# Guillaume-SOULIER/SOS-Radiative-Transfer

Measured on AMD Instinct MI355X. Metric: SOS columns/sec to 1e-4 convergence (Ntau=200, Nmu=128), higher is better.
Workload: dtype f64

## Files before the change

### include/sosrt.h

```cpp
#ifndef SOSRT_H
#define SOSRT_H

#ifdef __cplusplus
extern "C" {
#endif

typedef struct sosrt_handle sosrt_t;

#define SOSRT_OK              0
#define SOSRT_E_INVALID      -1
#define SOSRT_E_HIP          -2
#define SOSRT_E_STATE        -3
#define SOSRT_E_NOMEM        -4

#define SOSRT_COL_OK           0
#define SOSRT_COL_INDEXERROR   1
#define SOSRT_COL_MAXORDERS    2
#define SOSRT_COL_INTERNAL     3

#define SOSRT_GEOM_THREE_ZONE  0
#define SOSRT_GEOM_SINGLE_SLAB 1

#define SOSRT_SURFACE_NONE       0
#define SOSRT_SURFACE_SPECULAR   1
// ... 78 lines not shown
#define SOSRT_PHASE_TABLE     3
int sosrt_phase_table(sosrt_t* h, const double* tab_mu, const double* tab_p, int ntab);
int sosrt_phase_table_dev(sosrt_t* h, const double* d_tab_mu, const double* d_tab_p, int ntab);

#define SOSRT_MIE_MAX_X 20000.0
#define SOSRT_MIE_MAX_MX 200000.0
#define SOSRT_MIE_MAX_WORKSPACE (2ull << 30)
int sosrt_mie_ensembles(sosrt_t* h, int S, const double* wl, const double* m_re, const double* m_im, const double* r_m,
                        const double* sig, int nb_radius, double r_min, double r_max, int ntab, double* p_out, double* bulk_out);
int sosrt_mie_ensembles_dev(sosrt_t* h, int S, const double* wl, const double* m_re, const double* m_im, const double* r_m,
                            const double* sig, int nb_radius, double r_min, double r_max, int ntab, double* d_p_out,
                            double* d_bulk_out);
int sosrt_mie_efficiencies(sosrt_t* h, int K, const double* m_re, const double* m_im, const double* x, double* out);
int sosrt_mie_timing(sosrt_t* h, double* ms );

int sosrt_phase_p0_dev(sosrt_t* h, int B, int kind, double g, const double* d_mu0, double* d_P0_out);
int sosrt_phase_p0(sosrt_t* h, int B, int kind, double g, const double* mu0, double* P0_out);
int sosrt_phase_matrix(sosrt_t* h, int kind, double g, double* P_out);
int sosrt_phase_matrix_dev(sosrt_t* h, int kind, double g, double* d_P_out);

#define SOSRT_MAX_MODES 64
int sosrt_phase_modes(sosrt_t* h, int kind, double g, int m_first, int m_count, int nphi, double* P_out);
int sosrt_phase_p0_modes_dev(sosrt_t* h, int B, int kind, double g, int m_first, int m_count, int nphi, const double* d_mu0,
                             double* d_P0_out);
int sosrt_phase_p0_modes(sosrt_t* h, int B, int kind, double g, int m_first, int m_count, int nphi, const double* mu0,
                         double* P0_out);
int sosrt_set_order_targets(sosrt_t* h, const int* d_targets);
int sosrt_azimuth_accumulate_dev(sosrt_t* h, int B, int m, const double* d_Im, int nlev, const int* d_levels, int nphi_out,
                                 const double* d_phi, double* d_out);

int sosrt_comm_unique_id(void* id_out);
int sosrt_comm_init(sosrt_t* h, int rank, int world, const void* unique_id);
int sosrt_gather(sosrt_t* h, int root, const long long* counts, const double* d_send, double* d_recv);
int sosrt_comm_destroy(sosrt_t* h);

int sosrt_limit_mu_down(sosrt_t* h, int R, int idx, const double* rows, double* out);
int sosrt_asymptotic_down(sosrt_t* h, int R, int stride, const int* len, const double* J, const double* tau,
                          const double* tau_t, const double* mu, double* out);

int sosrt_plan_weights(sosrt_t* h, double* w_out );
int sosrt_plan_fold(sosrt_t* h, int which , double* W_out );
int sosrt_plan_fix_table(sosrt_t* h, int idx, int* s0, int* ns, double* C_out);
int sosrt_plan_fix_count(double tau_ref, int N);
#define SOSRT_PLAN_GEMM_DENSE        0
#define SOSRT_PLAN_GEMM_LIVE64       1
#define SOSRT_PLAN_GEMM_LIVE32       2
#define SOSRT_PLAN_GEMM_LIVE32_DEEP  3
#define SOSRT_PLAN_GEMM_LIVE16_REGS  4
#define SOSRT_PLAN_TRANSPORT_GENERAL 0
#define SOSRT_PLAN_TRANSPORT_FAST    1
#define SOSRT_PLAN_TRANSPORT_RING    3
#define SOSRT_PLAN_TRANSPORT_SCAN    4
int sosrt_plan_launch(sosrt_t* h, int batch, int live, int surface, int zones, int cus, int* out );

#define SOSRT_K_GEMM      0
#define SOSRT_K_TRANSPORT 1
#define SOSRT_K_FIRST     2
#define SOSRT_K_SMALLMU   3
#define SOSRT_K_ORDER_LOOP 4
#define SOSRT_K_COUNT     5
int sosrt_profile_enable(sosrt_t* h, int on);
int sosrt_profile_reset(sosrt_t* h);
int sosrt_profile_get(sosrt_t* h, int kernel, double* total_ms, long long* launches, double* work );

int sosrt_debug_stamps(sosrt_t* h, unsigned long long* d_stamps);

int sosrt_microbench(sosrt_t* h, int which, double* result);

#ifdef __cplusplus
}
#endif
#endif
```

### sos-radiative-transfer_amd/csrc/api.hip

```cpp
#include <hip/hip_runtime.h>

#include <algorithm>
#include <cmath>
#include <cstdarg>
#include <cstdio>
#include <cstdlib>
#include <chrono>
#include <cstring>
#include <mutex>
#include <new>
#include <string>
#include <vector>

#include "../../include/sosrt.h"
#include "comm.hpp"
#include "kernels.hpp"
#include "plan.hpp"

using namespace sosrt;

namespace {
thread_local std::string g_err;

int fail(int code, const char* fmt, ...) {
// ... 62 lines not shown
    int ntab = 0;
    char* d_mie = nullptr;
    char* h_mie = nullptr;
    size_t mie_cap = 0, mie_hcap = 0;
    hipEvent_t mie_ev = nullptr, mie_t[4] = {nullptr, nullptr, nullptr, nullptr};
    bool mie_timed = false;
    bool resident = false;
    int resident_B = 0;
    FixTab* d_fix = nullptr;
    int* d_small = nullptr;
    int *d_idx_up = nullptr, *d_idx_down = nullptr;
    int *d_nz = nullptr, *d_zr0 = nullptr, *d_zmix = nullptr;
    double *d_zwr = nullptr, *d_zdtr = nullptr;
    int max_nz = 1;
    bool simple_zones = true;
    double* d_scal = nullptr;
    ColDesc* d_desc = nullptr;
    double *d_rca = nullptr, *d_rcr = nullptr;
    int* d_slabrows = nullptr;
    int* d_mainrows = nullptr;
    int nslab = 0, nmain = 0;
    int max_main = 0, max_slab = 0;
    static constexpr int kMaxMixGroups = 32;
    static constexpr int kMaxMixGroupsSets = 128;
    static constexpr size_t kMixCacheBytes = 256ull << 20;
    int mix_groups_max = 1 << 30;
    bool wr_on_device = false;
    int nsets = 1;
    std::vector<std::vector<double>> Wrx_h;
    double* d_Wrsets = nullptr;
    size_t wrsets_capacity = 0;
    double* d_Wrsets_s = nullptr;
    size_t wrsets_s_capacity = 0;
    int* d_mixset = nullptr;
    int max_set_used = 0;
    int p0_zones = 0;
    double* d_P0rz = nullptr;
    size_t p0rz_capacity = 0;
    std::vector<int> c_nz, c_zr0, c_zmix, c_zset;
    std::vector<double> c_zwr, c_zdtr, c_alb_atm, c_dtau_atm;
    int mix_groups = 0;
    bool mix_dirty = true;
    double *d_Wmix = nullptr, *d_mixca = nullptr, *d_mixcr = nullptr;
    int* d_mixgroup = nullptr;
    int* d_slabtilegroup = nullptr;
    int contraction = SOSRT_CONTRACT_F64;
    double asymmetry = 0;
    bool sym_ok = false;
    bool sym_dirty = true, symmix_dirty = true, symsets_dirty = true;
    double *d_Wa_s = nullptr, *d_Wr_s = nullptr, *d_Wmix_s = nullptr;
    int lr_rank = -1;
    double lr_residual = 0;
    double *d_lrU = nullptr, *d_lrV = nullptr;
    size_t mixs_capacity = 0;
    float *d_Wa32 = nullptr, *d_Wmix32 = nullptr;
    size_t mix32_capacity = 0;
    bool w32_dirty = true;
    int* d_livelist = nullptr;
    size_t mix_capacity = 0;
    double *d_tau = nullptr, *d_P0a = nullptr, *d_P0r = nullptr;
    double *d_Jn = nullptr, *d_InA = nullptr, *d_InB = nullptr, *d_I = nullptr, *d_E = nullptr;
    int use_etab = 1;
    int *d_active = nullptr, *d_norders = nullptr, *d_status = nullptr, *d_redo = nullptr, *d_erep = nullptr;
    int *d_nactive_sets = nullptr, *d_nactive = nullptr;
    int nactive_set = 0;
    unsigned long long* d_tauhash = nullptr;
    int transport_mode = 3;
    int scan_cols = 200;
    bool ring_ok = false, scan_ok = false, scan_split_ok = false;
    int scan_split = 1;
    int cu_count = 0;
    double* d_scan_scratch = nullptr;
    int* d_scan_sync = nullptr;
    int gemm_tail_cols = 1 << 30;
    double gemm_tail_frac = 0.6;
    int gemm_small_cols = 200;
    int dense_live_list = 1;
    int gemm_regs_cols = -1;
    bool fast_ok = false;
    double* d_ratio = nullptr;
    int* h_pub = nullptr;
    bool need_small = true;
    int pub_seq = 0;
    int last_max_orders = 0;
    long long last_sum_orders = 0;
    Prof prof[kMaxGroups];
    int order_loop = 0;
    double ol_frac = 0.5;
    int* d_olsync = nullptr;
    int* h_oldone = nullptr;
    unsigned long long* d_ollog = nullptr;
    int ol_launches = 0, ol_refused = 0;
    bool ol_group_used[kMaxGroups] = {false, false};
    Rccl::comm_t comm = nullptr;
    int comm_rank = -1, comm_world = 0;
};

namespace {

size_t field_elems(const sosrt_handle* h) { return (size_t)h->max_batch * h->L * h->D; }

template <class T>
int dalloc(T** p, size_t n) {
    hipError_t e = hipMalloc((void**)p, n * sizeof(T));
    if (e != hipSuccess) return fail(SOSRT_E_NOMEM, "hipMalloc of %zu bytes failed: %s", n * sizeof(T), hipGetErrorString(e));
    return 0;
// ... 178 lines not shown
}

int ensure_matrices(sosrt_handle* h, hipStream_t s) {
    const Grid& g = h->g;
    const size_t per = (size_t)g.Dp * g.Wld;
    const bool mixed = h->mix_groups > 0 && h->mix_dirty;
    if (mixed) {
        prof_break(h);
        const bool sets = h->max_set_used > 0;
        launch_wmix(s, per, h->mix_groups, h->d_Wa, sets ? h->d_Wrsets : h->d_Wr, h->d_mixca, h->d_mixcr, h->d_Wmix,
                    sets ? h->d_mixset : nullptr);
        h->mix_dirty = false;
        h->symmix_dirty = true;
    }
    if (!use_sym(h)) return 0;
    if (h->sym_dirty) {
        prof_break(h);
        if (!h->d_Wa_s) { if (int e = dalloc(&h->d_Wa_s, per)) return e; }
        if (!h->d_Wr_s) { if (int e = dalloc(&h->d_Wr_s, per)) return e; }
        launch_symfold(s, 1, g.N, g.D, g.Dp, g.Wld, h->d_Wa, h->d_Wa_s);
        launch_symfold(s, 1, g.N, g.D, g.Dp, g.Wld, h->d_Wr, h->d_Wr_s);
        h->sym_dirty = false;
        h->symsets_dirty = true;
    }
    if (h->symsets_dirty && h->nsets > 1 && h->mix_groups == 0 && h->max_set_used > 0) {
        prof_break(h);
        {
            if (per * h->nsets > h->wrsets_s_capacity) {
                if (h->d_Wrsets_s) hipFree(h->d_Wrsets_s);
                h->d_Wrsets_s = nullptr; h->wrsets_s_capacity = 0;
                if (int e = dalloc(&h->d_Wrsets_s, per * h->nsets)) return e;
                h->wrsets_s_capacity = per * h->nsets;
            }
            launch_symfold(s, h->nsets, g.N, g.D, g.Dp, g.Wld, h->d_Wrsets, h->d_Wrsets_s);
        }
        h->symsets_dirty = false;
    }
    if (h->mix_groups > 0 && h->symmix_dirty) {
        prof_break(h);
        const size_t need = per * h->mix_groups;
        if (need > h->mixs_capacity) {
            if (h->d_Wmix_s) hipFree(h->d_Wmix_s);
            h->d_Wmix_s = nullptr; h->mixs_capacity = 0;
            if (int e = dalloc(&h->d_Wmix_s, need)) return e;
            h->mixs_capacity = need;
        }
        launch_symfold(s, h->mix_groups, g.N, g.D, g.Dp, g.Wld, h->d_Wmix, h->d_Wmix_s);
        h->symmix_dirty = false;
    }
    return 0;
}

void run_source(sosrt_handle* h, const double* In_1, double* Jn, const int* active, int tail_cols = 0, int pub_tag = 0,
                int grp = -1, bool all_live = false, bool regs_tile = false, int dense_live_cap = 0) {
    const int g0 = grp < 0 ? 0 : grp, g1 = grp < 0 ? h->ngroups : grp + 1;
    const int pg = grp < 0 ? 0 : grp;
    hipStream_t s = group_stream(h, pg);
    GemmArgs ga;
    ga.A = In_1; ga.Wa = h->d_Wa; ga.Wr = h->d_Wr; ga.ca = h->d_rca; ga.cr = h->d_rcr;
    if (h->nslab > 0) {
        ga.rows_main = h->d_mainrows + h->main_off[g0];
        ga.n_main = h->main_off[g1] - h->main_off[g0];
    } else {
        ga.rows_main = nullptr;
        ga.n_main = (h->gb[g1] - h->gb[g0]) * h->L;
        ga.A = In_1 + (size_t)h->gb[g0] * h->L * h->D;
        Jn += (size_t)h->gb[g0] * h->L * h->D;
        ga.ca = h->d_rca + (size_t)h->gb[g0] * h->L;
        ga.cr = h->d_rcr + (size_t)h->gb[g0] * h->L;
        if (active) active += h->gb[g0];
    }
    ga.rows_slab = h->d_slabrows + h->slab_off[g0]; ga.n_slab = h->slab_off[g1] - h->slab_off[g0];
    ga.D = h->g.D; ga.Dp = h->g.Dp; ga.Wld = h->g.Wld; ga.L = h->L; ga.C = Jn; ga.active = active;
    if (grp >= 0 && h->ngroups > 1) ga.pad_lds = h->coresident_pad;
    if (pub_tag) {
        ga.nactive = h->d_nactive + pg; ga.need_small = h->d_nactive + sosrt_handle::kMaxGroups;
        ga.host_pub = h->h_pub + 8 * pg; ga.tag = pub_tag;
    }
    ga.check_tiles = all_live ? 0 : 1;
    if (ensure_matrices(h, s)) return;
    if (h->mix_groups > 0) {
        ga.Wmix = h->d_Wmix; ga.mix_group = h->d_mixgroup; ga.slab_tile_group = h->d_slabtilegroup + h->slab_off[g0] / 32;
    }
    const bool two_pass_sets = h->mix_groups == 0 && h->max_set_used > 0 && h->nslab > 0;
    if (two_pass_sets) {
        ga.Wr = h->d_Wrsets; ga.mix_group = h->d_mixgroup; ga.slab_tile_group = h->d_slabtilegroup + h->slab_off[g0] / 32;
    }
    if (use_lowrank(h)) { ga.lr_rank = h->lr_rank; ga.lrU = h->d_lrU; ga.lrV = h->d_lrV; }
    if (use_sym(h)) {
        ga.sym = 1; ga.Ks = (h->g.N + GEMM_KC - 1) / GEMM_KC * GEMM_KC;
#ifdef SOSRT_DIAG
        if (h->diag_ks_mult > 1 && ga.Ks * h->diag_ks_mult <= h->g.Dp) ga.Ks *= h->diag_ks_mult;
#endif
        ga.Wa = h->d_Wa_s; ga.Wr = two_pass_sets ? h->d_Wrsets_s : h->d_Wr_s;
        if (ga.Wmix) ga.Wmix = h->d_Wmix_s;
    }
    if (h->contraction == SOSRT_CONTRACT_F32) {
        if (h->w32_dirty) {
            prof_break(h);
            const size_t per = (size_t)h->g.Dp * h->g.Wld;
            launch_to_float(s, per, h->d_Wa, h->d_Wa32);
            if (h->mix_groups > 0) launch_to_float(s, per * h->mix_groups, h->d_Wmix, h->d_Wmix32);
            h->w32_dirty = false;
        }
        prof_begin(h, SOSRT_K_GEMM, pg);
        launch_gemm_f32(s, ga, h->d_Wa32, h->d_Wmix32);
        prof_end(h, SOSRT_K_GEMM, pg);
        return;
    }
    prof_begin(h, SOSRT_K_GEMM, pg);
    if (tail_cols > 0 && active && h->nslab >= 0) {
        ga.col0 = h->nslab > 0 ? h->gb[g0] : 0; ga.B = h->gb[g1] - h->gb[g0];
        ga.max_main = h->max_main; ga.max_slab = h->max_slab;
        ga.idx_up = h->nslab > 0 ? h->d_idx_up : nullptr; ga.idx_down = h->nslab > 0 ? h->d_idx_down : nullptr;
        ga.live_list = h->d_livelist + h->gb[g0]; ga.live_cap = tail_cols;
        launch_gemm_tail(s, ga, tail_cols, tail_cols <= h->gemm_small_cols, regs_tile);
    } else {
        if (dense_live_cap > 0 && active && h->nslab >= 0) {
            ga.col0 = h->nslab > 0 ? h->gb[g0] : 0; ga.B = h->gb[g1] - h->gb[g0];
            ga.live_list = h->d_livelist + h->gb[g0]; ga.live_cap = dense_live_cap;
        }
        launch_gemm(s, ga);
    }
    prof_end(h, SOSRT_K_GEMM, pg);
}

struct SolveShape {
    bool ring_like = false;
    bool fast = false;
    int nzcap = kRingZones;
    int ring_mode = 1;
};
SolveShape solve_shape(const sosrt_handle* h, int max_nz) {
    SolveShape sh;
    sh.ring_like = h->transport_mode >= 2 && h->ring_ok && (max_nz <= kRingZones || transport_ring_fits(h->g, max_nz));
    sh.fast = h->transport_mode >= 1 && h->fast_ok && (max_nz <= kRingZones || sh.ring_like);
    sh.nzcap = max_nz > kRingZones ? max_nz : kRingZones;
    sh.ring_mode = (h->transport_mode >= 2 && h->ring_ok) ? 3 : 1;
    return sh;
}
struct OrderInputs {
    int nb = 0;
    int known = 0;
    int surface = SOSRT_SURFACE_NONE;
    bool simple_zones = true;
    bool slabs_mixed = true;
    bool need_small = false;
    bool saving = false;
    int orders_left = 1 << 30;
    int cu_share = 0;
};
struct LaunchPlan {
    int tail_cols = 0;
    int live_cap = 0;
    int gemm = SOSRT_PLAN_GEMM_DENSE;
    int transport = SOSRT_PLAN_TRANSPORT_GENERAL;
    int parts = 1;
    int repair = 0;
    int order_loop = 0;
    int ol_parts = 0;
    int ol_grid = 0;
};
LaunchPlan plan_order(const sosrt_handle* h, const SolveShape& sh, const OrderInputs& in) {
    LaunchPlan pl;
    const Grid& g = h->g;
    const bool live_tiling = h->contraction != SOSRT_CONTRACT_F32 && in.simple_zones && in.known <= h->gemm_tail_cols &&
                             (in.known <= h->gemm_tail_frac * in.nb || in.nb <= h->gemm_small_cols) &&
                             (in.known < in.nb || in.nb <= h->gemm_small_cols);
    pl.tail_cols = live_tiling ? in.known : 0;
    pl.gemm = !live_tiling ? SOSRT_PLAN_GEMM_DENSE
                           : (pl.tail_cols <= h->gemm_small_cols ? ((use_sym(h) && pl.tail_cols <= 32) ? SOSRT_PLAN_GEMM_LIVE32_DEEP : SOSRT_PLAN_GEMM_LIVE32)
                                                                 : SOSRT_PLAN_GEMM_LIVE64);
    {
        const int nct = (g.D + GEMM_BN - 1) / GEMM_BN;
        const int auto_cap = (3 * h->cu_count / 2) / (((g.L + 15) / 16 + 1) * nct);
        const int cap = h->gemm_regs_cols >= 0 ? h->gemm_regs_cols : auto_cap;
        if (live_tiling && use_sym(h) && pl.tail_cols <= cap && 16 * (g.D + 2) * 8 <= 150 * 1024 &&
            ((g.N + GEMM_KC - 1) / GEMM_KC * GEMM_KC) % 64 == 0) pl.gemm = SOSRT_PLAN_GEMM_LIVE16_REGS;
    }
    pl.live_cap = live_tiling ? pl.tail_cols : ((h->contraction != SOSRT_CONTRACT_F32 && h->dense_live_list && in.known < in.nb) ? in.known : 0);
    {
        const int cols_now = pl.live_cap > 0 ? pl.live_cap : in.nb;
        const int split_cap = sh.ring_mode == 3 ? h->cu_count : 4 * h->cu_count;
        const bool can_split = h->scan_split && h->scan_split_ok && transport_scan_parts(g) * cols_now <= split_cap &&
                               (in.surface == SOSRT_SURFACE_SPECULAR || in.surface == SOSRT_SURFACE_NONE);
        const bool want_scan = h->transport_mode == 4 || (h->transport_mode == 3 && cols_now <= h->scan_cols);
        const bool split = can_split && transport_scan_fits(g, sh.nzcap, true) && (sh.fast || (h->use_etab && h->transport_mode >= 3));
        const bool scan = want_scan && ((sh.fast && sh.ring_mode == 3 && h->scan_ok && transport_scan_fits(g, sh.nzcap, false)) || split);
        pl.transport = scan ? SOSRT_PLAN_TRANSPORT_SCAN
                            : (!sh.fast ? SOSRT_PLAN_TRANSPORT_GENERAL : (sh.ring_mode == 3 ? SOSRT_PLAN_TRANSPORT_RING : SOSRT_PLAN_TRANSPORT_FAST));
        if (scan && split) pl.parts = transport_scan_parts(g);
        pl.repair = (h->N - 3 > 61 && pl.transport == SOSRT_PLAN_TRANSPORT_FAST) ? 1 : 0;
    }
    if (h->order_loop && in.cu_share > 0 && h->transport_mode == 3 && sh.fast && sh.ring_mode == 3 && sh.nzcap <= kRingZones &&
        use_sym(h) && in.simple_zones && in.slabs_mixed && !in.saving && !in.need_small && in.orders_left >= 1 &&
        in.known <= kOrderLoopMaxCols) {
        Grid gt = g;
        gt.nsmall = 0;
        const bool split_ok = h->scan_split && (in.surface == SOSRT_SURFACE_SPECULAR || in.surface == SOSRT_SURFACE_NONE) && order_loop_ok(gt, true);
        const int sp = order_loop_parts(gt, true);
        if (split_ok && sp * in.known <= h->ol_frac * in.cu_share) {
            pl.order_loop = 1; pl.ol_parts = sp;
        } else if (order_loop_ok(gt, false) && in.known <= h->ol_frac * in.cu_share) {
            pl.order_loop = 1; pl.ol_parts = 1;
        }
        if (pl.order_loop) pl.ol_grid = in.cu_share;
    }
    return pl;
}

std::mutex g_ol_mutex;
int g_ol_held[64];
int ol_acquire(int device, int total, int want, int least) {
    if (device < 0 || device >= 64) return 0;
    std::lock_guard<std::mutex> lk(g_ol_mutex);
    int got = total - g_ol_held[device];
    if (got > want) got = want;
    if (got < least || got <= 0) return 0;
    g_ol_held[device] += got;
    return got;
}
void ol_release(int device, int n) {
    if (device < 0 || device >= 64 || n <= 0) return;
    std::lock_guard<std::mutex> lk(g_ol_mutex);
    g_ol_held[device] -= n;
}

}

extern "C" {

const char* sosrt_last_error(void) { return g_err.c_str(); }
int sosrt_version(void) { return SOSRT_VERSION; }

int sosrt_plan_fix_count(double tau_ref, int N) { return fix_count(tau_ref, N); }

int sosrt_create(int device, int L, int N, int max_batch, int max_orders, sosrt_t** out) {
    if (!out) return fail(SOSRT_E_INVALID, "out is null");
    *out = nullptr;
    if (L < 2) return fail(SOSRT_E_INVALID, "nb_layers must be >= 2 (got %d)", L);
    if (N < 4) return fail(SOSRT_E_INVALID, "nb_angles must be >= 4 (got %d)", N);
    if (N > 1024) return fail(SOSRT_E_INVALID, "nb_angles must be <= 1024 (got %d)", N);
    if (max_batch < 1 || max_orders < 1) return fail(SOSRT_E_INVALID, "max_batch and max_orders must be >= 1");
    {
        const int nt = (N + 63) / 64 * 64;
        const size_t need = (size_t)(3 * (size_t)L + nt + nt / 64 + 4) * sizeof(double);
        if (need > 64 * 1024)
            return fail(SOSRT_E_INVALID, "nb_layers = %d does not fit: at most %d layers at nb_angles = %d", L,
                        (int)((64 * 1024 / sizeof(double) - nt - nt / 64 - 4) / 3), N);
    }
    sosrt_handle* h = new (std::nothrow) sosrt_handle();
    if (!h) return fail(SOSRT_E_NOMEM, "out of host memory");
    h->device = device; h->L = L; h->N = N; h->D = 2 * N; h->max_batch = max_batch; h->max_orders = max_orders;
    h->order_budget = max_orders;
    h->saved_slots = max_orders;
    h->gpu = device >= 0;
    h->cu_count = 256;
    if (const char* ev = getenv("SOSRT_ETAB")) h->use_etab = atoi(ev);
    if (const char* ev = getenv("SOSRT_CONTRACT"))
        if (strcmp(ev, "full") == 0) h->contraction = SOSRT_CONTRACT_F64_FULL;
    if (const char* ev = getenv("SOSRT_TRANSPORT"))
        h->transport_mode = strcmp(ev, "general") == 0 ? 0 : (strcmp(ev, "ring") == 0 ? 2 : (strcmp(ev, "scan") == 0 ? 4 : (strcmp(ev, "auto") == 0 ? 3 : 1)));
    if (const char* ev = getenv("SOSRT_SCAN_COLS")) h->scan_cols = atoi(ev);
    if (const char* ev = getenv("SOSRT_SCAN_SPLIT")) h->scan_split = atoi(ev);
    if (const char* ev = getenv("SOSRT_GEMM_TAIL")) h->gemm_tail_cols = atoi(ev);
    if (const char* ev = getenv("SOSRT_GEMM_TAIL_FRAC")) h->gemm_tail_frac = atof(ev);
    if (const char* ev = getenv("SOSRT_GEMM_SMALL")) h->gemm_small_cols = atoi(ev);
    if (const char* ev = getenv("SOSRT_DENSE_LIVE_LIST")) h->dense_live_list = atoi(ev) != 0;
    if (const char* ev = getenv("SOSRT_GEMM_REGS")) h->gemm_regs_cols = atoi(ev);
    if (const char* ev = getenv("SOSRT_GROUPS")) h->want_groups = atoi(ev) >= 2 ? 2 : (atoi(ev) == 1 ? 1 : 0);
    if (const char* ev = getenv("SOSRT_SPLIT_MIN")) h->split_min = atoi(ev);
    if (const char* ev = getenv("SOSRT_MIX_GROUPS")) h->mix_groups_max = atoi(ev);
#ifdef SOSRT_DIAG
    if (const char* ev = getenv("SOSRT_STAGGER")) h->stagger = atof(ev);
    if (const char* ev = getenv("SOSRT_GROUP_SPLIT")) h->split_at = atoi(ev);
    if (const char* ev = getenv("SOSRT_GROUP_PRIO")) h->prio2 = atoi(ev);
    if (const char* ev = getenv("SOSRT_GEMM_PAD_LDS")) h->coresident_pad = atoi(ev);
    if (const char* ev = getenv("SOSRT_GEMM_KS_MULT")) h->diag_ks_mult = atoi(ev);
#endif
    if (const char* ev = getenv("SOSRT_GROUP_RING_SLOTS")) h->coresident_slots = atoi(ev);
    if (const char* ev = getenv("SOSRT_ORDER_LOOP")) h->order_loop = atoi(ev) != 0;
    if (const char* ev = getenv("SOSRT_RING_SLOTS")) g_ring_slots = atoi(ev);
#ifdef SOSRT_RING_DEBUG
    if (const char* ev = getenv("SOSRT_RING_DEBUG")) g_ring_debug = atoi(ev);
#endif
    Grid& g = h->g;
    g.L = L; g.N = N; g.D = 2 * N;
    g.Dp = (g.D + GEMM_KC - 1) / GEMM_KC * GEMM_KC;
    g.Wld = (g.D + GEMM_BN - 1) / GEMM_BN * GEMM_BN;
    if (h->gpu) {
        int e = 0;
        auto body = [&]() -> int {
            HIPCHK(hipSetDevice(device));
            HIPCHK(hipStreamCreateWithFlags(&h->own_stream, hipStreamDefault));
            h->stream = h->own_stream;
            HIPCHK(hipEventCreateWithFlags(&h->ev_fork, hipEventDisableTiming));
            HIPCHK(hipEventCreateWithFlags(&h->ev_join, hipEventDisableTiming));
            const size_t mb = max_batch, fe = field_elems(h);
            if ((e = dalloc(&h->d_mu, g.D))) return e;
            if ((e = dalloc(&h->d_Wa, (size_t)g.Dp * g.Wld))) return e;
            if ((e = dalloc(&h->d_Wr, (size_t)g.Dp * g.Wld))) return e;
            if ((e = dalloc(&h->d_lrU, (size_t)kLowRankMax * g.D))) return e;
            if ((e = dalloc(&h->d_lrV, (size_t)kLowRankMax * g.D))) return e;
            if ((e = dalloc(&h->d_wfdn, N))) return e;
            if ((e = dalloc(&h->d_wfup, N))) return e;
            if ((e = dalloc(&h->d_w, g.D))) return e;
            if ((e = dalloc(&h->d_phi, 2 * kNPhi))) return e;
            if ((e = dalloc(&h->d_z, L))) return e;
            if ((e = dalloc(&h->d_fix, 4))) return e;
            if ((e = dalloc(&h->d_small, N))) return e;
            if ((e = dalloc(&h->d_idx_up, mb))) return e;
            if ((e = dalloc(&h->d_idx_down, mb))) return e;
            if ((e = dalloc(&h->d_nz, mb))) return e;
            if ((e = dalloc(&h->d_zr0, mb * kMaxZones))) return e;
            if ((e = dalloc(&h->d_zmix, mb * kMaxZones))) return e;
            if ((e = dalloc(&h->d_zwr, mb * kMaxZones))) return e;
            if ((e = dalloc(&h->d_zdtr, mb * kMaxZones))) return e;
            if ((e = dalloc(&h->d_scal, 7 * mb))) return e;
            if ((e = dalloc(&h->d_desc, mb))) return e;
            if ((e = dalloc(&h->d_rca, mb * L))) return e;
            if ((e = dalloc(&h->d_rcr, mb * L))) return e;
            if ((e = dalloc(&h->d_slabrows, mb * L + 64 * (size_t)sosrt_handle::kMaxMixGroupsSets * sosrt_handle::kMaxGroups))) return e;
            if ((e = dalloc(&h->d_slabtilegroup, mb * L / 32 + 2 * sosrt_handle::kMaxMixGroupsSets * sosrt_handle::kMaxGroups + 2))) return e;
            if ((e = dalloc(&h->d_mainrows, mb * L))) return e;
            if ((e = dalloc(&h->d_tau, mb * L))) return e;
            if ((e = dalloc(&h->d_P0a, mb * g.D))) return e;
            if ((e = dalloc(&h->d_P0r, mb * g.D))) return e;
            if ((e = dalloc(&h->d_Jn, fe))) return e;
            if ((e = dalloc(&h->d_InA, fe))) return e;
            if ((e = dalloc(&h->d_InB, fe))) return e;
            if ((e = dalloc(&h->d_I, fe))) return e;
            if ((e = dalloc(&h->d_E, fe))) return e;
            if ((e = dalloc(&h->d_active, mb))) return e;
            if ((e = dalloc(&h->d_norders, mb))) return e;
            if ((e = dalloc(&h->d_status, mb))) return e;
            if ((e = dalloc(&h->d_nactive_sets, 2 * (sosrt_handle::kMaxGroups + 1)))) return e;
            HIPCHK(hipMemset(h->d_nactive_sets, 0, 2 * (sosrt_handle::kMaxGroups + 1) * sizeof(int)));
            h->d_nactive = h->d_nactive_sets;
            if ((e = dalloc(&h->d_redo, mb))) return e;
            if ((e = dalloc(&h->d_erep, mb))) return e;
            if ((e = dalloc(&h->d_mixgroup, mb))) return e;
            if ((e = dalloc(&h->d_livelist, mb))) return e;
            if ((e = dalloc(&h->d_mixca, sosrt_handle::kMaxMixGroupsSets))) return e;
            if ((e = dalloc(&h->d_mixcr, sosrt_handle::kMaxMixGroupsSets))) return e;
            if ((e = dalloc(&h->d_mixset, sosrt_handle::kMaxMixGroupsSets))) return e;
            if ((e = dalloc(&h->d_tauhash, mb))) return e;
            if ((e = dalloc(&h->d_ratio, mb))) return e;
            if ((e = dalloc(&h->d_scan_scratch, mb * transport_scan_scratch_doubles()))) return e;
            if ((e = dalloc(&h->d_scan_sync, 2 * mb))) return e;
            if ((e = dalloc(&h->d_olsync, sosrt_handle::kMaxGroups * order_loop_sync_ints(kOrderLoopMaxCols)))) return e;
            HIPCHK(hipHostMalloc((void**)&h->h_oldone, 2 * sosrt_handle::kMaxGroups * sizeof(int), hipHostMallocCoherent));
            memset(h->h_oldone, 0, 2 * sosrt_handle::kMaxGroups * sizeof(int));
            HIPCHK(hipMemset(h->d_scan_sync, 0, 2 * mb * sizeof(int)));
            HIPCHK(hipDeviceGetAttribute(&h->cu_count, hipDeviceAttributeMultiprocessorCount, device));
            HIPCHK(hipHostMalloc((void**)&h->h_pub, (8 * sosrt_handle::kMaxGroups + 2) * sizeof(int), hipHostMallocCoherent));
            memset(h->h_pub, 0, (8 * sosrt_handle::kMaxGroups + 2) * sizeof(int));

            HIPCHK(hipMemset(h->d_Wa, 0, (size_t)g.Dp * g.Wld * sizeof(double)));
            HIPCHK(hipMemset(h->d_Wr, 0, (size_t)g.Dp * g.Wld * sizeof(double)));
            HIPCHK(hipMemset(h->d_status, 0, mb * sizeof(int)));
            HIPCHK(hipMemset(h->d_redo, 0, mb * sizeof(int)));
            HIPCHK(hipMemset(h->d_tau, 0, mb * L * sizeof(double)));
            return 0;
        };
        if ((e = body())) { sosrt_destroy(h); return e; }
        g.mu = h->d_mu; g.Wa = h->d_Wa; g.Wr = h->d_Wr; g.fix = h->d_fix; g.small_lanes = h->d_small;
        g.wflux_dn = h->d_wfdn; g.wflux_up = h->d_wfup; g.nsmall = 0;
    }
    *out = h;
    return 0;
}

int sosrt_destroy(sosrt_t* h) {
    if (!h) return 0;
    if (h->gpu) {
        hipSetDevice(h->device);
        if (h->comm) { rccl().CommDestroy(h->comm); h->comm = nullptr; }
        if (h->own_stream) hipStreamSynchronize(h->own_stream);
        void* ptrs[] = {h->d_mu, h->d_Wa, h->d_Wr, h->d_wfdn, h->d_wfup, h->d_fix, h->d_small, h->d_idx_up,
                        h->d_idx_down, h->d_scal, h->d_desc, h->d_rca, h->d_rcr, h->d_slabrows, h->d_mainrows, h->d_tau, h->d_P0a,
                        h->d_P0r, h->d_Jn, h->d_InA, h->d_InB, h->d_I, h->d_E, h->d_active, h->d_norders, h->d_status,
                        h->d_nactive_sets, h->d_ratio, h->d_redo, h->d_erep, h->d_tauhash, h->d_Wmix, h->d_mixca, h->d_mixcr,
                        h->d_mixgroup, h->d_Wa_s, h->d_Wr_s, h->d_Wmix_s, h->d_scan_scratch, h->d_scan_sync, h->d_w, h->d_phi, h->d_z, h->d_tab, h->d_slabtilegroup, h->d_livelist, h->d_Wa32, h->d_Wmix32, h->d_nz, h->d_zr0, h->d_zmix, h->d_zwr, h->d_zdtr, h->d_olsync, h->d_ollog, h->d_modetab, h->d_lrU, h->d_lrV, h->d_Wrsets, h->d_Wrsets_s, h->d_mixset, h->d_P0rz};
        for (void* p : ptrs)
            if (p) hipFree(p);
        if (h->h_pub) hipHostFree(h->h_pub);
        if (h->h_oldone) hipHostFree(h->h_oldone);
        if (h->d_mie) hipFree(h->d_mie);
        if (h->h_mie) hipHostFree(h->h_mie);
        if (h->mie_ev) hipEventDestroy(h->mie_ev);
        for (auto& e : h->mie_t)
            if (e) hipEventDestroy(e);

        for (auto& p : h->prof)
            for (auto& e : p.ev) hipEventDestroy(e);
        if (h->stream2) { hipStreamSynchronize(h->stream2); hipStreamDestroy(h->stream2); }
        if (h->ev_fork) hipEventDestroy(h->ev_fork);
        if (h->ev_join) hipEventDestroy(h->ev_join);
        if (h->own_stream) hipStreamDestroy(h->own_stream);
    }
    delete h;
    return 0;
}

int sosrt_set_stream(sosrt_t* h, void* s) {
    if (int e = need_gpu(h)) return e;
    h->stream = (hipStream_t)s;
    return 0;
}

int sosrt_use_own_stream(sosrt_t* h) {
    if (int e = need_gpu(h)) return e;
    h->stream = h->own_stream;
    return 0;
}

int sosrt_set_saved_orders(sosrt_t* h, int slots) {
    if (!h) return fail(SOSRT_E_INVALID, "null handle");
    if (slots < 1 || slots > h->max_orders) return fail(SOSRT_E_INVALID, "slots must be in 1..max_orders=%d (got %d)", h->max_orders, slots);
    h->saved_slots = slots;
    return 0;
}

int sosrt_set_order_budget(sosrt_t* h, int max_orders) {
    if (!h) return fail(SOSRT_E_INVALID, "null handle");
    if (max_orders < 1 || max_orders > h->max_orders)
        return fail(SOSRT_E_INVALID, "the order budget must be in 1..max_orders=%d of sosrt_create (got %d)", h->max_orders, max_orders);
    h->order_budget = max_orders;
    return 0;
}

int sosrt_set_first_order(sosrt_t* h, int mode) {
    if (int e = need_gpu(h)) return e;
    if (mode != SOSRT_FIRST_ORDER_CODED && mode != SOSRT_FIRST_ORDER_README) return fail(SOSRT_E_INVALID, "unknown first-order mode %d", mode);
    if (mode == SOSRT_FIRST_ORDER_README && (h->nsets > 1 || h->p0_zones > 0))
        return fail(SOSRT_E_INVALID, "SOSRT_FIRST_ORDER_README reads one aerosol matrix: it cannot be combined with several phase sets");
    if (mode == SOSRT_FIRST_ORDER_README && h->geom != SOSRT_GEOM_THREE_ZONE)
        return fail(SOSRT_E_INVALID, "the README's Lambertian first order needs the three-zone geometry (it has a surface)");
    h->first_order_mode = mode;
    return 0;
}

int sosrt_set_contraction(sosrt_t* h, int mode) {
    if (int e = need_gpu(h)) return e;
    if (mode != SOSRT_CONTRACT_F64 && mode != SOSRT_CONTRACT_F32 && mode != SOSRT_CONTRACT_F64_FULL && mode != SOSRT_CONTRACT_F64_DENSE) return fail(SOSRT_E_INVALID, "unknown contraction mode %d", mode);
    if (mode == SOSRT_CONTRACT_F32) {
        HIPCHK(hipSetDevice(h->device));
        const size_t per = (size_t)h->g.Dp * h->g.Wld;
        if (!h->d_Wa32) { if (int e = dalloc(&h->d_Wa32, per)) return e; }
        h->w32_dirty = true;
    }
    h->contraction = mode;
    return 0;
}

int sosrt_set_order_loop(sosrt_t* h, int mode) {
    if (!h) return fail(SOSRT_E_INVALID, "null handle");
    if (mode < 0 || mode > 2) return fail(SOSRT_E_INVALID, "order-loop mode must be 0, 1 or 2 (got %d)", mode);
    h->order_loop = mode;
    return 0;
}

int sosrt_order_loop_stats(sosrt_t* h, int* launches, int* refused, long long* column_orders) {
    if (!h) return fail(SOSRT_E_INVALID, "null handle");
    if (launches) *launches = h->ol_launches;
    if (refused) *refused = h->ol_refused;
    if (column_orders) {
        *column_orders = 0;
        if (h->gpu && h->ol_launches > 0) {
            HIPCHK(hipSetDevice(h->device));
            HIPCHK(hipStreamSynchronize(h->stream));
            if (h->stream2) HIPCHK(hipStreamSynchronize(h->stream2));
            for (int k = 0; k < sosrt_handle::kMaxGroups; ++k) {
                if (!h->ol_group_used[k]) continue;
                int v = 0;
                HIPCHK(hipMemcpy(&v, h->d_olsync + (size_t)k * order_loop_sync_ints(kOrderLoopMaxCols) + kOlOrders, sizeof v, hipMemcpyDeviceToHost));
                *column_orders += v;
            }
        }
    }
    return 0;
}

int sosrt_plan_launch(sosrt_t* h, int batch, int live, int surface, int zones, int cus, int* out) {
    if (!h || !out) return fail(SOSRT_E_INVALID, "null argument");
    if (!h->have_grid) return fail(SOSRT_E_STATE, "sosrt_set_grid has not been called");
    if (batch < 1 || live < 0 || live > batch) return fail(SOSRT_E_INVALID, "need 0 <= live <= batch, batch >= 1");
    if (zones < 1 || zones > kMaxZones) return fail(SOSRT_E_INVALID, "zones must be in 1..%d", kMaxZones);
    int want = h->want_groups;
    if (want == 0) want = batch > h->split_min ? 2 : 1;
    const int ng = (want >= 2 && batch >= h->split_min && batch >= 2) ? 2 : 1;
    const int nb = ng == 2 ? batch / 2 : batch;
    const int saved_cus = h->cu_count;
    if (cus > 0) h->cu_count = cus;
    const SolveShape sh = solve_shape(h, zones);
    OrderInputs oi;
    oi.nb = nb; oi.known = live < nb ? live : nb; oi.surface = surface;
    oi.simple_zones = zones == 3 || zones == 1;
    oi.cu_share = h->cu_count / ng;
    const bool saved_sym = h->sym_ok;
    if (!h->have_phase) h->sym_ok = true;
    const LaunchPlan pl = plan_order(h, sh, oi);
    h->sym_ok = saved_sym;
    h->cu_count = saved_cus;
    out[0] = ng; out[1] = pl.gemm; out[2] = pl.tail_cols; out[3] = pl.transport; out[4] = pl.parts; out[5] = pl.repair;
    out[6] = pl.order_loop; out[7] = pl.ol_parts; out[8] = pl.ol_grid;
    return 0;
}

int sosrt_phase_asymmetry(sosrt_t* h, double* asymmetry, int* uses_symmetry) {
    if (!h) return fail(SOSRT_E_INVALID, "null handle");
    if (!h->have_phase) return fail(SOSRT_E_STATE, "sosrt_set_phase has not been called");
    if (asymmetry) *asymmetry = h->asymmetry;
    if (uses_symmetry) *uses_symmetry = use_sym(h) ? 1 : 0;
    return 0;
}

int sosrt_phase_rank(sosrt_t* h, int* rank, double* residual, int* uses) {
    if (!h) return fail(SOSRT_E_INVALID, "null handle");
    if (!h->have_phase) return fail(SOSRT_E_STATE, "sosrt_set_phase has not been called");
    if (rank) *rank = h->lr_rank;
    if (residual) *residual = h->lr_residual;
    if (uses) *uses = use_lowrank(h) ? 1 : 0;
    return 0;
}

int sosrt_synchronize(sosrt_t* h) {
    if (int e = need_gpu(h)) return e;
    HIPCHK(hipStreamSynchronize(h->stream));
    return 0;
}

int sosrt_set_grid(sosrt_t* h, const double* mu) {
    if (!h || !mu) return fail(SOSRT_E_INVALID, "null argument");
    for (int k = 0; k < h->D; ++k)
        if (!std::isfinite(mu[k])) return fail(SOSRT_E_INVALID, "mu[%d] is not finite", k);
    for (int k = 0; k < h->N; ++k) {
        if (!(mu[k] <= 0)) return fail(SOSRT_E_INVALID, "mu[%d]=%g: the first nb_angles directions must be <= 0", k, mu[k]);
        if (!(mu[h->N + k] >= 0)) return fail(SOSRT_E_INVALID, "mu[%d]=%g: the last nb_angles directions must be >= 0", h->N + k, mu[h->N + k]);
    }
    h->plan.set_grid(h->N, mu);
    for (int b = 0; b < 4; ++b)
        if (h->plan.fix[b].idx > kFixMaxIdx) return fail(SOSRT_E_INVALID, "nb_angles too large for the extrapolation tables");
    h->have_grid = true;
    h->have_phase = false;
    h->fast_ok = transport_fast_ok(h->plan);
    if (h->gpu) {
        HIPCHK(hipSetDevice(h->device));
        HIPCHK(hipMemcpy(h->d_mu, mu, h->D * sizeof(double), hipMemcpyHostToDevice));
        HIPCHK(hipMemcpy(h->d_wfdn, h->plan.wflux_dn.data(), h->N * sizeof(double), hipMemcpyHostToDevice));
        HIPCHK(hipMemcpy(h->d_wfup, h->plan.wflux_up.data(), h->N * sizeof(double), hipMemcpyHostToDevice));
        HIPCHK(hipMemcpy(h->d_w, h->plan.w.data(), h->D * sizeof(double), hipMemcpyHostToDevice));
        {
            double phi[kNPhi], tab[2 * kNPhi];
            const double step = 3.141592653589793 / (kNPhi - 1);
            for (int q = 0; q < kNPhi; ++q) phi[q] = q * step;
            phi[kNPhi - 1] = 3.141592653589793;
            for (int q = 0; q < kNPhi; ++q) {
                tab[q] = std::cos(0 - phi[q]);
// ... 772 lines not shown
                if (got == 0) { oi.cu_share = 0; pl = plan_order(h, shape, oi); }
                else { pl.ol_grid = got; ol_held[k] = got; }
            }
            if (pl.order_loop && h->order_loop == 2) pl.ol_grid = 2 * h->cu_count;
            if (pl.order_loop) {
                OrderLoopArgs oa;
                Grid gt = g;
                gt.nsmall = 0;
                oa.t = TransportArgs{gt, tau_g, h->d_Jn + fo, nullptr, d_I_out + fo, nullptr, 0, h->d_desc + q.b0, q.cv, 0, 1, h->d_E, erep_g, nullptr};
                oa.t.nzcap = kRingZones;
                oa.t.scan_split = pl.ol_parts > 1 ? 1 : 0;
                oa.t.scan_scratch = h->d_scan_scratch + (size_t)q.b0 * transport_scan_scratch_doubles();
                oa.t.scan_sync = h->d_scan_sync + 2 * q.b0;
                GemmArgs& ga = oa.gm;
                ga.A = nullptr; ga.Wa = h->d_Wa_s; ga.Wr = h->d_Wr_s; ga.ca = h->d_rca; ga.cr = h->d_rcr;
                ga.D = g.D; ga.Dp = g.Dp; ga.Wld = g.Wld; ga.L = h->L; ga.C = h->d_Jn;
                ga.sym = 1; ga.Ks = (g.N + GEMM_KC - 1) / GEMM_KC * GEMM_KC;
                if (use_lowrank(h)) { ga.lr_rank = h->lr_rank; ga.lrU = h->d_lrU; ga.lrV = h->d_lrV; }
                ga.max_main = h->max_main; ga.max_slab = h->max_slab;
                ga.idx_up = h->nslab > 0 ? h->d_idx_up : nullptr; ga.idx_down = h->nslab > 0 ? h->d_idx_down : nullptr;
                if (h->mix_groups > 0) { ga.Wmix = h->d_Wmix_s; ga.mix_group = h->d_mixgroup; }
                oa.in0 = q.In_1;
                oa.gbufP = q.In;
                oa.gbufQ = (q.In_1 == d_I_out) ? h->d_InA : q.In_1;
                oa.bufP = oa.gbufP + fo; oa.bufQ = oa.gbufQ + fo;
                oa.order0 = q.n + 1; oa.kmax = h->order_budget - q.n;
                oa.B = q.nb; oa.col0 = q.b0;
                oa.fixcap = (int)(0.06 * g.N) + 1;
                oa.sync = h->d_olsync + (size_t)k * order_loop_sync_ints(kOrderLoopMaxCols);
                oa.host_done = h->h_oldone + 2 * k;
                oa.tag = q.ol_tag = ((++h->pub_seq) & 0x3fffffff) | 0x40000000;
#ifdef SOSRT_OL_STAMPS
                if (getenv("SOSRT_OL_LOG")) {
                    if (!h->d_ollog) { if (int e = dalloc(&h->d_ollog, 65001)) return bail(e); }
                    HIPCHK(hipMemsetAsync(h->d_ollog, 0, 8, sg));
                    oa.log = h->d_ollog;
                }
#endif
                prof_break(h);
                HIPCHK(hipMemsetAsync(oa.sync, 0, order_loop_sync_ints(q.known) * sizeof(int), sg));
                prof_begin(h, SOSRT_K_ORDER_LOOP, k);
                const hipError_t le = launch_order_loop(sg, pl.ol_grid, pl.ol_parts > 1, oa);
                prof_end(h, SOSRT_K_ORDER_LOOP, k);
                if (le != hipSuccess) return bail(fail(SOSRT_E_HIP, "order-loop launch failed: %s", hipGetErrorString(le)));
                q.ol_pending = true;
                used_order_loop = true;
                ++h->ol_launches;
                continue;
            }
            const int n = ++q.n;
            n_max = n > n_max ? n : n_max;
            const int tail_cols = pl.tail_cols;
            run_source(h, q.In_1, h->d_Jn, h->d_active, tail_cols, tagbase + n - 1, k, q.known == q.nb, pl.gemm == SOSRT_PLAN_GEMM_LIVE16_REGS,
                       tail_cols > 0 ? 0 : pl.live_cap);
            if (g.nsmall > 0 && h->need_small) {
                prof_begin(h, SOSRT_K_SMALLMU, k);
                launch_smallmu(sg, g, q.nb, tau_g, h->d_Jn + fo, q.In + fo, h->d_desc + q.b0, q.cv.active);
                prof_end(h, SOSRT_K_SMALLMU, k);
            }
            prof_begin(h, SOSRT_K_TRANSPORT, k);
            double* sv_n = (d_I_saved_out && n <= h->saved_slots) ? d_I_saved_out + (size_t)q.b0 * saved_stride + (size_t)(n - 1) * LD : nullptr;
            if (pl.transport != SOSRT_PLAN_TRANSPORT_GENERAL) {
                Grid gt = g;
                if (pl.transport >= SOSRT_PLAN_TRANSPORT_RING && !h->need_small) gt.nsmall = 0;
                launch_transport(sg, gt, q.nb, tau_g, h->d_Jn + fo, q.In + fo, d_I_out + fo, sv_n, saved_stride, h->d_desc + q.b0, q.cv, n, 1,
                                 h->d_E, pl.transport, erep_g, pl.live_cap, h->d_livelist + q.b0, NG > 1 ? h->coresident_slots : 0,
                                 pl.parts > 1 ? 1 : 0, h->d_scan_scratch + (size_t)q.b0 * transport_scan_scratch_doubles(),
                                 h->d_scan_sync + 2 * q.b0, nzcap);
                if (pl.repair)
                    launch_transport(sg, g, q.nb, tau_g, h->d_Jn + fo, q.In + fo, d_I_out + fo, sv_n, saved_stride, h->d_desc + q.b0, q.cv, n, 1,
                                     h->d_E, 2, erep_g);
            } else {
                launch_transport(sg, g, q.nb, tau_g, h->d_Jn + fo, q.In + fo, d_I_out + fo, sv_n, saved_stride, h->d_desc + q.b0, q.cv, n, 1,
                                 h->use_etab ? h->d_E : nullptr, 0, erep_g);
            }
            prof_end(h, SOSRT_K_TRANSPORT, k);
            if (q.In_1 == d_I_out) { q.In_1 = q.In; q.In = h->d_InA; }
            else { double* tmp = q.In_1; q.In_1 = q.In; q.In = tmp; }
        }
        if (!progressed) __builtin_ia32_pause();
    }
    if (NG > 1) {
        HIPCHK(hipEventRecord(h->ev_join, h->stream2));
        HIPCHK(hipStreamWaitEvent(s, h->ev_join, 0));
    }
    prof_break(h);
    launch_finalize(s, B, make_conv(h, tol), h->order_budget, d_n_orders_out, d_status_out);
    HIPCHK(hipGetLastError());
    h->last_max_orders = used_order_loop ? -1 : n_max;
    h->last_sum_orders = -1;
    return 0;
}

int sosrt_solve(sosrt_t* h, int B, const double* tau, const double* P0_atm, const double* P0_aer, double tol,
                const double* I1_in, double* I_out, double* I_saved_out, int* n_orders_out, int* status_out) {
    if (int e = check_ready(h, B, true)) return e;
    if (!tau) return fail(SOSRT_E_INVALID, "null argument");
    HIPCHK(hipSetDevice(h->device));
    hipStream_t s = h->stream;
    h->resident = false;
    const size_t LD = (size_t)h->L * h->D, n = (size_t)B * LD;
    HIPCHK(hipMemcpyAsync(h->d_tau, tau, (size_t)B * h->L * sizeof(double), hipMemcpyHostToDevice, s));
    if (P0_atm) HIPCHK(hipMemcpyAsync(h->d_P0a, P0_atm, (size_t)B * h->D * sizeof(double), hipMemcpyHostToDevice, s));
    const double* d_p0r = nullptr;
    if (int e = stage_p0_aer(h, B, P0_aer, s, &d_p0r)) return e;
    double* d_I1 = nullptr;
    double* d_saved = nullptr;
    int rc = 0;
    auto body = [&]() -> int {
        if (I1_in) {
            if (int e = dalloc(&d_I1, n)) return e;
            HIPCHK(hipMemcpyAsync(d_I1, I1_in, n * sizeof(double), hipMemcpyHostToDevice, s));
        }
        if (I_saved_out) {
            if (int e = dalloc(&d_saved, (size_t)B * h->saved_slots * LD)) return e;
            HIPCHK(hipMemsetAsync(d_saved, 0, (size_t)B * h->saved_slots * LD * sizeof(double), s));
        }
        if (int e = sosrt_solve_dev(h, B, h->d_tau, P0_atm ? h->d_P0a : nullptr, d_p0r, tol, d_I1,
                                    h->d_I, d_saved, nullptr, nullptr))
            return e;
        if (I_out) HIPCHK(hipMemcpyAsync(I_out, h->d_I, n * sizeof(double), hipMemcpyDeviceToHost, s));
// ... 759 lines not shown
```

### sos-radiative-transfer_amd/csrc/jn_gemm_tile.hpp

```cpp
#pragma once
#include "kernels.hpp"
#include "transport_util.hpp"

namespace sosrt {

namespace {

typedef double f64x4 __attribute__((ext_vector_type(4)));

constexpr int A_LD = GEMM_KC + 2;
constexpr int B_LD = GEMM_BN + 16;

struct ListRows {
    const int* rows;
    int n;
    __device__ int operator()(int lr) const { return lr < n ? (rows ? rows[lr] : lr) : -1; }
};
struct ColumnRows {
    int base, iu, ns, n;
    bool slab;
    __device__ int operator()(int lr) const {
        if (lr >= n) return -1;
        return base + (slab ? iu + lr : (lr < iu ? lr : lr + ns));
    }
// ... 290 lines not shown
        const int b_ = (blk_);                                                                                    \
        if (b_ < nblk) {                                                                                          \
            const int pass_ = b_ >= nkb ? 1 : 0;                                                                  \
            lone_load(F, pass_ ? rW1 : rW0, b_ - pass_ * nkb, fk, Wld, Nh, mcol);                                 \
        }                                                                                                         \
    }
    const __amdgpu_buffer_rsrc_t rW0 = make_rsrc(wmix ? wmix : g.Wa, g.Dp * Wld * 8);
    const __amdgpu_buffer_rsrc_t rW1 = make_rsrc(SLAB ? g.Wr : g.Wa, g.Dp * Wld * 8);
    if (!PRELOADED) {
        SOSRT_LONE_LOAD(f0, 0);
        SOSRT_LONE_LOAD(f1, 1);
    }
    asm volatile("s_waitcnt vmcnt(0)" ::: "memory");
    __syncthreads();
    f64x4 accx = (f64x4){0, 0, 0, 0}, accy = (f64x4){0, 0, 0, 0};
    const double* __restrict__ arow = sRaw + (size_t)fr * RS;
#define SOSRT_LONE_COMPUTE(F, blk_)                                                                               \
    {                                                                                                             \
        const int b_ = (blk_);                                                                                    \
        const int pass_ = b_ >= nkb ? 1 : 0;                                                                      \
        const double cf_ = pass_ ? cf_r : cf_a;                                                                   \
        const int k0_ = 4 * (b_ - pass_ * nkb) * LONE_KB + fk;                                                    \
        _Pragma("unroll") for (int q = 0; q < LONE_KB; ++q) {                                                     \
            const int k_ = k0_ + 4 * q;                                                                           \
            const bool ok_ = grow >= 0 && k_ < Nn;                                                                \
            const double a_ = arow[k_], m_ = arow[D - 1 - k_];                  \
            const double u_ = ok_ ? cf_ * (a_ + m_) : 0.0, v_ = ok_ ? cf_ * (a_ - m_) : 0.0;                      \
            accx = __builtin_amdgcn_mfma_f64_16x16x4f64(u_, F.s[q], accx, 0, 0, 0);                               \
            accy = __builtin_amdgcn_mfma_f64_16x16x4f64(v_, F.a[q], accy, 0, 0, 0);                               \
        }                                                                                                         \
    }
    for (int blk = 0; blk < nblk; blk += 2) {
        SOSRT_LONE_COMPUTE(f0, blk);
        SOSRT_LONE_LOAD(f0, blk + 2);
        if (blk + 1 < nblk) {
            SOSRT_LONE_COMPUTE(f1, blk + 1);
            SOSRT_LONE_LOAD(f1, blk + 3);
        }
    }
#undef SOSRT_LONE_LOAD
#undef SOSRT_LONE_COMPUTE
#pragma unroll
    for (int r = 0; r < 4; ++r) {
        const int gr = row_of(tile * 16 + 4 * r + fk);
        if (gr >= 0 && mcol < Nn) {
            const double x = accx[r], y = accy[r];
            g.C[(size_t)gr * D + mcol] = x + y;
            g.C[(size_t)gr * D + D - 1 - mcol] = x - y;
        }
    }
}

constexpr int LR_ROWS = 4;
template <bool COH>
__device__ __forceinline__ void lowrank_rows(const GemmArgs& g, const int (&rows)[LR_ROWS], int lane) {
    const int D = g.D, R = g.lr_rank;
    __amdgpu_buffer_rsrc_t rA[LR_ROWS], rC[LR_ROWS];
    double cf[LR_ROWS];
#pragma unroll
    for (int i = 0; i < LR_ROWS; ++i) {
        const int r = rows[i] >= 0 ? rows[i] : rows[0];
        const int bytes = rows[i] >= 0 ? D * 8 : 0;
        rA[i] = make_rsrc(g.A + (size_t)r * D, bytes);
        rC[i] = make_rsrc(g.C + (size_t)r * D, bytes);
        cf[i] = rows[i] >= 0 ? g.ca[rows[i]] : 0.0;
    }
    const double* __restrict__ U = g.lrU;
    const double* __restrict__ V = g.lrV;
    double m[LR_ROWS][kLowRankMax];
#pragma unroll
    for (int i = 0; i < LR_ROWS; ++i)
#pragma unroll
        for (int q = 0; q < kLowRankMax; ++q) m[i][q] = 0.0;
#pragma unroll 2
    for (int k = 2 * lane; k < D; k += 128) {
        double2 x[LR_ROWS];
#pragma unroll
        for (int i = 0; i < LR_ROWS; ++i) x[i] = bload2_aux<COH ? 16 : 0>(rA[i], k * 8, 0);
#pragma unroll
        for (int q = 0; q < kLowRankMax; ++q) {
            if (q < R) {
                const double2 u = *reinterpret_cast<const double2*>(U + (size_t)q * D + k);
#pragma unroll
                for (int i = 0; i < LR_ROWS; ++i) m[i][q] = __builtin_fma(x[i].y, u.y, __builtin_fma(x[i].x, u.x, m[i][q]));
            }
        }
    }
#pragma unroll
    for (int s = 32; s >= 1; s >>= 1)
#pragma unroll
        for (int q = 0; q < kLowRankMax; ++q)
            if (q < R) {
#pragma unroll
                for (int i = 0; i < LR_ROWS; ++i) m[i][q] += __shfl_xor(m[i][q], s);
            }
#pragma unroll 2
    for (int k = 2 * lane; k < D; k += 128) {
        double2 o[LR_ROWS];
#pragma unroll
        for (int i = 0; i < LR_ROWS; ++i) o[i] = make_double2(0.0, 0.0);
#pragma unroll
        for (int q = 0; q < kLowRankMax; ++q) {
            if (q < R) {
                const double2 v = *reinterpret_cast<const double2*>(V + (size_t)q * D + k);
#pragma unroll
                for (int i = 0; i < LR_ROWS; ++i) {
                    o[i].x = __builtin_fma(m[i][q], v.x, o[i].x);
                    o[i].y = __builtin_fma(m[i][q], v.y, o[i].y);
                }
            }
        }
#pragma unroll
        for (int i = 0; i < LR_ROWS; ++i) bstore2_aux<COH ? 17 : 0>(rC[i], k * 8, 0, make_double2(cf[i] * o[i].x, cf[i] * o[i].y));
    }
}
template <bool COH, class RowOf>
__device__ __forceinline__ void lowrank_tile(const GemmArgs& g, RowOf row_of, int tile, int BM, int bn0, bool check_active) {
    const int nct = (g.D + GEMM_BN - 1) / GEMM_BN, ct = bn0 / GEMM_BN;
    const int lane = threadIdx.x & 63, wave = __builtin_amdgcn_readfirstlane(threadIdx.x) >> 6;
    const int per = (BM - ct + nct - 1) / nct;
    const bool chk = check_active && g.active && g.check_tiles;
    for (int j = LR_ROWS * wave; j < per; j += 4 * LR_ROWS) {
        int rows[LR_ROWS];
        int n = 0;
#pragma unroll
        for (int i = 0; i < LR_ROWS; ++i) {
            int r = j + i < per ? __builtin_amdgcn_readfirstlane(row_of(tile * BM + ct + nct * (j + i))) : -1;
            if (chk && r >= 0 && !g.active[r / g.L]) r = -1;
            rows[i] = r;
            n += r >= 0 ? 1 : 0;
        }
        if (n == 0) continue;
        if (rows[0] < 0)
#pragma unroll
            for (int i = 1; i < LR_ROWS; ++i)
                if (rows[i] >= 0) { rows[0] = rows[i]; rows[i] = -1; break; }
        lowrank_rows<COH>(g, rows, lane);
    }
}

constexpr int TAIL_RT_SLAB = 1;
constexpr int TAIL_RT = 2;

}
}
```

### sos-radiative-transfer_amd/csrc/kernels.hip

```cpp
#include <cstdlib>

#include "kernels.hpp"

#include "../../include/sosrt.h"

namespace sosrt {


typedef double f64x4 __attribute__((ext_vector_type(4)));

#define SOSRT_PI 3.14159265358979323846

__device__ __forceinline__ double wave_fmax(double v) {
#pragma unroll
    for (int o = 32; o > 0; o >>= 1) v = fmax(v, __shfl_xor(v, o, 64));
    return v;
}
__device__ __forceinline__ double wave_sum(double v) {
#pragma unroll
    for (int o = 32; o > 0; o >>= 1) v += __shfl_xor(v, o, 64);
    return v;
}

__device__ double block_pymax(double x, bool valid, double* s_red, int first_tid = 0) {
// ... 957 lines not shown
            bool same = true;
            for (int i = lane; i < L; i += 64) same = same && (tb[i] == tc[i]);
            if (__ballot(!same) == 0) rep = cc;
        }
    }
    if (lane == 0) erep[b] = rep;
}
void launch_tau_groups(hipStream_t s, const Grid& g, int B, const double* tau, unsigned long long* hash, int* erep,
                       const int* need_small, int* host_flag, int tag) {
    hipLaunchKernelGGL(k_tau_rep, dim3(B), dim3(64), 0, s, g.L, tau, hash, erep, need_small, host_flag, tag);
}

template <int MAXT>
static void launch_transport_t(hipStream_t s, dim3 grid, dim3 block, size_t shm, const TransportArgs& a, int mode) {
    if (mode == 1) {
        launch_transport_fast(s, grid, block, a);
    } else if (mode == 3) {
        launch_transport_ring(s, grid, a, g_ring_slots);
    } else if (mode == 4) {
        launch_transport_scan(s, grid, a);
    } else if (mode == 2) {
        if (a.accumulate) {
            if (a.saved) hipLaunchKernelGGL((k_transport<MAXT, true, true, true, true>), grid, block, shm, s, a);
            else hipLaunchKernelGGL((k_transport<MAXT, true, false, true, true>), grid, block, shm, s, a);
        } else {
            hipLaunchKernelGGL((k_transport<MAXT, false, false, true, true>), grid, block, shm, s, a);
        }
    } else if (a.accumulate) {
        if (a.Etab) {
            if (a.saved) hipLaunchKernelGGL((k_transport<MAXT, true, true, true>), grid, block, shm, s, a);
            else hipLaunchKernelGGL((k_transport<MAXT, true, false, true>), grid, block, shm, s, a);
        } else {
            if (a.saved) hipLaunchKernelGGL((k_transport<MAXT, true, true, false>), grid, block, shm, s, a);
            else hipLaunchKernelGGL((k_transport<MAXT, true, false, false>), grid, block, shm, s, a);
        }
    } else {
        if (a.Etab) hipLaunchKernelGGL((k_transport<MAXT, false, false, true>), grid, block, shm, s, a);
        else hipLaunchKernelGGL((k_transport<MAXT, false, false, false>), grid, block, shm, s, a);
    }
}

unsigned long long* g_transport_stamps = nullptr;
int g_ring_slots = 3, g_ring_debug = 0;

bool transport_fast_ok(const Plan& plan) {
    for (int bkt = 0; bkt < 4; ++bkt)
        if (plan.fix[bkt].idx > 0 && (plan.fix[bkt].s0 >> 6) != ((plan.N - 1) >> 6)) return false;
    return true;
}

void launch_transport(hipStream_t s, const Grid& g, int B, const double* tau, const double* Jn, double* In, double* I,
                      double* saved, size_t saved_col_stride, const ColDesc* desc, Conv cv, int order,
                      int accumulate, const double* Etab, int mode, const int* erep, int live, const int* live_list,
                      int ring_slots, int scan_split, double* scan_scratch, int* scan_sync, int nzcap) {
    const int nt = round64(g.N);
    const size_t shm = (size_t)(g.L + 2 * TC * (nt + 2) + 2 * nt + nt / 64 + 2) * sizeof(double);
    TransportArgs a{g, tau, Jn, In, I, accumulate ? saved : nullptr, saved_col_stride, desc, cv, order, accumulate, Etab, Etab ? erep : nullptr, g_transport_stamps};
    a.slots = ring_slots;
    a.nzcap = nzcap > kRingZones ? nzcap : kRingZones;
    if (mode == 4 && scan_split && scan_scratch && scan_sync) { a.scan_split = 1; a.scan_scratch = scan_scratch; a.scan_sync = scan_sync; }
    if ((mode == 3 || mode == 4) && accumulate && live > 0 && live < B && live_list) {
        a.live = live;
        a.live_list = live_list;
        B = live;
    }
    if (nt <= 128) launch_transport_t<128>(s, dim3(B), dim3(nt), shm, a, mode);
    else if (nt <= 256) launch_transport_t<256>(s, dim3(B), dim3(nt), shm, a, mode);
    else if (nt <= 512) launch_transport_t<512>(s, dim3(B), dim3(nt), shm, a, mode);
    else launch_transport_t<1024>(s, dim3(B), dim3(nt), shm, a, mode);
}

__global__ void k_finalize(int B, Conv cv, int max_orders, int* __restrict__ n_out, int* __restrict__ status_out) {
    const int b = blockIdx.x * blockDim.x + threadIdx.x;
    if (b >= B) return;
    int st = cv.status[b];
    if (cv.active[b]) { st = SOSRT_COL_MAXORDERS; cv.status[b] = st; }
    if (n_out) n_out[b] = cv.norders[b];
    if (status_out) status_out[b] = st;
}
void launch_finalize(hipStream_t s, int B, Conv cv, int max_orders, int* n_out, int* status_out) {
    hipLaunchKernelGGL(k_finalize, dim3((B + 127) / 128), dim3(128), 0, s, B, cv, max_orders, n_out, status_out);
}

__global__ void k_fluxes(Grid g, int B, const double* __restrict__ tau_all, const double* __restrict__ I_all,
                         const ColDesc* __restrict__ desc, int beam_norm, double* __restrict__ fdn,
                         double* __restrict__ fup) {
    const int row = blockIdx.x * (blockDim.x >> 6) + (threadIdx.x >> 6);
    if (row >= B * g.L) return;
    const int lane = threadIdx.x & 63, b = row / g.L, t = row % g.L;
    const double* I = I_all + (size_t)row * g.D;
    double sd = 0, su = 0;
    for (int k = lane; k < g.N; k += 64) {
        sd += g.wflux_dn[k] * I[k];
        su += g.wflux_up[k] * I[g.N + k];
    }
    sd = wave_sum(sd);
    su = wave_sum(su);
    if (lane == 0) {
        const ColDesc& d = desc[b];
        const double* tau = tau_all + (size_t)b * g.L;
        const double F0 = SOSRT_PI / d.mu0;
        const double fb = beam_norm ? F0 : F0 / (4 * SOSRT_PI);
        fdn[row] = sd - fb * exp(-tau[t] / d.mu0);
        fup[row] = su + fb * d.rho * exp(-(2 * tau[g.L - 1] - tau[t]) / d.mu0);
    }
}
void launch_fluxes(hipStream_t s, const Grid& g, int B, const double* tau, const double* I, const ColDesc* desc,
                   int beam_norm, double* fdn, double* fup) {
    const int rows = B * g.L;
    hipLaunchKernelGGL(k_fluxes, dim3((rows + 3) / 4), dim3(256), 0, s, g, B, tau, I, desc, beam_norm, fdn, fup);
}

// ... 103 lines not shown
```

### sos-radiative-transfer_amd/csrc/kernels.hpp

```cpp
#pragma once
#include <hip/hip_runtime.h>

#include "plan.hpp"

namespace sosrt {

constexpr int kMaxZones = 8;
constexpr int kRingZones = 3;

struct alignas(16) ColDesc {
    int nz;
    int r0[kMaxZones];
    int r1[kMaxZones];
    int mix[kMaxZones];
    int nfix[kMaxZones];
    int fixtab[kMaxZones];
    int surface;
    int geom;
    double mu0, rho, T, tau_bottom;
    double wa;
    double wr[kMaxZones];
    double fa[kMaxZones];
    double fr[kMaxZones];
    double ca[kMaxZones];
// ... 35 lines not shown
    const double* wflux_dn;
    const double* wflux_up;
};

struct Conv {
    int* active;
    int* norders;
    int* status;
    int* nactive;
    double* ratio;
    int* redo;
    const int* target;
    double tol;
};

__device__ __forceinline__ bool conv_go(const Conv& cv, int b, int order, double r) {
    return cv.target ? order < cv.target[b] : r >= cv.tol;
}

constexpr int GEMM_BM = 64, GEMM_BN = 128, GEMM_KC = 16;
#ifndef SOSRT_GEMM_RT
#define SOSRT_GEMM_RT 4
#endif
#ifndef SOSRT_GEMM_WPS
#define SOSRT_GEMM_WPS 3
#endif
constexpr int GEMM_RT = SOSRT_GEMM_RT;
constexpr int GEMM_WPS = SOSRT_GEMM_WPS;

constexpr int TC = 8;

struct TransportArgs {
    Grid g;
    const double* tau;
    const double* Jn;
    double* In;
    double* I;
    double* saved;
    size_t saved_col_stride;
    const ColDesc* desc;
    Conv cv;
    int order;
    int accumulate;
    const double* Etab;
    const int* erep;
    unsigned long long* stamps;
    int live = 0;
    const int* live_list = nullptr;
    int slots = 0;
    int nzcap = kRingZones;
    int scan_split = 0;
    double* scan_scratch = nullptr;
    int* scan_sync = nullptr;
};
void launch_transport_fast(hipStream_t s, dim3 grid, dim3 block, const TransportArgs& a);
bool transport_ring_ok(const Grid& g);
bool transport_ring_fits(const Grid& g, int nzcap);
void launch_transport_ring(hipStream_t s, dim3 grid, const TransportArgs& a, int slots);
bool transport_scan_ok(const Grid& g);
bool transport_scan_split_ok(const Grid& g);
bool transport_scan_fits(const Grid& g, int nzcap, bool split);
int transport_scan_parts(const Grid& g);
size_t transport_scan_scratch_doubles();
void launch_transport_scan(hipStream_t s, dim3 grid, const TransportArgs& a);
constexpr int kOrderLoopMaxCols = 256;
constexpr int kOlArrive = 0, kOlState = 32, kOlLeft = 64, kOlAbort = 96, kOlOrders = 100, kOlCols = 128;
constexpr int kOlColStride = 64, kOlOrdDone = 0, kOlColStop = 1, kOlJnDone = 32;
constexpr int kOlReady = 1, kOlNotResident = 2, kOlAborted = 3;
inline size_t order_loop_sync_ints(int cols) { return (size_t)kOlCols + (size_t)cols * kOlColStride; }
extern int g_ring_slots, g_ring_debug;
extern unsigned long long* g_transport_stamps;

struct SolveSetup {
    int* zero_next = nullptr;
    int n_zero = 0;
    int* redo = nullptr;
    unsigned long long* hash = nullptr;
    int* scan_sync = nullptr;
};
void launch_prepare(hipStream_t s, const Grid& g, int B, int geom, int surface, ColScalars sc, const double* tau,
                    ColDesc* desc, double* rowcoef_a, double* rowcoef_r, int* need_small = nullptr, SolveSetup su = SolveSetup());
void launch_first_order_readme(hipStream_t s, const Grid& g, const double* w, int B, const double* tau, const double* P0a,
                               const double* P0r, const ColDesc* desc, double* I1_out, double* I_out, double* saved,
                               size_t saved_col_stride, Conv cv, int do_conv);
void launch_first_order(hipStream_t s, const Grid& g, int B, const double* tau, const double* P0a, const double* P0r,
                        const ColDesc* desc, double* I1_out, double* I_out, double* saved, size_t saved_col_stride,
                        Conv cv, int do_conv, int p0r_zones = 0 );
struct GemmArgs {
    const double* A;
    const double* Wa;
    const double* Wr;
    const double* ca;
    const double* cr;
    const int* rows_main;
    int n_main;
    const int* rows_slab;
    int n_slab;
    int D, Dp, Wld, L;
    double* C;
    const int* active;
    int B = 0;
    int col0 = 0;
    const int* idx_up = nullptr;
    const int* idx_down = nullptr;
    int max_main = 0, max_slab = 0;
    const double* Wmix = nullptr;
    const int* mix_group = nullptr;
    int pad_lds = 0;
    int* live_list = nullptr;
    int live_cap = 0;
    const int* slab_tile_group = nullptr;
    const int* nactive = nullptr;
    const int* need_small = nullptr;
    int* host_pub = nullptr;
    int tag = 0;
    int sym = 0;
    int Ks = 0;
    int check_tiles = 1;
    int lr_rank = -1;
    const double* lrU = nullptr;
    const double* lrV = nullptr;
};
constexpr int kLowRankMax = 4;

__device__ inline void publish_live_now(const GemmArgs& g) {
    const int live = __hip_atomic_load(g.nactive, __ATOMIC_RELAXED, __HIP_MEMORY_SCOPE_AGENT);
    int* slot = g.host_pub + 4 * (g.tag & 1);
    __hip_atomic_store(slot, live, __ATOMIC_RELAXED, __HIP_MEMORY_SCOPE_SYSTEM);
    __hip_atomic_store(slot + 2, g.need_small ? g.need_small[0] : 1, __ATOMIC_RELAXED, __HIP_MEMORY_SCOPE_SYSTEM);
    __hip_atomic_store(slot + 1, g.tag, __ATOMIC_RELEASE, __HIP_MEMORY_SCOPE_SYSTEM);
}
__device__ inline void publish_live(const GemmArgs& g) {
    if (g.host_pub && blockIdx.x == 0 && blockIdx.y == 0 && threadIdx.x == 0) publish_live_now(g);
}
struct PerDeviceOnce {
    bool seen[64] = {};
    bool first() {
        int d = 0;
        if (hipGetDevice(&d) != hipSuccess || d < 0 || d >= 64) return true;
        if (seen[d]) return false;
        seen[d] = true;
        return true;
    }
};
void launch_gemm(hipStream_t s, const GemmArgs& a);
struct OrderLoopArgs {
    TransportArgs t;
    GemmArgs gm;
    const double* in0;
    double* gbufP;
    double* gbufQ;
    double* bufP;
    double* bufQ;
    int order0;
    int kmax;
    int B, col0;
    int fixcap;
    int* sync;
    int* host_done;
    int tag;
    unsigned long long* log = nullptr;
    int astage = 0;
};
bool order_loop_ok(const Grid& g, bool split);
int order_loop_parts(const Grid& g, bool split);
hipError_t launch_order_loop(hipStream_t s, int grid, bool split, const OrderLoopArgs& p);
void launch_gemm_f32(hipStream_t s, const GemmArgs& a, const float* Wa32, const float* Wmix32);
void launch_to_float(hipStream_t s, size_t n, const double* src, float* dst);
void launch_wmix(hipStream_t s, size_t n, int ngroups, const double* Wa, const double* Wr, const double* ca, const double* cr,
                 double* Wmix, const int* gset = nullptr );
void launch_fold_sets(hipStream_t s, int S, int D, int Wld, size_t per, const double* w, const double* P, double* W);
void launch_fold_asymmetry(hipStream_t s, int S, int nblk, int D, int Wld, size_t per, const double* W, double* out);
void launch_symfold(hipStream_t s, int nmat, int N, int D, int Dp, int Wld, const double* W, double* SA);
void launch_gemm_tail(hipStream_t s, const GemmArgs& a, int cols, bool small_tiles, bool regs = false);
void launch_smallmu(hipStream_t s, const Grid& g, int B, const double* tau, const double* Jn, double* In,
                    const ColDesc* desc, const int* active);
void launch_transport(hipStream_t s, const Grid& g, int B, const double* tau, const double* Jn, double* In, double* I,
                      double* saved, size_t saved_col_stride, const ColDesc* desc, Conv cv, int order, int accumulate,
                      const double* Etab, int mode, const int* erep = nullptr, int live = 0, const int* live_list = nullptr,
                      int ring_slots = 0, int scan_split = 0, double* scan_scratch = nullptr, int* scan_sync = nullptr,
                      int nzcap = kRingZones);
bool transport_fast_ok(const Plan& plan);
void launch_attenuation(hipStream_t s, const Grid& g, int B, const double* tau, double* Etab, const int* erep);
void launch_tau_groups(hipStream_t s, const Grid& g, int B, const double* tau, unsigned long long* hash, int* erep,
                       const int* need_small = nullptr, int* host_flag = nullptr, int tag = 0);
void launch_fluxes(hipStream_t s, const Grid& g, int B, const double* tau, const double* I, const ColDesc* desc,
                   int beam_norm, double* fdn, double* fup);
struct EpilogueOut {
    double* flux_down;
    double* flux_up;
    double* diffusivity;
    double* heating_rate;
    double* net_toa;
};
void launch_epilogue(hipStream_t s, const Grid& g, const double* w, int B, const double* tau, const double* I,
                     const ColDesc* desc, int beam_norm, const double* z_profile, const EpilogueOut& out);
void launch_phase_p0(hipStream_t s, const Grid& g, const double* w, int B, int kind, double gpar, const double* tab_mu,
                     const double* tab_p, int ntab, const double* cosphi, const double* wphi, int nphi,
                     const double* mu0, double* P0);
void launch_phase_matrix(hipStream_t s, const Grid& g, const double* w, int kind, double gpar, const double* tab_mu,
                         const double* tab_p, int ntab, const double* cosphi, const double* wphi, int nphi, double* P);
constexpr int kMaxModes = 64;
void launch_phase_modes(hipStream_t s, const Grid& g, const double* w, int kind, double gpar, const double* tab_mu,
                        const double* tab_p, int ntab, const double* cosphi, const double* tab, int nphi, int m_first,
                        int m_count, double* P_out);
void launch_phase_p0_modes(hipStream_t s, const Grid& g, const double* w, int B, int kind, double gpar, const double* tab_mu,
                           const double* tab_p, int ntab, const double* cosphi, const double* tab, int nphi, int m_first,
                           int m_count, const double* mu0, double* P0_out);
void launch_azimuth_accumulate(hipStream_t s, const Grid& g, int B, int m, const double* Im, int nlev, const int* levels,
                               int nphi_out, const double* phi, double* out);
constexpr int kMieQ = 6;
constexpr int kMieChunk = 4;
inline int mie_chunks(int R) { return (R + kMieChunk - 1) / kMieChunk; }
void launch_mie_coefficients(hipStream_t s, int nlanes, int R, int n_cap, const double* x, const int* nmax, const int* nstart,
                             const double* m_re, const double* m_im, const double* radii, const double* r_m, const double* sig,
                             double* ab, double* qw);
void launch_mie_angles(hipStream_t s, int S, int R, int ntab, int n_cap, const double* mu, const double* ab, const int* nmax,
                       const double* tn, const double* qw, double* part);
void launch_mie_integrate(hipStream_t s, int S, int R, int ntab, const double* part, const double* radii, const double* qw,
                          double* p, double* bulk);
void launch_limit_rows(hipStream_t s, const Grid& g, int R, int table, const double* rows, double* out);
void launch_asymptotic(hipStream_t s, int R, int stride, const int* len, const double* J, const double* tau,
                       const double* tau_t, const double* mu, double* out);
void launch_finalize(hipStream_t s, int B, Conv cv, int max_orders, int* n_out = nullptr, int* status_out = nullptr);
void launch_bench(hipStream_t s, int which, double* a, double* b, size_t n, int iters);

}
```

### sos-radiative-transfer_amd/csrc/transport_ring.hip

```cpp
#include <type_traits>

#include "../../include/sosrt.h"
#include "kernels.hpp"
#include "transport_util.hpp"

namespace sosrt {

namespace {

#ifndef SOSRT_RING_STORE_AUX
#define SOSRT_RING_STORE_AUX 0
#endif
__device__ __forceinline__ void rstore(__amdgpu_buffer_rsrc_t r, int voff, int soff, double x) { bstore_aux<SOSRT_RING_STORE_AUX>(r, voff, soff, x); }

typedef __attribute__((address_space(3))) void* lds_ptr_t;

constexpr size_t kRingLdsBytes = 152 * 1024;

template <int CNT>
__device__ __forceinline__ void wait_vm() {
    asm volatile("s_waitcnt vmcnt(%0)" ::"n"(CNT) : "memory");
}
__device__ __forceinline__ void wg_barrier() {
    asm volatile("s_waitcnt lgkmcnt(0)\n\ts_barrier" ::: "memory");
}

template <bool ACC, bool SAVED, int PIECES, bool MZ>
__global__ __launch_bounds__(512) void k_transport_ring(TransportArgs a, int NS, int dbg_arg, int fixcap) {
    constexpr int NWL = 2;
#ifdef SOSRT_RING_DEBUG
    const int dbg = dbg_arg;
#else
    constexpr int dbg = 0;
    (void)dbg_arg;
#endif
    int b = blockIdx.x;
    if (ACC && a.live > 0) {
        b = a.live_list[blockIdx.x];
        if (b < 0) return;
    } else if (ACC && !a.cv.active[b]) {
        return;
    }
    const Grid& g = a.g;
    const int tid = threadIdx.x, lane = tid & 63;
    const int wid = __builtin_amdgcn_readfirstlane(tid) >> 6;
    const int L = g.L, N = g.N, D = g.D;
    const int nwc = (N + 63) >> 6;
    const bool loader = wid >= nwc;
    const int lid = wid - nwc;
    const bool w0 = wid == 0 && !(dbg & 8);
    const bool wl = wid == ((N - 1) >> 6) && !(dbg & 4);
    auto stamp = [&](int i) {
        if (a.stamps && (tid == 0 || tid == 64)) a.stamps[((size_t)b * 2 + (tid >> 6)) * 8 + i] = clock64();
    };
    stamp(0);
    constexpr int NARR = ACC ? 3 : 2;
    constexpr int RS = 128 * PIECES;
    constexpr int SLOT = NARR * TC * RS;
    constexpr int IPC = NARR * TC * PIECES;
    extern __shared__ double sm[];
    double* ring = sm;
    double* s_sfc = ring + (size_t)NS * SLOT;
    double* s_fixc = s_sfc;
    double* s_red = s_sfc + max(RS, (MZ ? a.nzcap : kRingZones) * fixcap * kFixMaxSrc);
    double* s_hd = s_red + (blockDim.x >> 6) + 2;
    double* s_S = s_hd + L + 1;
    double* s_x = s_S + (size_t)g.nsmall * L;
    double* s_prmu = s_x + TC * 16;
    int* s_nf = reinterpret_cast<int*>(s_prmu + 16);
    const int xb_dn = max(((N - 1) & 63) - 15, 0);
    __shared__ int s_flag[3];
    const ColDesc* __restrict__ dg = a.desc + b;
    const int nz = dg->nz;
    const ZoneRows<MZ> zr(dg);
    const int nfix0 = dg->nfix[0], nfix1 = dg->nfix[1], nfix2 = dg->nfix[2];
    const int surface = dg->surface;
    const double rho = dg->rho;
    const int fbytes = L * D * 8, RB = D * 8;
    const int lbytes = (dbg & 1) ? 0 : fbytes, sbytes = (dbg & 2) ? 0 : fbytes;
    const __amdgpu_buffer_rsrc_t rJ = make_rsrc(a.Jn + (size_t)b * L * D, lbytes);
    const __amdgpu_buffer_rsrc_t rE = make_rsrc(a.Etab + (size_t)(a.erep ? a.erep[b] : b) * L * D, lbytes);
    const __amdgpu_buffer_rsrc_t rIn = make_rsrc(a.In + (size_t)b * L * D, sbytes);
    const __amdgpu_buffer_rsrc_t rIl = make_rsrc(ACC ? a.I + (size_t)b * L * D : a.In, ACC ? lbytes : 0);
    const __amdgpu_buffer_rsrc_t rI = make_rsrc(ACC ? a.I + (size_t)b * L * D : a.In, ACC ? sbytes : 0);
    const __amdgpu_buffer_rsrc_t rS = make_rsrc(SAVED ? a.saved + (size_t)b * a.saved_col_stride : a.In, SAVED ? sbytes : 0);
    const int NCH = (L + TC - 1) / TC, NQ = 2 * NCH, R = NS - 1;
    const bool valid = tid < N;
    const int tidc = valid ? tid : N - 1;
    unsigned long long sp_dn = NCH > 64 ? ~0ull : 1ull << (NCH - 1), sp_up = sp_dn;
    if (NCH <= 64) {
        sp_dn |= zr.boundary_chunks(L, TC, false);
        sp_up |= zr.boundary_chunks(L, TC, true);
    }
    auto plain_run = [&](unsigned long long mask, int j) {
        const unsigned long long rest = NCH > 64 ? 1ull : mask >> j;
        return rest ? __builtin_ctzll(rest) : 0;
    };
    double rdn_v = 0, rdn_i = 1, rup_v = 0, rup_i = 1;
    double sfc_own = 0;
    int slot_rd = 0;

    int slot_ld = 0;
    auto issue = [&](int q) {
        const bool up = q >= NCH;
        const int j = up ? q - NCH : q;
        double* dst = ring + (size_t)slot_ld * SLOT;
        slot_ld = slot_ld + 1 == NS ? 0 : slot_ld + 1;
        const int half = up ? N * 8 : 0;
        const int vo = lane * 16;
#pragma unroll
        for (int i = 0; i < TC / NWL; ++i) {
            const int u = i * NWL + lid;
            const int row = up ? max(L - 1 - j * TC - u, 0) : min(j * TC + u, L - 1);
#pragma unroll
            for (int p = 0; p < PIECES; ++p) {
                const int so = row * RB + half + p * 1024;
                __builtin_amdgcn_raw_ptr_buffer_load_lds(rJ, (lds_ptr_t)(dst + (0 * TC + u) * RS + p * 128), 16, vo, so, 0, 0);
                __builtin_amdgcn_raw_ptr_buffer_load_lds(rE, (lds_ptr_t)(dst + (1 * TC + u) * RS + p * 128), 16, vo, so, 0, 0);
                if (ACC) __builtin_amdgcn_raw_ptr_buffer_load_lds(rIl, (lds_ptr_t)(dst + (2 * TC + u) * RS + p * 128), 16, vo, so, 0, 0);
            }
        }
    };
    auto loader_phase = [&](auto keep_t, int qa, int qb) {
        constexpr int KEEP = decltype(keep_t)::value;
        for (int q = qa; q < qb; ++q) {
            if (q + R < NQ) {
                issue(q + R);
                wait_vm<KEEP>();
            } else {
                wait_vm<0>();
            }
            wg_barrier();
        }
    };
    const int ncomp = nwc * 64;
    if (loader) {
        for (int q = 0; q < min(R, NQ); ++q) issue(q);
    } else {
        for (int zz = 0; zz < (MZ ? nz : kRingZones); ++zz) {
            const FixTab& src = g.fix[dg->fixtab[zz]];
            for (int i = tid; i < fixcap * kFixMaxSrc; i += ncomp) s_fixc[zz * fixcap * kFixMaxSrc + i] = src.C[i];
        }
        if (tid < 3) s_flag[tid] = 0;
        for (int i = tid; i < (L + 31) / 32; i += ncomp) s_nf[i] = 0;
        const double* __restrict__ tau = a.tau + (size_t)b * L;
        for (int t = tid; t <= L; t += ncomp) s_hd[t] = (t == 0 || t == L) ? 0.0 : (tau[t] - tau[t - 1]) * 0.5;
        if (tid < 16) s_prmu[tid] = (tid > 0 && tid < N) ? 1.0 / g.mu[N + tid] : 0.0;
        const double* __restrict__ In0 = a.In + (size_t)b * L * D;
        for (int i = tid; i < g.nsmall * L; i += ncomp) {
            const int k = i / L, t = i - k * L;
            s_S[i] = In0[(size_t)t * D + g.small_lanes[k]];
        }
    }
    __syncthreads();

    const int seam_barriers = surface == SOSRT_SURFACE_NONE ? 0 : (surface == SOSRT_SURFACE_SPECULAR ? 1 : 3);
    double Bv = 0;
    if (loader) {
        constexpr int PER = IPC / NWL;
        auto run = [&](auto keep_t) {
            loader_phase(keep_t, 0, NCH);
            for (int i = 0; i < seam_barriers; ++i) wg_barrier();
            loader_phase(keep_t, NCH, NQ);
            wait_vm<0>();
        };
        if (R <= 1) run(std::integral_constant<int, 0>{});
        else if (R == 2) run(std::integral_constant<int, (PER < 60 ? PER : 60)>{});
        else if (R == 3) run(std::integral_constant<int, (2 * PER < 60 ? 2 * PER : 60)>{});
        else run(std::integral_constant<int, (3 * PER < 60 ? 3 * PER : 60)>{});
    } else {
    stamp(1);
    const double mu_up = (valid && tid > 0) ? g.mu[N + tidc] : 1.0;
    const int uT = lane >> 3, pT = lane & 7;
    const double muT = (pT + 1 < N) ? g.mu[N + pT + 1] : 1.0;
    const double* xrow = s_x + uT * 16;
    {
        const int m = tidc;
        const int vo = m * 8;
        const double mu = g.mu[m];
        const bool tr = valid && m <= N - 2;
        const bool small = tr && fabs(mu) < kMuThreshold;
        const bool stdl = tr && !small;
        const double nrmu = stdl ? -1.0 / mu : 0.0;
        const bool has_small = wl && g.nsmall > 0;
        double Dv = 0, Jprev = 0;
        double c[kFixMaxSrc] = {0, 0, 0, 0, 0};
        double cT[kFixMaxSrc] = {0, 0, 0, 0, 0};
        int sl[kFixMaxSrc] = {0, 0, 0, 0, 0};
        int nfx = 0;
        bool fixlane = false;
        auto load_fix = [&](int zz) {
            const double* ftC = s_fixc + zz * fixcap * kFixMaxSrc;
            nfx = zz == 0 ? nfix0 : (zz == 1 ? nfix1 : ((!MZ || zz == 2) ? nfix2 : zr.nfix(zz)));
            const int ns = nfx < 2 ? 2 : (nfx < kFixMaxSrc ? nfx : kFixMaxSrc);
            fixlane = valid && nfx > 0 && m >= N - nfx;
            const int i = fixlane ? N - 1 - m : 0;
            const int s0 = nfx < 2 ? N - nfx - 2 : N - nfx - ns;
#pragma unroll
            for (int q = 0; q < kFixMaxSrc; ++q) {
                c[q] = (fixlane && q < ns) ? ftC[i * ns + min(q, ns - 1)] : 0.0;
                cT[q] = (pT < nfx && q < ns) ? ftC[pT * ns + min(q, ns - 1)] : 0.0;
                sl[q] = (s0 + min(q, ns - 1)) & 63;
            }
        };
        if (wl) load_fix(0);
        const int sbase = small ? (m - g.small_lanes[0]) * L : 0;
        int t0 = 0, q = 0;
        auto process = [&](auto special_t, auto mode_t, const double* slot, double (&Jc)[TC], double (&Ic)[TC], double (&Ec)[TC]) __attribute__((always_inline)) {
            constexpr bool SP = decltype(special_t)::value;
            constexpr int MODE = decltype(mode_t)::value;
            double cc[TC], v[TC], Sc[TC];
#pragma unroll
            for (int u = 0; u < TC; ++u) Sc[u] = 0;
            if ((SP || MODE == 2) && has_small) {
#pragma unroll
                for (int u = 0; u < TC; ++u) {
                    const double sv = s_S[sbase + min(t0 + u, L - 1)];
                    Sc[u] = small ? sv : 0.0;
                }
            }
#pragma unroll
            for (int u = 0; u < TC; ++u) {
                const int t = SP ? min(t0 + u, L - 1) : t0 + u;
                const double hk = s_hd[t];
                const double Jp = u == 0 ? Jprev : Jc[u - 1];
// ... 32 lines not shown
                        if (ACC) rstore(rI, voT, 0, IcT + acc);
                        if (SAVED) rstore(rS, voT, 0, acc);
                    }
                } else if (MODE == 2 && wl && nfx > 0) {
#pragma unroll
                    for (int u = 0; u < TC; ++u) {
                        double acc = 0;
#pragma unroll
                        for (int k = 0; k < kFixMaxSrc; ++k) acc = fix_acc(c[k], readlane_f64(v[u], sl[k]), acc);
                        v[u] = fixlane ? acc : v[u];
                    }
                }
                if (valid && !(tfix && fixlane)) {
#pragma unroll
                    for (int u = 0; u < TC; ++u) {
                        const int so = (t0 + u) * RB;
                        rstore(rIn, vo, so, v[u]);
                        if (ACC) rstore(rI, vo, so, Ic[u] + v[u]);
                        if (SAVED) rstore(rS, vo, so, v[u]);
                    }
                }
            } else {
#pragma unroll
                for (int u = 0; u < TC; ++u) {
                    const int t = t0 + u;
                    if (wl) { const int zs = zr.starts(t); if (zs) load_fix(zs); }
                    const double Dn = rec_step(Dv, Ec[u], cc[u]);
                    double x = has_small ? rec_add(Dn, Sc[u]) : Dn;
                    if (wl && nfx > 0) {
                        double acc = 0;
#pragma unroll
                        for (int k = 0; k < kFixMaxSrc; ++k) acc = fix_acc(c[k], readlane_f64(x, sl[k]), acc);
                        x = fixlane ? acc : x;
                    }
                    v[u] = x;
                    const bool zone_end = zr.ends(t);
                    Dv = t < L ? (zone_end ? (stdl ? x : 0.0) : Dn) : Dv;
                    if (valid && t < L) {
                        const int so = t * RB;
                        rstore(rIn, vo, so, x);
                        if (ACC) rstore(rI, vo, so, Ic[u] + x);
                        if (SAVED) rstore(rS, vo, so, x);
                    }
                }
            }
            if (SP && t0 + TC >= L) {
#pragma unroll
                for (int u = 0; u < TC; ++u)
                    if (t0 + u == L - 1) { sfc_own = v[u]; rdn_v = v[u]; rdn_i = Ic[u] + v[u]; }
            }
            Jprev = Jc[TC - 1];
            t0 += TC;
        };
        auto chunk = [&](auto special_t, auto mode_t) __attribute__((always_inline)) {
            const double* sp = ring + (size_t)slot_rd * SLOT + tid;
            slot_rd = slot_rd + 1 == NS ? 0 : slot_rd + 1;
            double Jc[TC], Ic[TC], Ec[TC];
#pragma unroll
            for (int u = 0; u < TC; ++u) {
                Jc[u] = sp[(0 * TC + u) * RS];
                Ec[u] = sp[(1 * TC + u) * RS];
                Ic[u] = ACC ? sp[(2 * TC + u) * RS] : 0.0;
            }
            process(special_t, mode_t, sp - tid, Jc, Ic, Ec);
            wg_barrier();
        };
        using M0 = std::integral_constant<int, 0>;
        using M1 = std::integral_constant<int, 1>;
        using M2 = std::integral_constant<int, 2>;
        while (q < NCH) {
            const int qe = q + plain_run(sp_dn, q);
            const int mode = (!wl || (nfx == 0 && !has_small)) ? 0 : ((!has_small && nfx <= 8 && sl[0] >= xb_dn) ? 1 : 2);
            if (mode == 0) for (; q < qe; ++q) chunk(std::false_type{}, M0{});
            else if (mode == 1) for (; q < qe; ++q) chunk(std::false_type{}, M1{});
            else for (; q < qe; ++q) chunk(std::false_type{}, M2{});
            if (q < NCH) { chunk(std::true_type{}, M2{}); ++q; }
        }
    }

    stamp(2);
    if (surface != SOSRT_SURFACE_NONE) {
        if (valid) s_sfc[tid] = sfc_own;
        wg_barrier();
    }
    if (surface == SOSRT_SURFACE_SPECULAR) {
        Bv = valid ? rho * s_sfc[N - 1 - tid] : 0.0;
    } else if (surface == SOSRT_SURFACE_LAMBERTIAN || surface == SOSRT_SURFACE_LAMBERTIAN_README) {
        double term = 0;
        if (tid <= N - 3) {
            const int k0 = N - 2 - tid, k1 = k0 - 1;
            const double x0 = g.mu[k0], x1 = g.mu[k1];
            term = (x1 - x0) * (s_sfc[k1] * x1 + s_sfc[k0] * x0) / 2;
        }
        double ws = wave_sum_(term);
        wg_barrier();
        if (lane == 0) s_red[tid >> 6] = ws;
        wg_barrier();
        double S = 0;
        for (int i = 0; i < nwc; ++i) S += s_red[i];
        Bv = (surface == SOSRT_SURFACE_LAMBERTIAN_README ? 2 : -2) * rho * S;
    }

    stamp(3);
    {
        const int mj = N + tidc;
        const int vo = mj * 8;
        const bool tr = valid && tid > 0;
        const double mu = mu_up;
        const double prmu = tr ? 1.0 / mu : 0.0;
        const int last_cand = min(N - 3, 61);
        bool notfound = false;
        double U = Bv, Jnext = 0;
        auto blend = [&](double x, int t) {
            const double x1 = lane_up1(x), x2 = lane_up1(x1);
            const bool stop = lane >= 1 && lane <= last_cand && !(fabs((x - x1) - (x1 - x2)) > 0.0001);
            const unsigned long long mk = __ballot(stop);
            const int kf = mk ? __ffsll((long long)mk) : 1;
            if (mk == 0) {
                notfound = true;
                if (N - 3 > 61 && lane == 0) {
                    if (zr.starts(t)) s_flag[0] = 1;
                    else { flag_row(s_nf, t); s_flag[2] = 1; }
                }
            }
            const double r0 = readlane_f64(x, 0), rk = readlane_f64(x, kf);
            const double w = blend_weight(mu, readlane_f64(prmu, kf));
            const double bl = blend_val(w, r0, rk);
            return (tr && tid < kf) ? bl : x;
        };
// ... 47 lines not shown
                            const int voT = (t0 - uT) * RB + (N + k) * 8;
                            rstore(rIn, voT, 0, val);
                            if (ACC) rstore(rI, voT, 0, IcT + val);
                            if (SAVED) rstore(rS, voT, 0, val);
                        }
                    } else {
#pragma unroll
                        for (int u = 0; u < TC; ++u) {
                            const double xb_ = blend(v[u], t0 - u);
                            if (valid) {
                                const int so = (t0 - u) * RB;
                                rstore(rIn, vo, so, xb_);
                                if (ACC) rstore(rI, vo, so, Ic[u] + xb_);
                                if (SAVED) rstore(rS, vo, so, xb_);
                            }
                        }
                    }
                }
                if (valid && (MODE == 0 || (tblend && !(tid >= 1 && tid <= 8)))) {
#pragma unroll
                    for (int u = 0; u < TC; ++u) {
                        const int so = (t0 - u) * RB;
                        rstore(rIn, vo, so, v[u]);
                        if (ACC) rstore(rI, vo, so, Ic[u] + v[u]);
                        if (SAVED) rstore(rS, vo, so, v[u]);
                    }
                }
            } else {
#pragma unroll
                for (int u = 0; u < TC; ++u) {
                    const int t = t0 - u;
                    const double Un = rec_step(U, Ec[u], cc[u]);
                    double x = Un;
                    if (w0 && t >= 0) x = blend(tid == 0 ? Jc[u] : Un, t);
                    v[u] = x;
                    const bool zone_start = zr.starts(t) != 0;
                    U = t >= 0 ? ((zone_start && tr) ? x : Un) : U;
                    if (valid && t >= 0) {
                        const int so = t * RB;
                        rstore(rIn, vo, so, x);
                        if (ACC) rstore(rI, vo, so, Ic[u] + x);
                        if (SAVED) rstore(rS, vo, so, x);
                    }
                }
            }
            if (SP && t0 - TC < 0) {
#pragma unroll
                for (int u = 0; u < TC; ++u)
                    if (t0 - u == 0) { rup_v = v[u]; rup_i = Ic[u] + v[u]; }
            }
            Jnext = Jc[TC - 1];
            t0 -= TC;
        };
        auto chunk = [&](auto special_t, auto mode_t) __attribute__((always_inline)) {
            const double* sp = ring + (size_t)slot_rd * SLOT + tid;
            slot_rd = slot_rd + 1 == NS ? 0 : slot_rd + 1;
            double Jc[TC], Ic[TC], Ec[TC];
#pragma unroll
            for (int u = 0; u < TC; ++u) {
                Jc[u] = sp[(0 * TC + u) * RS];
                Ec[u] = sp[(1 * TC + u) * RS];
                Ic[u] = ACC ? sp[(2 * TC + u) * RS] : 0.0;
            }
            process(special_t, mode_t, sp - tid, Jc, Ic, Ec);
            wg_barrier();
        };
        using M0 = std::integral_constant<int, 0>;
        using M1 = std::integral_constant<int, 1>;
        while (q < NQ) {
            const int qe = q + plain_run(sp_up, q - NCH);
            if (!w0) for (; q < qe; ++q) chunk(std::false_type{}, M0{});
            else for (; q < qe; ++q) chunk(std::false_type{}, M1{});
            if (q < NQ) { chunk(std::true_type{}, M1{}); ++q; }
        }
        if (w0 && notfound && lane == 0 && N - 3 <= 61) s_flag[1] = 1;
    }
    }
    stamp(4);
    __syncthreads();
    stamp(5);
    if (s_flag[1]) {
        if (tid == 0) {
            a.cv.status[b] = SOSRT_COL_INDEXERROR;
            if (ACC) { a.cv.active[b] = 0; a.cv.norders[b] = a.order; atomicSub(a.cv.nactive, 1); }
        }
        return;
    }
    if (!s_flag[0] && s_flag[2]) {
        if (finish_flagged_rows<ACC, SAVED>(s_nf, L, N, RB, g.mu, rIn, rI, rS, ring, rup_v, rup_i)) {
            if (tid == 0) {
                a.cv.status[b] = SOSRT_COL_INDEXERROR;
                if (ACC) { a.cv.active[b] = 0; a.cv.norders[b] = a.order; atomicSub(a.cv.nactive, 1); }
            }
            return;
        }
    }
    if (s_flag[0]) {
        const bool missing = redo_upward_sweep<ACC, SAVED, MZ>(L, N, RB, zr, s_hd, g.mu, rJ, rE, rIn, rI, rS, Bv, ring,
                                                            rup_v, rup_i);
        if (missing) {
            if (tid == 0) {
                a.cv.status[b] = SOSRT_COL_INDEXERROR;
                if (ACC) { a.cv.active[b] = 0; a.cv.norders[b] = a.order; atomicSub(a.cv.nactive, 1); }
            }
            return;
        }
    }
    if (ACC) {
        const double ra = block_pymax_(rup_v / rup_i, valid, s_red, 0);
        const double rb = block_pymax_(rdn_v / rdn_i, valid, s_red, 0);
        const double r = (rb > ra) ? rb : ra;
        if (tid == 0) {
            a.cv.ratio[b] = r;
            a.cv.norders[b] = a.order;
            if (!conv_go(a.cv, b, a.order, r)) {
                a.cv.active[b] = 0;
                atomicSub(a.cv.nactive, 1);
            }
        }
    } else if (tid == 0 && a.cv.status) {
        a.cv.status[b] = SOSRT_COL_OK;
    }
}

inline int ring_fixcap(const Grid& g) { return (int)(0.06 * g.N) + 1; }
inline size_t ring_extra_doubles(const Grid& g, int nt, int nzcap = kRingZones) {
    const int rs = g.N <= 128 ? 128 : 256, fc = nzcap * ring_fixcap(g) * kFixMaxSrc;
    return (size_t)(rs > fc ? rs : fc) + nt / 64 + 2 + g.L + 1 + (size_t)g.nsmall * g.L + TC * 16 + 16 + (g.L + 63) / 64;
}

template <int PIECES>
void launch_p(hipStream_t s, dim3 grid, dim3 block, const TransportArgs& a, int NS) {
    const int nt = (int)block.x;
    const int narr = a.accumulate ? 3 : 2;
    const size_t shm = ((size_t)NS * narr * TC * 128 * PIECES + ring_extra_doubles(a.g, nt, a.nzcap)) * sizeof(double);
#define SOSRT_RING_LAUNCH_Z(ACC_, SAVED_, MZ_)                                                                 \
    do {                                                                                                       \
        auto kern = k_transport_ring<ACC_, SAVED_, PIECES, MZ_>;                                               \
        static PerDeviceOnce big_lds;                                                                                 \
        if (big_lds.first()) {                                                                                        \
            hipFuncSetAttribute(reinterpret_cast<const void*>(kern), hipFuncAttributeMaxDynamicSharedMemorySize, \
                                (int)kRingLdsBytes);                                                                   \
        }                                                                                                      \
        hipLaunchKernelGGL(kern, grid, block, shm, s, a, NS, g_ring_debug, ring_fixcap(a.g));                           \
    } while (0)
#define SOSRT_RING_LAUNCH(ACC_, SAVED_)                                                                        \
    do {                                                                                                       \
        if (a.nzcap > kRingZones) SOSRT_RING_LAUNCH_Z(ACC_, SAVED_, true);                                     \
        else SOSRT_RING_LAUNCH_Z(ACC_, SAVED_, false);                                                         \
    } while (0)
    if (a.accumulate) {
        if (a.saved) SOSRT_RING_LAUNCH(true, true);
        else SOSRT_RING_LAUNCH(true, false);
    } else {
        SOSRT_RING_LAUNCH(false, false);
    }
#undef SOSRT_RING_LAUNCH
#undef SOSRT_RING_LAUNCH_Z
}

}

bool transport_ring_ok(const Grid& g) {
    if (g.N % 2 || g.N < 4 || g.N > 256) return false;
    const int nwc = (g.N + 63) / 64, pieces = g.N <= 128 ? 1 : 2;
    const size_t slot_bytes = (size_t)3 * TC * 128 * pieces * sizeof(double);
    if (flagged_rows_work_doubles(g.L, g.N) * sizeof(double) > 2 * slot_bytes * 2 / 3) return false;
    return 2 * slot_bytes + ring_extra_doubles(g, (nwc + 4) * 64) * sizeof(double) <= kRingLdsBytes;
}

bool transport_ring_fits(const Grid& g, int nzcap) {
    if (!transport_ring_ok(g)) return false;
    const int nwc = (g.N + 63) / 64, pieces = g.N <= 128 ? 1 : 2;
    const size_t slot_bytes = (size_t)3 * TC * 128 * pieces * sizeof(double);
    return 2 * slot_bytes + ring_extra_doubles(g, (nwc + 4) * 64, nzcap < kRingZones ? kRingZones : nzcap) * sizeof(double) <= kRingLdsBytes;
}

void launch_transport_ring(hipStream_t s, dim3 grid, const TransportArgs& a, int slots) {
    if (a.slots > 0) slots = a.slots;
    const int N = a.g.N;
    const int nwc = (N + 63) / 64;
    const int pieces = N <= 128 ? 1 : 2;
    const int narr = a.accumulate ? 3 : 2;
    const dim3 block((nwc + 2) * 64);
    const size_t slot_bytes = (size_t)narr * TC * 128 * pieces * sizeof(double);
    const size_t extra = ring_extra_doubles(a.g, (int)block.x, a.nzcap) * sizeof(double);
    int NS = slots < 2 ? 2 : slots;
    while (NS > 2 && NS * slot_bytes + extra > kRingLdsBytes) --NS;
    if (pieces == 1) launch_p<1>(s, grid, block, a, NS);
    else launch_p<2>(s, grid, block, a, NS);
}

}
```

### sos-radiative-transfer_amd/csrc/transport_scan.hip

```cpp
#include "transport_scan_body.hpp"

namespace sosrt {

namespace {

template <bool ACC, bool SAVED, bool SPLIT, int NC = 0, bool MZ = false, bool WIDE = false>
__global__ __launch_bounds__(768) void k_transport_scan(TransportArgs a, int fixcap) {
    const int nparts = SPLIT ? ((NC ? NC : a.g.N) + 63) >> 6 : 1;
    const int part = SPLIT ? (int)(blockIdx.x % nparts) : 0;
    int b = SPLIT ? (int)(blockIdx.x / nparts) : (int)blockIdx.x;
    if (ACC && a.live > 0) {
        b = a.live_list[b];
        if (b < 0) return;
    } else if (ACC && !a.cv.active[b]) {
        return;
    }
    (void)transport_scan_order<ACC, SAVED, SPLIT, NC, MZ, false, WIDE>(a, fixcap, b, part, ScanFused());
}

inline bool scan_wide(const Grid& g) { return (g.N & 1) || g.N > 256 || (g.L + TC - 1) / TC > 64; }

void launch_scan_wide(hipStream_t s, dim3 grid, const TransportArgs& a) {
    using C = ScanCfg<true, true>;
    const dim3 block((C::SW + NLOAD) * 64);
    const size_t shm = scan_lds_bytes<true, true>(a.g, a.nzcap);
#define SOSRT_SCAN_LAUNCH_W(SAVED_, MZ_)                                                                       \
    do {                                                                                                       \
        auto kern = k_transport_scan<true, SAVED_, true, 0, MZ_, true>;                                        \
        static PerDeviceOnce big_lds;                                                                                 \
        if (big_lds.first()) {                                                                                        \
            hipFuncSetAttribute(reinterpret_cast<const void*>(kern), hipFuncAttributeMaxDynamicSharedMemorySize, \
                                (int)kScanLdsBytes);                                                           \
        }                                                                                                      \
        hipLaunchKernelGGL(kern, grid, block, shm, s, a, scan_fixcap(a.g));                                    \
    } while (0)
    const bool mz = a.nzcap > kRingZones;
    if (a.saved && mz) SOSRT_SCAN_LAUNCH_W(true, true);
    else if (a.saved) SOSRT_SCAN_LAUNCH_W(true, false);
    else if (mz) SOSRT_SCAN_LAUNCH_W(false, true);
    else SOSRT_SCAN_LAUNCH_W(false, false);
#undef SOSRT_SCAN_LAUNCH_W
}

template <bool SPLIT>
void launch_scan_t(hipStream_t s, dim3 grid, const TransportArgs& a) {
    using C = ScanCfg<SPLIT>;
    const int nwc = SPLIT ? 1 : (a.g.N + 63) / 64;
    const dim3 block((nwc * C::SW + NLOAD) * 64);
    const size_t shm = scan_lds_bytes<SPLIT>(a.g, a.nzcap);
#define SOSRT_SCAN_LAUNCH_Z(ACC_, SAVED_, NC_, MZ_)                                                            \
    do {                                                                                                       \
        auto kern = k_transport_scan<ACC_, SAVED_, SPLIT, NC_, MZ_>;                                           \
        static PerDeviceOnce big_lds;                                                                                 \
        if (big_lds.first()) {                                                                                        \
            hipFuncSetAttribute(reinterpret_cast<const void*>(kern), hipFuncAttributeMaxDynamicSharedMemorySize, \
                                (int)kScanLdsBytes);                                                           \
        }                                                                                                      \
        hipLaunchKernelGGL(kern, grid, block, shm, s, a, scan_fixcap(a.g));                                    \
    } while (0)
#define SOSRT_SCAN_LAUNCH_N(ACC_, SAVED_, NC_) SOSRT_SCAN_LAUNCH_Z(ACC_, SAVED_, NC_, false)
#define SOSRT_SCAN_LAUNCH(ACC_, SAVED_)                                                                        \
    do {                                                                                                       \
        if (a.nzcap > kRingZones) SOSRT_SCAN_LAUNCH_Z(ACC_, SAVED_, 0, true);                                  \
        else SOSRT_SCAN_LAUNCH_Z(ACC_, SAVED_, 0, false);                                                      \
    } while (0)
    static const bool kFixN = !(getenv("SOSRT_SCAN_NC") && atoi(getenv("SOSRT_SCAN_NC")) == 0);
    if (a.accumulate) {
        if (a.saved) SOSRT_SCAN_LAUNCH(true, true);
        else if (SPLIT && kFixN && a.nzcap <= kRingZones && a.g.N == 128) SOSRT_SCAN_LAUNCH_N(true, false, SPLIT ? 128 : 0);
        else if (SPLIT && kFixN && a.nzcap <= kRingZones && a.g.N == 256) SOSRT_SCAN_LAUNCH_N(true, false, SPLIT ? 256 : 0);
        else SOSRT_SCAN_LAUNCH(true, false);
    } else {
        SOSRT_SCAN_LAUNCH(false, false);
    }
#undef SOSRT_SCAN_LAUNCH
#undef SOSRT_SCAN_LAUNCH_N
#undef SOSRT_SCAN_LAUNCH_Z
}

}

bool transport_scan_ok(const Grid& g) {
    if (g.N % 2 || g.N < 4 || g.N > 128) return false;
    if ((g.L + TC - 1) / TC > 64) return false;
    return scan_lds_bytes<false>(g) <= kScanLdsBytes;
}
bool transport_scan_split_ok(const Grid& g) {
    if (g.N <= 64 || g.N > kScanDirs) return false;
    if (scan_wide(g)) return (g.L + TC - 1) / TC <= kScanChunks && scan_lds_bytes<true, true>(g) <= kScanLdsBytes;
    return scan_lds_bytes<true>(g) <= kScanLdsBytes;
}
int transport_scan_parts(const Grid& g) { return (g.N + 63) / 64; }
bool transport_scan_fits(const Grid& g, int nzcap, bool split) {
    if (split && scan_wide(g)) return scan_lds_bytes<true, true>(g, nzcap) <= kScanLdsBytes;
    return (split ? scan_lds_bytes<true>(g, nzcap) : scan_lds_bytes<false>(g, nzcap)) <= kScanLdsBytes;
}
size_t transport_scan_scratch_doubles() { return kScanScratch; }

void launch_transport_scan(hipStream_t s, dim3 grid, const TransportArgs& a) {
    if (a.scan_split && a.accumulate && scan_wide(a.g)) launch_scan_wide(s, dim3(transport_scan_parts(a.g) * grid.x), a);
    else if (a.scan_split && a.accumulate) launch_scan_t<true>(s, dim3(transport_scan_parts(a.g) * grid.x), a);
    else launch_scan_t<false>(s, grid, a);
}

}
```

### sos-radiative-transfer_amd/csrc/transport_scan_body.hpp

```cpp
#pragma once
#include <cstdlib>
#include <type_traits>

#include "../../include/sosrt.h"
#include "kernels.hpp"
#include "transport_util.hpp"

namespace sosrt {

namespace {


template <bool SPLIT, bool WIDE = false> struct ScanCfg {
    static constexpr int SW = SPLIT ? 8 : 4;
    static constexpr int NST = SPLIT ? (WIDE ? 10 : 12) : 6;
    static constexpr int SROW = SPLIT ? 64 : 128;
    static constexpr int STAGE = (2 * TC + 1) * SROW;
};
constexpr int NLOAD = 4;
constexpr int CR = 16;
constexpr int kScanDirs = 512;
constexpr int kScanChunks = 128;
constexpr int kScanScratch = 5 * kScanDirs + 16;
static_assert(kScanChunks * TC / 32 <= 32, "the flagged-row mask of the split form's exchange holds 32 ints: 128 chunks of TC rows");
constexpr size_t kScanLdsBytes = 152 * 1024;
typedef __attribute__((address_space(3))) void* lds_ptr_t;
constexpr unsigned kSpinLimit = 1u << 20;
constexpr unsigned kFusedSpinLimit = 1u << 21;
struct ScanFused {
    int k = 1;
    int first = 1;
    int last = 0;
    const int* jn_done = nullptr;
    int jn_need = 0;
    int* ord_done = nullptr;
    int* col_stop = nullptr;
    int* abort = nullptr;
    int* orders = nullptr;
    unsigned long long* log = nullptr;
    int wg = 0;
};
#ifdef SOSRT_OL_STAMPS
__device__ __forceinline__ void ol_stamp(unsigned long long* log, int wg, int k, int ev) {
    if (!log) return;
    const unsigned long long i = __hip_atomic_fetch_add(log, 1ull, __ATOMIC_RELAXED, __HIP_MEMORY_SCOPE_AGENT);
    if (i < 65000) log[1 + i] = ((unsigned long long)(wg & 0xffff) << 48) | ((unsigned long long)(k & 0xff) << 40) | ((unsigned long long)(ev & 0xff) << 32) |
                                (unsigned long long)(wall_clock64() & 0xffffffffull);
}
#define SOSRT_OL_STAMP(log_, wg_, k_, ev_) ol_stamp(log_, wg_, k_, ev_)
#else
#define SOSRT_OL_STAMP(log_, wg_, k_, ev_)
#endif
__device__ __forceinline__ bool fused_wait_ge(const int* p, int want, int* abort) {
    for (unsigned it = 0;; ++it) {
        if (__hip_atomic_load(p, __ATOMIC_RELAXED, __HIP_MEMORY_SCOPE_AGENT) >= want) return true;
        if ((it & 63) == 63 && __hip_atomic_load(abort, __ATOMIC_RELAXED, __HIP_MEMORY_SCOPE_AGENT)) return false;
        if (it > kFusedSpinLimit) { __hip_atomic_store(abort, 1, __ATOMIC_RELAXED, __HIP_MEMORY_SCOPE_AGENT); return false; }
        __builtin_amdgcn_s_sleep(8);
    }
}

template <bool ACC, bool SAVED, bool SPLIT, int NC = 0, bool MZ = false, bool FUSED = false, bool WIDE = false>
__device__ __forceinline__ int transport_scan_order(const TransportArgs& a, int fixcap, const int b, const int part, const ScanFused& fu) {
    static_assert(!WIDE || (SPLIT && !FUSED && NC == 0), "WIDE is an instantiation of the plain split form");
    using Cfg = ScanCfg<SPLIT, WIDE>;
    constexpr int SW = Cfg::SW, NST = Cfg::NST, SROW = Cfg::SROW, STAGE = Cfg::STAGE;
    const int nparts = SPLIT ? ((NC ? NC : a.g.N) + 63) >> 6 : 1;
    constexpr int LDX = FUSED ? 16 : 0, STX = FUSED ? 17 : 0;
    const Grid& g = a.g;
    int tid_ = threadIdx.x;
    if (FUSED) asm volatile("" : "+v"(tid_));
    const int tid = tid_, lane = tid & 63;
    const int wid = __builtin_amdgcn_readfirstlane(tid) >> 6;
    const int L = g.L, N = NC ? NC : g.N, D = 2 * N;
    if (NC) fixcap = (int)(0.06 * NC) + 1;
    const int nwc = SPLIT ? 1 : (N + 63) >> 6;
    const int ND = ((N + 63) >> 6) * 64;
    const int ncw = nwc * SW;
    const bool loader = wid >= ncw;
    const int lg = wid % nwc, grp = loader ? wid - ncw : wid / nwc;
    const int dir = SPLIT ? part * 64 + lane : lg * 64 + lane;
    const int dn0 = SPLIT ? max(N - 64 * (part + 1), 0) : 0;
    const int dir_dn = SPLIT ? dn0 + lane : dir;
    const bool valid = dir < N;
    const bool valid_dn = SPLIT ? dir_dn < N - 64 * part : valid;
    const int dirc = valid ? dir : N - 1;
    const int dirc_dn = valid_dn ? dir_dn : 0;
    const bool w0 = !loader && (SPLIT ? part == 0 : lg == 0);
    const bool wl = !loader && (SPLIT ? part == 0 : lg == ((N - 1) >> 6));
    const int lane_last = SPLIT ? 63 : ((N - 1) & 63);
    const int dn_base = SPLIT ? N - 64 : (((N - 1) >> 6) << 6);
    const int nwaves = blockDim.x >> 6;
    const int NCH = (L + TC - 1) / TC;

#ifdef SOSRT_SCAN_STAMPS
    unsigned long long t_wait = 0, t_stage = 0, t_pre = 0, t_post = 0, t_c = 0;
    auto stamp = [&](int i) __attribute__((always_inline)) {
        if (a.stamps && lane == 0 && part == 0 && (wid == 0 || wid == ncw - 1))
            a.stamps[((size_t)b * 2 + (wid == 0 ? 0 : 1)) * 16 + i] = i == 6 ? t_wait : (i == 7 ? t_stage : (i == 8 ? t_pre : (i == 9 ? t_post : clock64())));
    };
#define SCAN_T0() t_c = clock64()
#define SCAN_T1() t_pre += clock64() - t_c
#define SCAN_T2() t_c = clock64()
#define SCAN_T3() t_post += clock64() - t_c
#define SCAN_CB(gq_)
#elif defined(SOSRT_SCAN_CHAIN)
    auto stamp = [](int) {};
    int cgq = 0;
#define SCAN_C(k_) do { if (a.stamps && lane == 0) a.stamps[(size_t)b * 4096 + (part * 128 + cgq) * 5 + (k_)] = clock64(); } while (0)
#define SCAN_CB(gq_) do { cgq = (gq_); SCAN_C(0); } while (0)
#define SCAN_T0() SCAN_C(1)
#define SCAN_T1() SCAN_C(2)
#define SCAN_T2() SCAN_C(3)
#define SCAN_T3() SCAN_C(4)
#else
    auto stamp = [](int) {};
#define SCAN_T0()
#define SCAN_T1()
#define SCAN_T2()
#define SCAN_T3()
#define SCAN_CB(gq_)
#endif
    stamp(0);
    extern __shared__ double sm[];
    double* s_stage = sm;
    double* s_carry = s_stage + (size_t)NST * STAGE;
    double* s_sfc = s_carry + (size_t)nwc * CR * 64;
    double* s_fixc = s_sfc + ND;
    double* s_red = s_fixc + (MZ ? a.nzcap : kRingZones) * fixcap * kFixMaxSrc;
    double* s_hd = s_red + nwaves + 2;
    double* s_S = s_hd + L + 1;
    double* s_prmu = s_S + (WIDE ? 0 : (size_t)g.nsmall * L);
    double* s_conv = s_prmu + 16;
    double* s_xw = s_conv + 4 * ND;
    int* s_flagq = reinterpret_cast<int*>(s_xw + (size_t)ncw * 2 * TC * 16);
    int* s_landed = s_flagq + nwc * CR;
    int* s_taken = s_landed + NST;
    int* s_nf = s_taken + NST * nwc;
    int* s_nfz = s_nf + (L + 31) / 32;
    __shared__ int s_flag[4];
    double* s_x = s_xw + (size_t)(loader ? 0 : wid) * 2 * TC * 16;
    double* s_xI = s_x + TC * 16;
    const int xb_dn = max(lane_last - 15, 0);

    const ColDesc* __restrict__ dg = a.desc + b;
    const int nz = dg->nz;
    const ZoneRows<MZ> zr(dg);
    const int nfix0 = dg->nfix[0], nfix1 = dg->nfix[1], nfix2 = dg->nfix[2];
    const int surface = dg->surface;
    const double rho = dg->rho;
    const int fbytes = L * D * 8, RB = D * 8;
    const __amdgpu_buffer_rsrc_t rJ = make_rsrc(a.Jn + (size_t)b * L * D, fbytes);
    const __amdgpu_buffer_rsrc_t rE = make_rsrc(a.Etab + (size_t)(a.erep ? a.erep[b] : b) * L * D, fbytes);
    const __amdgpu_buffer_rsrc_t rIn = make_rsrc(a.In + (size_t)b * L * D, fbytes);
    const __amdgpu_buffer_rsrc_t rI = make_rsrc(ACC ? a.I + (size_t)b * L * D : a.In, ACC ? fbytes : 0);
    (void)rJ; (void)rE;
    const __amdgpu_buffer_rsrc_t rS = make_rsrc(SAVED ? a.saved + (size_t)b * a.saved_col_stride : a.In, SAVED ? fbytes : 0);

    unsigned long long sp_dn = 0, sp_up = 0, sp_dn1 = 0, sp_up1 = 0;
    if (!WIDE) {
        sp_dn = sp_up = 1ull << (NCH - 1);
        sp_dn |= zr.boundary_chunks(L, TC, false);
        sp_up |= zr.boundary_chunks(L, TC, true);
    } else {
        sp_dn = zr.boundary_chunks(L, TC, false, 0); sp_dn1 = zr.boundary_chunks(L, TC, false, 1);
        sp_up = zr.boundary_chunks(L, TC, true, 0); sp_up1 = zr.boundary_chunks(L, TC, true, 1);
        if (NCH - 1 < 64) { sp_dn |= 1ull << (NCH - 1); sp_up |= 1ull << (NCH - 1); }
        else { sp_dn1 |= 1ull << (NCH - 1 - 64); sp_up1 |= 1ull << (NCH - 1 - 64); }
    }
    auto special_dn = [&](int q) __attribute__((always_inline)) { return WIDE ? (((q < 64 ? sp_dn : sp_dn1) >> (q & 63)) & 1) != 0 : ((sp_dn >> q) & 1) != 0; };
    auto special_up = [&](int j) __attribute__((always_inline)) { return WIDE ? (((j < 64 ? sp_up : sp_up1) >> (j & 63)) & 1) != 0 : ((sp_up >> j) & 1) != 0; };


    typedef __attribute__((address_space(3))) volatile int lds_vint;
    typedef __attribute__((address_space(3))) volatile double lds_vdouble;
    lds_vint* const l_flagq = (lds_vint*)(s_flagq + lg * CR);
    lds_vdouble* const l_carry = (lds_vdouble*)(s_carry + (size_t)lg * CR * 64 + lane);
    lds_vint* const l_landed = (lds_vint*)s_landed;
    lds_vint* const l_taken = (lds_vint*)s_taken;
    auto spin = [&](lds_vint* f, int want) __attribute__((always_inline)) {
#ifdef SOSRT_SCAN_STAMPS
        const unsigned long long w0_ = clock64();
#endif
        unsigned it = 0;
        while (*f != want) {
            __builtin_amdgcn_s_sleep(1);
            if (++it > kSpinLimit) { s_flag[2] = 1; break; }
        }
#ifdef SOSRT_SCAN_STAMPS
        t_wait += clock64() - w0_;
#endif
    };
    auto wait_carry = [&](int cs) __attribute__((always_inline)) -> double {
        spin(l_flagq + (cs & (CR - 1)), cs);
        return l_carry[(cs & (CR - 1)) * 64];
    };
    auto publish = [&](int cs, double val) __attribute__((always_inline)) {
        l_carry[(cs & (CR - 1)) * 64] = val;
        if (lane == 0) l_flagq[cs & (CR - 1)] = cs;
    };
    auto take = [&](auto clamp_t, int gq, int vo_, int so0, int dso, double (&J)[TC], double (&E)[TC], double (&I)[TC], double& Jx) __attribute__((always_inline)) {
        constexpr bool CLAMP = decltype(clamp_t)::value;
        const int stg = gq % NST;
#ifdef SOSRT_SCAN_STAMPS
        const unsigned long long tw_ = t_wait;
#endif
        spin(l_landed + stg, gq + 1);
#ifdef SOSRT_SCAN_STAMPS
        t_stage += t_wait - tw_; t_wait = tw_;
#endif
        typedef __attribute__((address_space(3))) double lds_double;
        const lds_double* st = (const lds_double*)(s_stage + (size_t)stg * STAGE + (SPLIT ? lane : (gq < NCH ? dirc_dn : dirc)));
        asm volatile("" ::: "memory");
#pragma unroll
        for (int u = 0; u < TC; ++u) {
            J[u] = st[(0 * TC + u) * SROW];
            E[u] = st[(1 * TC + u) * SROW];
        }
        Jx = st[(2 * TC) * SROW];
        asm volatile("" ::: "memory");
        if (lane == 0) l_taken[stg * nwc + lg] = gq + 1;
#pragma unroll
        for (int u = 0; u < TC; ++u) I[u] = ACC ? bload_aux<LDX>(rI, vo_, CLAMP ? min(max(so0 + u * dso, 0), (L - 1) * RB) : so0 + u * dso) : 0.0;
    };

    auto issue = [&](int gq) __attribute__((always_inline)) {
        const bool up = gq >= NCH;
        const int q = up ? gq - NCH : gq;
        double* dst = s_stage + (size_t)(gq % NST) * STAGE;
        const int t0 = up ? L - 1 - q * TC : q * TC;
        const int half = SPLIT ? (up ? N * 8 + part * 512 : dn0 * 8) : (up ? N * 8 : 0);
        if (WIDE && (N & 1)) {
            const int v4 = lane * 4;
#pragma unroll
            for (int u = 0; u < TC; ++u) {
                const int row = up ? max(t0 - u, 0) : min(t0 + u, L - 1);
                const int so = row * RB + half;
                __builtin_amdgcn_raw_ptr_buffer_load_lds(rJ, (lds_ptr_t)(dst + (0 * TC + u) * SROW), 4, v4, so, 0, LDX);
                __builtin_amdgcn_raw_ptr_buffer_load_lds(rJ, (lds_ptr_t)(dst + (0 * TC + u) * SROW + 32), 4, v4, so + 256, 0, LDX);
                __builtin_amdgcn_raw_ptr_buffer_load_lds(rE, (lds_ptr_t)(dst + (1 * TC + u) * SROW), 4, v4, so, 0, 0);
                __builtin_amdgcn_raw_ptr_buffer_load_lds(rE, (lds_ptr_t)(dst + (1 * TC + u) * SROW + 32), 4, v4, so + 256, 0, 0);
            }
            const int rx = up ? min(t0 + 1, L - 1) : max(t0 - 1, 0);
            __builtin_amdgcn_raw_ptr_buffer_load_lds(rJ, (lds_ptr_t)(dst + (2 * TC) * SROW), 4, v4, rx * RB + half, 0, LDX);
            __builtin_amdgcn_raw_ptr_buffer_load_lds(rJ, (lds_ptr_t)(dst + (2 * TC) * SROW + 32), 4, v4, rx * RB + half + 256, 0, LDX);
        } else if (SPLIT) {
            const int hl = lane >> 5, vl = (lane & 31) * 16;
#pragma unroll
            for (int u = 0; u < TC; u += 2) {
                const int uu = u + hl;
                const int row = up ? max(t0 - uu, 0) : min(t0 + uu, L - 1);
                const int vo = vl + row * RB;
                __builtin_amdgcn_raw_ptr_buffer_load_lds(rJ, (lds_ptr_t)(dst + (0 * TC + u) * SROW), 16, vo, half, 0, LDX);
                __builtin_amdgcn_raw_ptr_buffer_load_lds(rE, (lds_ptr_t)(dst + (1 * TC + u) * SROW), 16, vo, half, 0, 0);
            }
            const int rx = up ? min(t0 + 1, L - 1) : max(t0 - 1, 0);
            if (lane < 32) __builtin_amdgcn_raw_ptr_buffer_load_lds(rJ, (lds_ptr_t)(dst + (2 * TC) * SROW), 16, vl, rx * RB + half, 0, LDX);
        } else {
            const int vo = lane * 16;
#pragma unroll
            for (int u = 0; u < TC; ++u) {
                const int row = up ? max(t0 - u, 0) : min(t0 + u, L - 1);
                const int so = row * RB + half;
                __builtin_amdgcn_raw_ptr_buffer_load_lds(rJ, (lds_ptr_t)(dst + (0 * TC + u) * SROW), 16, vo, so, 0, LDX);
                __builtin_amdgcn_raw_ptr_buffer_load_lds(rE, (lds_ptr_t)(dst + (1 * TC + u) * SROW), 16, vo, so, 0, 0);
            }
            const int rx = up ? min(t0 + 1, L - 1) : max(t0 - 1, 0);
            __builtin_amdgcn_raw_ptr_buffer_load_lds(rJ, (lds_ptr_t)(dst + (2 * TC) * SROW), 16, vo, rx * RB + half, 0, LDX);
        }
    };
    auto load_chunks = [&](int g0, int g1, bool first_issued) __attribute__((always_inline)) {
        for (int gq = g0; gq < g1; gq += NLOAD) {
            if (gq >= NST)
                for (int i = 0; i < nwc; ++i) spin(l_taken + (gq % NST) * nwc + i, gq - NST + 1);
            if (!(first_issued && gq == g0)) issue(gq);
            asm volatile("s_waitcnt vmcnt(0)" ::: "memory");
            if (lane == 0) l_landed[gq % NST] = gq + 1;
        }
    };
    const int g_seam = min(NCH + NST, 2 * NCH);
    int g_next = grp;

    const double mu_up = (valid && dir > 0) ? g.mu[N + dirc] : 1.0;
    const int uT = lane >> 3, pT = lane & 7;
    const double muT = (pT + 1 < N) ? g.mu[N + pT + 1] : 1.0;
    const double* xrow = s_x + uT * 16;
    double Bv = 0;

    if (!FUSED && loader && g_next < g_seam) issue(g_next);
    {
        const int nt = blockDim.x;
        if (!FUSED || fu.first) {
            for (int zz = 0; zz < (MZ ? nz : kRingZones); ++zz) {
                const FixTab& src = g.fix[dg->fixtab[zz]];
                for (int i = tid; i < fixcap * kFixMaxSrc; i += nt) s_fixc[zz * fixcap * kFixMaxSrc + i] = src.C[i];
            }
            if (tid < kMaxZones) s_nfz[tid] = tid < nz ? dg->nfix[tid] : 0;
            const double* __restrict__ tau = a.tau + (size_t)b * L;
            for (int t = tid; t <= L; t += nt) s_hd[t] = (t == 0 || t == L) ? 0.0 : (tau[t] - tau[t - 1]) * 0.5;
            if (tid < 16) s_prmu[tid] = (tid > 0 && tid < N) ? 1.0 / g.mu[N + tid] : 0.0;
        }
        if (tid < 4) s_flag[tid] = 0;
        for (int i = tid; i < nwc * CR + NST + NST * nwc + (L + 31) / 32; i += nt) s_flagq[i] = 0;
        if (!FUSED && !WIDE) {
            const double* __restrict__ In0 = a.In + (size_t)b * L * D;
            for (int i = tid; i < g.nsmall * L; i += nt) {
                const int k = i / L, t = i - k * L;
                s_S[i] = In0[(size_t)t * D + g.small_lanes[k]];
            }
        }
    }
    __syncthreads();
    stamp(1);
    if (FUSED && loader) {
        if (!fused_wait_ge(fu.jn_done, fu.jn_need, fu.abort) && lane == 0) s_flag[2] = 1;
        if (FUSED && wid == ncw && lane == 0) SOSRT_OL_STAMP(fu.log, fu.wg, fu.k, 2);
    }

    if (loader) {
        load_chunks(g_next, g_seam, !FUSED);
        while (g_next < g_seam) g_next += NLOAD;
    } else {
        const int m = dirc_dn;
        const int vo = m * 8;
        const bool valid = valid_dn;
        const double mu = g.mu[m];
        const bool tr = valid && m <= N - 2;
        const bool small = tr && fabs(mu) < kMuThreshold;
        const bool stdl = tr && !small;
        const double nrmu = stdl ? -1.0 / mu : 0.0;
        const bool has_small = wl && g.nsmall > 0;
        const int sbase = small ? (m - g.small_lanes[0]) * L : 0;
        const int lmT = lane_last - pT;
        auto zone_of = [&](int t) __attribute__((always_inline)) { return zr.of(t); };
        const int nfix_packed = nfix0 | (nfix1 << 10) | (nfix2 << 20);
        auto nfix_of = [&](int zz) __attribute__((always_inline)) { if constexpr (MZ) { if (zz > 2) return s_nfz[min(zz, kMaxZones - 1)]; }
            return (nfix_packed >> (10 * zz)) & 1023; };
        auto chunk = [&](auto special_t, auto mode_t, int q) __attribute__((always_inline)) {
            constexpr bool SP = decltype(special_t)::value;
            constexpr int MODE = decltype(mode_t)::value;
            const int t0 = q * TC;
            double Jc[TC], Ec[TC], Ic[TC], Jx_;
            SCAN_CB(q);
            take(special_t, q, vo, t0 * RB, RB, Jc, Ec, Ic, Jx_);
            SCAN_T0();
            const double Jprev = q > 0 ? Jx_ : 0.0;
            double c[kFixMaxSrc] = {0, 0, 0, 0, 0};
            double cT[kFixMaxSrc] = {0, 0, 0, 0, 0};
            int sl[kFixMaxSrc] = {0, 0, 0, 0, 0};
            int nfx = 0;
            bool fixlane = false;
            auto load_fix = [&](int zz) __attribute__((always_inline)) {
                const double* ftC = s_fixc + zz * fixcap * kFixMaxSrc;
// ... 511 lines not shown
                    const bool ok = fused_wait_ge(fu.ord_done, fu.k, fu.abort);
                    s_verdict = (!ok || __hip_atomic_load(fu.col_stop, __ATOMIC_RELAXED, __HIP_MEMORY_SCOPE_AGENT)) ? 1 : 0;
                }
                __syncthreads();
                return s_verdict;
            }
            return 0;
        }
        if (tid == 0) {
            const int f = __hip_atomic_exchange(sync + 1, 0, __ATOMIC_RELAXED, __HIP_MEMORY_SCOPE_AGENT);
            s_flag[0] = f & 1; s_flag[1] = (f >> 1) & 1; s_flag[2] = (f >> 2) & 1; s_flag[3] = (f >> 3) & 1;
            __hip_atomic_store(sync, 0, __ATOMIC_RELAXED, __HIP_MEMORY_SCOPE_AGENT);
        }
        __syncthreads();
        if (s_flag[0] || s_flag[3]) __atomic_thread_fence(__ATOMIC_ACQUIRE);
        if (s_flag[3] && tid < (L + 31) / 32) s_nf[tid] = __hip_atomic_load(gnf + tid, __ATOMIC_RELAXED, __HIP_MEMORY_SCOPE_AGENT);
        for (int i = tid; i < N; i += blockDim.x) {
#pragma unroll
            for (int k = 0; k < 4; ++k) s_conv[k * ND + i] = __hip_atomic_load(gs + k * kScanDirs + i, __ATOMIC_RELAXED, __HIP_MEMORY_SCOPE_AGENT);
            s_sfc[i] = __hip_atomic_load(gs + 4 * kScanDirs + i, __ATOMIC_RELAXED, __HIP_MEMORY_SCOPE_AGENT);
        }
        __syncthreads();
    }
    if (s_flag[2]) {
        if (tid == 0) {
            a.cv.status[b] = SOSRT_COL_INTERNAL;
            if (ACC) { a.cv.active[b] = 0; a.cv.norders[b] = a.order; atomicSub(a.cv.nactive, 1); }
        }
        return leave(1);
    }
    if (s_flag[1]) {
        if (tid == 0) {
            a.cv.status[b] = SOSRT_COL_INDEXERROR;
            if (ACC) { a.cv.active[b] = 0; a.cv.norders[b] = a.order; atomicSub(a.cv.nactive, 1); }
        }
        return leave(1);
    }
    const bool act = tid < N;
    double rup_v = act ? s_conv[2 * ND + tid] : 0.0, rup_i = act ? s_conv[3 * ND + tid] : 1.0;
    const double rdn_v = act ? s_conv[0 * ND + tid] : 0.0, rdn_i = act ? s_conv[1 * ND + tid] : 1.0;
    if (!s_flag[0] && s_flag[3]) {
        __syncthreads();
        if (finish_flagged_rows<ACC, SAVED, LDX, STX>(s_nf, L, N, RB, g.mu, rIn, rI, rS, s_stage, rup_v, rup_i)) {
            if (tid == 0) {
                a.cv.status[b] = SOSRT_COL_INDEXERROR;
                if (ACC) { a.cv.active[b] = 0; a.cv.norders[b] = a.order; atomicSub(a.cv.nactive, 1); }
            }
            return leave(1);
        }
    }
    if (s_flag[0]) {
        const double U0 = SPLIT ? ((act && surface == SOSRT_SURFACE_SPECULAR) ? rho * s_sfc[N - 1 - tid] : 0.0) : Bv;
        __syncthreads();
        const bool missing = redo_upward_sweep<ACC, SAVED, MZ, LDX, STX>(L, N, RB, zr, s_hd, g.mu, rJ, rE, rIn, rI, rS, U0,
                                                            s_stage, rup_v, rup_i);
        if (missing) {
            if (tid == 0) {
                a.cv.status[b] = SOSRT_COL_INDEXERROR;
                if (ACC) { a.cv.active[b] = 0; a.cv.norders[b] = a.order; atomicSub(a.cv.nactive, 1); }
            }
            return leave(1);
        }
    }
    if (ACC) {
        const double ra = block_pymax_(rup_v / rup_i, act, s_red, 0);
        const double rb = block_pymax_(rdn_v / rdn_i, act, s_red, 0);
        const double r = (rb > ra) ? rb : ra;
        if (tid == 0) {
            a.cv.ratio[b] = r;
            a.cv.norders[b] = a.order;
            if (!conv_go(a.cv, b, a.order, r)) {
                a.cv.active[b] = 0;
                atomicSub(a.cv.nactive, 1);
            }
        }
        return leave(!conv_go(a.cv, b, a.order, r) ? 1 : 0);
    } else if (tid == 0 && a.cv.status) {
        a.cv.status[b] = SOSRT_COL_OK;
    }
    return leave(1);
}

inline int scan_fixcap(const Grid& g) { return (int)(0.06 * g.N) + 1; }
template <bool SPLIT, bool WIDE = false>
inline size_t scan_lds_bytes(const Grid& g, int nzcap = kRingZones) {
    using C = ScanCfg<SPLIT, WIDE>;
    const int nwc = SPLIT ? 1 : (g.N + 63) / 64, ncw = nwc * C::SW, nwaves = ncw + NLOAD, ND = (g.N + 63) / 64 * 64;
    const size_t doubles = (size_t)C::NST * C::STAGE + (size_t)nwc * CR * 64 + ND + (size_t)nzcap * scan_fixcap(g) * kFixMaxSrc + nwaves + 2 +
                           g.L + 1 + (WIDE ? 0 : (size_t)g.nsmall * g.L) + 16 + 4 * ND + (size_t)ncw * 2 * TC * 16;
    return doubles * sizeof(double) + ((size_t)(nwc * CR + C::NST + C::NST * nwc + (g.L + 31) / 32 + kMaxZones) * sizeof(int) + 7) / 8 * 8;
}

}
}
```

### sos-radiative-transfer_amd/csrc/transport_util.hpp

```cpp
#pragma once
#include <hip/hip_runtime.h>

#include "kernels.hpp"

namespace sosrt {
namespace {

__device__ __forceinline__ double readlane_f64(double v, int srclane) {
    int lo = __double2loint(v), hi = __double2hiint(v);
    lo = __builtin_amdgcn_readlane(lo, srclane);
    hi = __builtin_amdgcn_readlane(hi, srclane);
    return __hiloint2double(hi, lo);
}

typedef unsigned int u32x2 __attribute__((ext_vector_type(2)));

__device__ __forceinline__ __amdgpu_buffer_rsrc_t make_rsrc(const void* p, int bytes) {
    return __builtin_amdgcn_make_buffer_rsrc(const_cast<void*>(p), 0, bytes, 0x00020000);
}
__device__ __forceinline__ double bload(__amdgpu_buffer_rsrc_t r, int voff, int soff) {
    const u32x2 v = __builtin_amdgcn_raw_buffer_load_b64(r, voff, soff, 0);
    return __hiloint2double((int)v.y, (int)v.x);
}
__device__ __forceinline__ double bload_glc(__amdgpu_buffer_rsrc_t r, int voff, int soff) {
// ... 34 lines not shown
    v.x = (unsigned)__double2loint(x.x); v.y = (unsigned)__double2hiint(x.x);
    v.z = (unsigned)__double2loint(x.y); v.w = (unsigned)__double2hiint(x.y);
    __builtin_amdgcn_raw_buffer_store_b128(v, r, voff, soff, 0);
}
template <int AUX>
__device__ __forceinline__ void bstore2_aux(__amdgpu_buffer_rsrc_t r, int voff, int soff, double2 x) {
    u32x4 v;
    v.x = (unsigned)__double2loint(x.x); v.y = (unsigned)__double2hiint(x.x);
    v.z = (unsigned)__double2loint(x.y); v.w = (unsigned)__double2hiint(x.y);
    __builtin_amdgcn_raw_buffer_store_b128(v, r, voff, soff, AUX);
}

__device__ __forceinline__ double lane_up1(double v) {
    int lo = __double2loint(v), hi = __double2hiint(v);
    lo = __builtin_amdgcn_update_dpp(lo, lo, 0x130, 0xf, 0xf, false);
    hi = __builtin_amdgcn_update_dpp(hi, hi, 0x130, 0xf, 0xf, false);
    return __hiloint2double(hi, lo);
}

__device__ __forceinline__ double wave_fmax_(double v) {
#pragma unroll
    for (int o = 32; o > 0; o >>= 1) v = fmax(v, __shfl_xor(v, o, 64));
    return v;
}
__device__ __forceinline__ double wave_sum_(double v) {
#pragma unroll
    for (int o = 32; o > 0; o >>= 1) v += __shfl_xor(v, o, 64);
    return v;
}

__device__ __forceinline__ double rec_src(double h_rmu, double Ja, double E, double Jb) {
#pragma clang fp contract(off)
    return h_rmu * __builtin_fma(Ja, E, Jb);
}
__device__ __forceinline__ double rec_hr(double h, double rmu) {
#pragma clang fp contract(off)
    return h * rmu;
}
__device__ __forceinline__ double rec_step(double S, double E, double c) { return __builtin_fma(S, E, c); }
__device__ __forceinline__ double rec_add(double a, double b) {
#pragma clang fp contract(off)
    return a + b;
}
__device__ __forceinline__ double blend_weight(double mu_m, double rmu_k) {
#pragma clang fp contract(off)
    return mu_m * rmu_k;
}
__device__ __forceinline__ double blend_val(double w, double r0, double rk) {
#pragma clang fp contract(off)
    const double a = (1 - w) * r0;
    return __builtin_fma(w, rk, a);
}
__device__ __forceinline__ double fix_acc(double c, double x, double acc) { return __builtin_fma(c, x, acc); }

template <bool MZ> struct ZoneRows {
    const ColDesc* dg;
    int nz, zend0, zend1, zbeg1, zbeg2;
    int zb[MZ ? kMaxZones : 1];
    __device__ __forceinline__ explicit ZoneRows(const ColDesc* d) : dg(d) {
        nz = d->nz;
        zend0 = nz > 1 ? d->r1[0] : -9; zend1 = nz > 2 ? d->r1[1] : -9;
        zbeg1 = nz > 1 ? d->r0[1] : -9; zbeg2 = nz > 2 ? d->r0[2] : -9;
        if constexpr (MZ) {
#pragma unroll
            for (int k = 3; k < kMaxZones; ++k) zb[k] = k < nz ? d->r0[k] : -99;
        }
    }
    __device__ __forceinline__ bool ends(int t) const {
        bool e = t == zend0 || t == zend1;
        if constexpr (MZ) {
#pragma unroll
            for (int k = 3; k < kMaxZones; ++k) e = e || t == zb[k] - 1;
        }
        return e;
    }
    __device__ __forceinline__ int starts(int t) const {
        int z = t == zbeg1 ? 1 : (t == zbeg2 ? 2 : 0);
        if constexpr (MZ) {
#pragma unroll
            for (int k = 3; k < kMaxZones; ++k) z = t == zb[k] ? k : z;
        }
        return z;
    }
    __device__ __forceinline__ int of(int t) const {
        int z = (zbeg2 >= 0 && t >= zbeg2) ? 2 : ((zbeg1 >= 0 && t >= zbeg1) ? 1 : 0);
        if constexpr (MZ) {
#pragma unroll
            for (int k = 3; k < kMaxZones; ++k) z = (zb[k] >= 0 && t >= zb[k]) ? k : z;
        }
        return z;
    }
    __device__ __forceinline__ int nfix(int zz) const { return dg->nfix[zz]; }
    __device__ __forceinline__ unsigned long long boundary_chunks(int L, int tc, bool up, int word) const {
        unsigned long long m = 0;
        if constexpr (!MZ) {
            const int rows[4] = {zend0, zend1, zbeg1, zbeg2};
#pragma unroll
            for (int i = 0; i < 4; ++i) {
                const int c = (up ? L - 1 - rows[i] : rows[i]) / tc;
                if (rows[i] >= 0 && (c >> 6) == word) m |= 1ull << (c & 63);
            }
        } else {
            for (int k = 1; k < nz; ++k) {
                const int rb = dg->r0[k], re = rb - 1;
                const int cb = (up ? L - 1 - rb : rb) / tc, ce = (up ? L - 1 - re : re) / tc;
                if ((cb >> 6) == word) m |= 1ull << (cb & 63);
// ... 45 lines not shown
    __syncthreads();
    const int cnt = *s_cnt;
    const bool act = tid < N, tr = act && tid > 0;
    const int j = act ? tid : 0;
    const double mu = tr ? gmu[N + j] : 1.0;
    const int vo = (N + j) * 8;
    bool missing = false;
    for (int c0 = 0; c0 < cnt; c0 += kNfBatch) {
        const int nb = min(kNfBatch, cnt - c0);
        double xo[kNfBatch], Io[kNfBatch];
#pragma unroll
        for (int i = 0; i < kNfBatch; ++i) {
            const int t = s_list[c0 + min(i, nb - 1)];
            xo[i] = bload_aux<LDX ? LDX : 1>(rIn, vo, t * RB);
            Io[i] = ACC ? bload_aux<LDX ? LDX : 1>(rI, vo, t * RB) : 0.0;
        }
#pragma unroll
        for (int i = 0; i < kNfBatch; ++i)
            if (act) s_rows[i * NP + j] = xo[i];
        if (tid < kNfBatch) s_kf[tid] = 1 << 30;
        __syncthreads();
#pragma unroll
        for (int i = 0; i < kNfBatch; ++i) {
            const double* r = s_rows + i * NP;
            if (i < nb && act && j >= 1 && j <= N - 3 && !(fabs((r[j] - r[j + 1]) - (r[j + 1] - r[j + 2])) > 0.0001)) atomicMin(&s_kf[i], j);
        }
        __syncthreads();
#pragma unroll
        for (int i = 0; i < kNfBatch; ++i) {
            if (i >= nb) continue;
            const double* r = s_rows + i * NP;
            const int ks = s_kf[i];
            missing |= ks == (1 << 30);
            const int kf = ks == (1 << 30) ? 1 : ks + 1;
            const int t = s_list[c0 + i];
            if (tr && tid < kf) {
                const double x = blend_val(blend_weight(mu, 1.0 / gmu[N + kf]), r[0], r[kf]);
                bstore_aux<STX>(rIn, vo, t * RB, x);
                double It = 0;
                if (ACC) {
                    It = Io[i] + (x - xo[i]);
                    bstore_aux<STX>(rI, vo, t * RB, It);
                }
                if (SAVED) bstore_aux<STX>(rS, vo, t * RB, x);
                if (t == 0) { rup_v = x; rup_i = It; }
            }
        }
        __syncthreads();
    }
    return missing;
}

constexpr int kRedoRows = 8;
template <bool ACC, bool SAVED, bool MZ, int LDX = 0, int STX = 0>
__device__ SOSRT_HELPER_INLINE bool redo_upward_sweep(int L, int N, int RB, const ZoneRows<MZ>& zr, const double* s_hd,
                                  const double* __restrict__ gmu, __amdgpu_buffer_rsrc_t rJ, __amdgpu_buffer_rsrc_t rE,
                                  __amdgpu_buffer_rsrc_t rIn, __amdgpu_buffer_rsrc_t rI, __amdgpu_buffer_rsrc_t rS, double U0,
                                  double* s_work, double& rup_v, double& rup_i) {
    const int tid = threadIdx.x;
    double* s_row = s_work;
    int* s_kf = reinterpret_cast<int*>(s_work + 2 * (N + 2));
    const bool act = tid < N, tr = act && tid > 0;
    const int j = act ? tid : 0;
    const double mu = tr ? gmu[N + j] : 1.0;
    const double prmu = tr ? 1.0 / mu : 0.0;
    const int vo = (N + j) * 8;
    double U = U0, Jnext = 0;
    bool missing = false;
    if (tid < 2) s_kf[tid] = 1 << 30;
    __syncthreads();
    int par = 0;
    for (int t0 = L - 1; t0 >= 0; t0 -= kRedoRows) {
        double Jc[kRedoRows], Ec[kRedoRows], xo[kRedoRows], Io[kRedoRows];
#pragma unroll
        for (int u = 0; u < kRedoRows; ++u) {
            const int t = max(t0 - u, 0);
            Jc[u] = bload_aux<LDX>(rJ, vo, t * RB);
            Ec[u] = bload(rE, vo, t * RB);
            xo[u] = bload_aux<LDX ? LDX : 1>(rIn, vo, t * RB);
            Io[u] = ACC ? bload_aux<LDX ? LDX : 1>(rI, vo, t * RB) : 0.0;
        }
#pragma unroll
        for (int u = 0; u < kRedoRows; ++u) {
            const int t = t0 - u;
            if (t < 0) break;
            double* row = s_row + par * (N + 2);
            const double src = rec_src(rec_hr(s_hd[t + 1], prmu), Jnext, Ec[u], Jc[u]);
            const double Un = rec_step(U, Ec[u], zr.ends(t) ? 0.0 : src);
            if (act) row[j] = tid == 0 ? Jc[u] : Un;
            __syncthreads();
            if (act && j >= 1 && j <= N - 3 && !(fabs((row[j] - row[j + 1]) - (row[j + 1] - row[j + 2])) > 0.0001)) atomicMin(&s_kf[par], j);
            if (tid == 0) s_kf[par ^ 1] = 1 << 30;
            __syncthreads();
            const int ks = s_kf[par];
            missing |= ks == (1 << 30);
            const int kf = ks == (1 << 30) ? 1 : ks + 1;
            double x = act ? row[j] : 0.0;
            if (tr && tid < kf) x = blend_val(blend_weight(mu, 1.0 / gmu[N + kf]), row[0], row[kf]);
            const bool zone_start = zr.starts(t) != 0;
            U = (zone_start && tr) ? x : Un;
            Jnext = Jc[u];
            if (act) {
                bstore_aux<STX>(rIn, vo, t * RB, x);
                double It = 0;
                if (ACC) {
                    It = Io[u] + (x - xo[u]);
                    bstore_aux<STX>(rI, vo, t * RB, It);
                }
                if (SAVED) bstore_aux<STX>(rS, vo, t * RB, x);
                if (t == 0) { rup_v = x; rup_i = It; }
            }
            par ^= 1;
        }
    }
    __syncthreads();
    return missing;
}

__device__ __forceinline__ double block_pymax_(double x, bool valid, double* s_red, int first_tid) {
    const int tid = threadIdx.x, nw = blockDim.x >> 6;
    double v = wave_fmax_(valid ? x : __builtin_nan(""));
    __syncthreads();
    if ((tid & 63) == 0) s_red[tid >> 6] = v;
    if (tid == first_tid) s_red[nw] = x;
    __syncthreads();
    double r = s_red[0];
    for (int i = 1; i < nw; ++i) r = fmax(r, s_red[i]);
    const double first = s_red[nw];
    return (first != first) ? first : r;
// ... 5 lines not shown
```

### sos-radiative-transfer_amd/sosrt/_lib.py

```python
import ctypes
import os
from ctypes import POINTER, c_char_p, c_double, c_int, c_longlong, c_void_p

_HERE = os.path.dirname(os.path.abspath(__file__))
LIB_PATH = os.environ.get("SOSRT_LIB") or os.path.join(os.path.dirname(_HERE), "libsosrt.so")

SOSRT_OK, E_INVALID, E_HIP, E_STATE, E_NOMEM = 0, -1, -2, -3, -4
COL_OK, COL_INDEXERROR, COL_MAXORDERS, COL_INTERNAL = 0, 1, 2, 3
GEOM_THREE_ZONE, GEOM_SINGLE_SLAB = 0, 1
SURFACE_NONE, SURFACE_SPECULAR, SURFACE_LAMBERTIAN, SURFACE_LAMBERTIAN_README = 0, 1, 2, 3
K_GEMM, K_TRANSPORT, K_FIRST, K_SMALLMU, K_ORDER_LOOP = 0, 1, 2, 3, 4
PLAN_GEMM_DENSE, PLAN_GEMM_LIVE64, PLAN_GEMM_LIVE32, PLAN_GEMM_LIVE32_DEEP, PLAN_GEMM_LIVE16_REGS = 0, 1, 2, 3, 4
PLAN_TRANSPORT_GENERAL, PLAN_TRANSPORT_FAST, PLAN_TRANSPORT_RING, PLAN_TRANSPORT_SCAN = 0, 1, 3, 4
CONTRACT_F64, CONTRACT_F32, CONTRACT_F64_FULL, CONTRACT_F64_DENSE = 0, 1, 2, 3
FIRST_ORDER_CODED, FIRST_ORDER_README = 0, 1
PHASE_ISO, PHASE_RAYLEIGH, PHASE_HG, PHASE_TABLE = 0, 1, 2, 3
MAX_MODES = 64
MAX_PHASE_SETS = 64

_dp = POINTER(c_double)
_ip = POINTER(c_int)

SIGNATURES = {
    "sosrt_last_error": (c_char_p, []),
    "sosrt_version": (c_int, []),
    "sosrt_create": (c_int, [c_int, c_int, c_int, c_int, c_int, POINTER(c_void_p)]),
    "sosrt_destroy": (c_int, [c_void_p]),
    "sosrt_set_stream": (c_int, [c_void_p, c_void_p]),
    "sosrt_use_own_stream": (c_int, [c_void_p]),
    "sosrt_synchronize": (c_int, [c_void_p]),
    "sosrt_set_saved_orders": (c_int, [c_void_p, c_int]),
    "sosrt_set_order_budget": (c_int, [c_void_p, c_int]),
    "sosrt_set_contraction": (c_int, [c_void_p, c_int]),
    "sosrt_phase_asymmetry": (c_int, [c_void_p, POINTER(c_double), _ip]),
    "sosrt_phase_rank": (c_int, [c_void_p, _ip, POINTER(c_double), _ip]),
    "sosrt_set_order_loop": (c_int, [c_void_p, c_int]),
    "sosrt_order_loop_stats": (c_int, [c_void_p, _ip, _ip, POINTER(c_longlong)]),
    "sosrt_plan_launch": (c_int, [c_void_p, c_int, c_int, c_int, c_int, c_int, _ip]),
    "sosrt_set_first_order": (c_int, [c_void_p, c_int]),
    "sosrt_set_grid": (c_int, [c_void_p, c_void_p]),
    "sosrt_set_phase": (c_int, [c_void_p, c_void_p, c_void_p]),
    "sosrt_set_phase_sets": (c_int, [c_void_p, c_void_p, c_int, c_void_p]),
    "sosrt_set_phase_sets_dev": (c_int, [c_void_p, c_void_p, c_int, c_void_p]),
    "sosrt_phase_matrix_dev": (c_int, [c_void_p, c_int, c_double, c_void_p]),
    "sosrt_set_aerosol_sets": (c_int, [c_void_p, c_int, c_int, c_void_p]),
    "sosrt_phase_sets_info": (c_int, [c_void_p, _ip]),
    "sosrt_set_columns": (c_int, [c_void_p, c_int, c_int, c_int] + [c_void_p] * 9),
    "sosrt_set_columns_zones": (c_int, [c_void_p, c_int, c_int, c_int] + [c_void_p] * 10),
    "sosrt_first_order": (c_int, [c_void_p, c_int, c_void_p, c_void_p, c_void_p, c_void_p]),
    "sosrt_source": (c_int, [c_void_p, c_int, c_void_p, c_void_p]),
    "sosrt_transport": (c_int, [c_void_p, c_int, c_void_p, c_void_p, c_void_p, c_void_p]),
    "sosrt_solve": (c_int, [c_void_p, c_int, c_void_p, c_void_p, c_void_p, c_double, c_void_p, c_void_p, c_void_p, c_void_p, c_void_p]),
    "sosrt_solve_dev": (c_int, [c_void_p, c_int, c_void_p, c_void_p, c_void_p, c_double, c_void_p, c_void_p, c_void_p, c_void_p, c_void_p]),
    "sosrt_last_solve_stats": (c_int, [c_void_p, _ip, POINTER(c_longlong)]),
    "sosrt_fluxes": (c_int, [c_void_p, c_int, c_void_p, c_void_p, c_int, c_void_p, c_void_p]),
    "sosrt_epilogue_dev": (c_int, [c_void_p, c_int, c_void_p, c_void_p, c_int] + [c_void_p] * 6),
    "sosrt_epilogue": (c_int, [c_void_p, c_int, c_int] + [c_void_p] * 6),
    "sosrt_phase_table": (c_int, [c_void_p, c_void_p, c_void_p, c_int]),
    "sosrt_phase_table_dev": (c_int, [c_void_p, c_void_p, c_void_p, c_int]),
    "sosrt_mie_ensembles": (c_int, [c_void_p, c_int] + [c_void_p] * 5 + [c_int, c_double, c_double, c_int, c_void_p, c_void_p]),
    "sosrt_mie_ensembles_dev": (c_int, [c_void_p, c_int] + [c_void_p] * 5 + [c_int, c_double, c_double, c_int, c_void_p, c_void_p]),
    "sosrt_mie_efficiencies": (c_int, [c_void_p, c_int, c_void_p, c_void_p, c_void_p, c_void_p]),
    "sosrt_mie_timing": (c_int, [c_void_p, _dp]),
    "sosrt_phase_p0_dev": (c_int, [c_void_p, c_int, c_int, c_double, c_void_p, c_void_p]),
    "sosrt_phase_p0": (c_int, [c_void_p, c_int, c_int, c_double, c_void_p, c_void_p]),
    "sosrt_phase_matrix": (c_int, [c_void_p, c_int, c_double, c_void_p]),
    "sosrt_phase_modes": (c_int, [c_void_p, c_int, c_double, c_int, c_int, c_int, c_void_p]),
    "sosrt_phase_p0_modes_dev": (c_int, [c_void_p, c_int, c_int, c_double, c_int, c_int, c_int, c_void_p, c_void_p]),
    "sosrt_phase_p0_modes": (c_int, [c_void_p, c_int, c_int, c_double, c_int, c_int, c_int, c_void_p, c_void_p]),
    "sosrt_set_order_targets": (c_int, [c_void_p, c_void_p]),
    "sosrt_azimuth_accumulate_dev": (c_int, [c_void_p, c_int, c_int, c_void_p, c_int, c_void_p, c_int, c_void_p, c_void_p]),
    "sosrt_comm_unique_id": (c_int, [c_void_p]),
    "sosrt_comm_init": (c_int, [c_void_p, c_int, c_int, c_void_p]),
    "sosrt_gather": (c_int, [c_void_p, c_int, c_void_p, c_void_p, c_void_p]),
    "sosrt_comm_destroy": (c_int, [c_void_p]),
    "sosrt_limit_mu_down": (c_int, [c_void_p, c_int, c_int, c_void_p, c_void_p]),
    "sosrt_asymptotic_down": (c_int, [c_void_p, c_int, c_int, c_void_p, c_void_p, c_void_p, c_void_p, c_void_p, c_void_p]),
    "sosrt_plan_weights": (c_int, [c_void_p, c_void_p]),
    "sosrt_plan_fold": (c_int, [c_void_p, c_int, c_void_p]),
    "sosrt_plan_fix_table": (c_int, [c_void_p, c_int, _ip, _ip, c_void_p]),
    "sosrt_plan_fix_count": (c_int, [c_double, c_int]),
    "sosrt_debug_stamps": (c_int, [c_void_p, c_void_p]),
    "sosrt_microbench": (c_int, [c_void_p, c_int, _dp]),
    "sosrt_profile_enable": (c_int, [c_void_p, c_int]),
    "sosrt_profile_reset": (c_int, [c_void_p]),
    "sosrt_profile_get": (c_int, [c_void_p, c_int, _dp, POINTER(c_longlong), _dp]),
}

_lib = None


def _preload_hip_runtime():
    import importlib.util
    try:
        spec = importlib.util.find_spec("torch")
    except (ImportError, ValueError):
        spec = None
    if spec is None or not spec.submodule_search_locations:
        return
    p = os.path.join(list(spec.submodule_search_locations)[0], "lib", "libamdhip64.so")
    if os.path.exists(p):
        try:
            ctypes.CDLL(p, mode=ctypes.RTLD_GLOBAL)
        except OSError:
            pass


def lib():
    global _lib
    if _lib is None:
        if not os.path.exists(LIB_PATH):
            raise ImportError(
                "libsosrt.so not found at %s: build it with `python __graft_entry__.py build` "
                "(hipcc --offload-arch=gfx950); there is no CPU fallback" % LIB_PATH)
        _preload_hip_runtime()
        L = ctypes.CDLL(LIB_PATH)
        for name, (res, args) in SIGNATURES.items():
            fn = getattr(L, name)
            fn.restype = res
            fn.argtypes = args
        _lib = L
    return _lib


class SosrtError(RuntimeError):
    pass


def check(rc):
    if rc == SOSRT_OK:
        return
    msg = lib().sosrt_last_error().decode()
    if rc == E_INVALID:
        raise ValueError(msg)
    if rc == E_NOMEM:
        raise MemoryError(msg)
    raise SosrtError(msg)
```

### sos-radiative-transfer_amd/sosrt/solver.py

```python
from __future__ import annotations

import ctypes
from dataclasses import dataclass
from typing import Optional

import numpy as np

from . import _lib
from ._lib import check, lib


def _f64(a, shape=None, name="array"):
    a = np.ascontiguousarray(a, dtype=np.float64)
    if shape is not None and a.shape != tuple(shape):
        raise ValueError("%s has shape %s, expected %s" % (name, a.shape, tuple(shape)))
    return a


def _i32(a, n, name):
    a = np.ascontiguousarray(a, dtype=np.int32)
    if a.shape != (n,):
        raise ValueError("%s has shape %s, expected (%d,)" % (name, a.shape, n))
    return a

# ... 381 lines not shown

    def gather_device(self, root: int, counts, d_send: int, d_recv: int):
        c = np.ascontiguousarray(counts, dtype=np.int64)
        check(lib().sosrt_gather(self._h, int(root), _ptr(c), ctypes.c_void_p(d_send) if d_send else None,
                                 ctypes.c_void_p(d_recv) if d_recv else None))

    def comm_destroy(self):
        check(lib().sosrt_comm_destroy(self._h))

    def limit_mu_down(self, rows, idx):
        rows = np.ascontiguousarray(rows, dtype=np.float64)
        if rows.ndim != 2 or rows.shape[1] != self.N:
            raise ValueError("rows must be [R, nb_angles]")
        out = np.empty((rows.shape[0], idx))
        if idx:
            check(lib().sosrt_limit_mu_down(self._h, rows.shape[0], int(idx), _ptr(rows), _ptr(out)))
        return out

    def asymptotic_down(self, J, tau, lens, tau_t, mu):
        J = np.ascontiguousarray(J, dtype=np.float64)
        tau = _f64(tau, J.shape, "tau")
        R, stride = J.shape
        lens = _i32(lens, R, "len")
        tt = _f64(tau_t, (R,), "tau_t")
        m = _f64(mu, (R,), "mu")
        out = np.empty(R)
        check(lib().sosrt_asymptotic_down(self._h, R, stride, _ptr(lens), _ptr(J), _ptr(tau), _ptr(tt), _ptr(m), _ptr(out)))
        return out

    def plan_weights(self):
        w = np.empty(self.D)
        check(lib().sosrt_plan_weights(self._h, _ptr(w)))
        return w

    def plan_fold(self, which=0):
        W = np.empty((self.D, self.D))
        check(lib().sosrt_plan_fold(self._h, which, _ptr(W)))
        return W

    def plan_fix_table(self, idx):
        s0, ns = ctypes.c_int(), ctypes.c_int()
        C = np.zeros((max(idx, 1), 5))
        check(lib().sosrt_plan_fix_table(self._h, int(idx), ctypes.byref(s0), ctypes.byref(ns), _ptr(C)))
        return s0.value, ns.value, C.reshape(-1)[: idx * ns.value].reshape(idx, ns.value).copy()

    def plan_launch(self, batch, live, surface="specular", zones=3, cus=0):
        sf = {"none": _lib.SURFACE_NONE, "specular": _lib.SURFACE_SPECULAR, "lambertian": _lib.SURFACE_LAMBERTIAN,
              "lambertian_readme": _lib.SURFACE_LAMBERTIAN_README}[surface]
        out = (ctypes.c_int * 9)()
        check(lib().sosrt_plan_launch(self._h, int(batch), int(live), sf, int(zones), int(cus), out))
        keys = ("groups", "gemm", "tail_cols", "transport", "parts", "repair", "order_loop", "ol_parts", "ol_grid")
        return dict(zip(keys, list(out)))

    def microbench(self, which):
        r = ctypes.c_double()
        check(lib().sosrt_microbench(self._h, int(which), ctypes.byref(r)))
        return r.value

    def profile_enable(self, on=True):
        check(lib().sosrt_profile_enable(self._h, 1 if on else 0))

    def profile_reset(self):
        check(lib().sosrt_profile_reset(self._h))

    def profile_get(self, kernel):
        ms, cnt, w = ctypes.c_double(), ctypes.c_longlong(), ctypes.c_double()
        check(lib().sosrt_profile_get(self._h, kernel, ctypes.byref(ms), ctypes.byref(cnt), ctypes.byref(w)))
        return ms.value, cnt.value


def fix_count(tau_ref: float, nb_angles: int) -> int:
    return lib().sosrt_plan_fix_count(float(tau_ref), int(nb_angles))
```

Measured before the change: 123,700.

## Pass low-rank Jn moments to transport instead of materializing full source rows

When the phase matrix is low-rank (rank ≤ 2), the source GEMM now writes a few per-row moment coefficients instead of the full D-wide Jn row. The ring and scan transport kernels rebuild Jn on the fly from those moments and the lrV vectors for rows in non-mixed zones. Mixed-zone rows still load the full Jn. This is meant to cut global memory traffic for writing and reading Jn each order, at the cost of extra arithmetic, more template variants and extra planning conditions. The path is on by default and can be disabled with SOSRT_JN_MOMENTS.

```diff
diff --git a/include/sosrt.h b/include/sosrt.h
--- a/include/sosrt.h
+++ b/include/sosrt.h
@@ -154,6 +154,9 @@
 #define SOSRT_PLAN_TRANSPORT_RING    3
 #define SOSRT_PLAN_TRANSPORT_SCAN    4
 int sosrt_plan_launch(sosrt_t* h, int batch, int live, int surface, int zones, int cus, int* out );
+#define SOSRT_PLAN_NEED_SMALL 1
+#define SOSRT_PLAN_SAVING     2
+int sosrt_plan_launch2(sosrt_t* h, int batch, int live, int surface, int zones, int cus, int flags, int* out );
 
 #define SOSRT_K_GEMM      0
 #define SOSRT_K_TRANSPORT 1
diff --git a/sos-radiative-transfer_amd/csrc/api.hip b/sos-radiative-transfer_amd/csrc/api.hip
--- a/sos-radiative-transfer_amd/csrc/api.hip
+++ b/sos-radiative-transfer_amd/csrc/api.hip
@@ -138,6 +138,8 @@
     int lr_rank = -1;
     double lr_residual = 0;
     double *d_lrU = nullptr, *d_lrV = nullptr;
+    double* d_mom = nullptr;
+    bool jn_moments = true;
     size_t mixs_capacity = 0;
     float *d_Wa32 = nullptr, *d_Wmix32 = nullptr;
     size_t mix32_capacity = 0;
@@ -422,7 +424,7 @@
 }
 
 void run_source(sosrt_handle* h, const double* In_1, double* Jn, const int* active, int tail_cols = 0, int pub_tag = 0,
-                int grp = -1, bool all_live = false, bool regs_tile = false, int dense_live_cap = 0) {
+                int grp = -1, bool all_live = false, bool regs_tile = false, int dense_live_cap = 0, bool moments = false) {
     const int g0 = grp < 0 ? 0 : grp, g1 = grp < 0 ? h->ngroups : grp + 1;
     const int pg = grp < 0 ? 0 : grp;
     hipStream_t s = group_stream(h, pg);
@@ -457,6 +459,7 @@
         ga.Wr = h->d_Wrsets; ga.mix_group = h->d_mixgroup; ga.slab_tile_group = h->d_slabtilegroup + h->slab_off[g0] / 32;
     }
     if (use_lowrank(h)) { ga.lr_rank = h->lr_rank; ga.lrU = h->d_lrU; ga.lrV = h->d_lrV; }
+    if (moments && use_lowrank(h)) ga.mom = h->d_mom;
     if (use_sym(h)) {
         ga.sym = 1; ga.Ks = (h->g.N + GEMM_KC - 1) / GEMM_KC * GEMM_KC;
 #ifdef SOSRT_DIAG
@@ -530,6 +533,7 @@
     int order_loop = 0;
     int ol_parts = 0;
     int ol_grid = 0;
+    int jn_moments = 0;
 };
 LaunchPlan plan_order(const sosrt_handle* h, const SolveShape& sh, const OrderInputs& in) {
     LaunchPlan pl;
@@ -576,6 +580,10 @@
         }
         if (pl.order_loop) pl.ol_grid = in.cu_share;
     }
+    const bool expands = pl.transport == SOSRT_PLAN_TRANSPORT_RING ||
+                         (pl.transport == SOSRT_PLAN_TRANSPORT_SCAN && transport_scan_moments_ok(g, sh.nzcap, pl.parts > 1));
+    pl.jn_moments = (h->jn_moments && use_lowrank(h) && h->lr_rank >= 1 && h->lr_rank <= kMomRankMax &&
+                     expands && !pl.order_loop && !pl.repair && !in.need_small) ? 1 : 0;
     return pl;
 }
 
@@ -649,6 +657,7 @@
     if (const char* ev = getenv("SOSRT_GEMM_KS_MULT")) h->diag_ks_mult = atoi(ev);
 #endif
     if (const char* ev = getenv("SOSRT_GROUP_RING_SLOTS")) h->coresident_slots = atoi(ev);
+    if (const char* ev = getenv("SOSRT_JN_MOMENTS")) h->jn_moments = atoi(ev) != 0;
     if (const char* ev = getenv("SOSRT_ORDER_LOOP")) h->order_loop = atoi(ev) != 0;
     if (const char* ev = getenv("SOSRT_RING_SLOTS")) g_ring_slots = atoi(ev);
 #ifdef SOSRT_RING_DEBUG
@@ -672,6 +681,7 @@
             if ((e = dalloc(&h->d_Wr, (size_t)g.Dp * g.Wld))) return e;
             if ((e = dalloc(&h->d_lrU, (size_t)kLowRankMax * g.D))) return e;
             if ((e = dalloc(&h->d_lrV, (size_t)kLowRankMax * g.D))) return e;
+            if ((e = dalloc(&h->d_mom, mb * L * kMomStride))) return e;
             if ((e = dalloc(&h->d_wfdn, N))) return e;
             if ((e = dalloc(&h->d_wfup, N))) return e;
             if ((e = dalloc(&h->d_w, g.D))) return e;
@@ -751,7 +761,7 @@
                         h->d_idx_down, h->d_scal, h->d_desc, h->d_rca, h->d_rcr, h->d_slabrows, h->d_mainrows, h->d_tau, h->d_P0a,
                         h->d_P0r, h->d_Jn, h->d_InA, h->d_InB, h->d_I, h->d_E, h->d_active, h->d_norders, h->d_status,
                         h->d_nactive_sets, h->d_ratio, h->d_redo, h->d_erep, h->d_tauhash, h->d_Wmix, h->d_mixca, h->d_mixcr,
-                        h->d_mixgroup, h->d_Wa_s, h->d_Wr_s, h->d_Wmix_s, h->d_scan_scratch, h->d_scan_sync, h->d_w, h->d_phi, h->d_z, h->d_tab, h->d_slabtilegroup, h->d_livelist, h->d_Wa32, h->d_Wmix32, h->d_nz, h->d_zr0, h->d_zmix, h->d_zwr, h->d_zdtr, h->d_olsync, h->d_ollog, h->d_modetab, h->d_lrU, h->d_lrV, h->d_Wrsets, h->d_Wrsets_s, h->d_mixset, h->d_P0rz};
+                        h->d_mixgroup, h->d_Wa_s, h->d_Wr_s, h->d_Wmix_s, h->d_scan_scratch, h->d_scan_sync, h->d_w, h->d_phi, h->d_z, h->d_tab, h->d_slabtilegroup, h->d_livelist, h->d_Wa32, h->d_Wmix32, h->d_nz, h->d_zr0, h->d_zmix, h->d_zwr, h->d_zdtr, h->d_olsync, h->d_ollog, h->d_modetab, h->d_lrU, h->d_lrV, h->d_mom, h->d_Wrsets, h->d_Wrsets_s, h->d_mixset, h->d_P0rz};
         for (void* p : ptrs)
             if (p) hipFree(p);
         if (h->h_pub) hipHostFree(h->h_pub);
@@ -852,7 +862,14 @@
     return 0;
 }
 
+static int plan_launch_impl(sosrt_t* h, int batch, int live, int surface, int zones, int cus, int flags, int* out, int nout);
 int sosrt_plan_launch(sosrt_t* h, int batch, int live, int surface, int zones, int cus, int* out) {
+    return plan_launch_impl(h, batch, live, surface, zones, cus, 0, out, 9);
+}
+int sosrt_plan_launch2(sosrt_t* h, int batch, int live, int surface, int zones, int cus, int flags, int* out) {
+    return plan_launch_impl(h, batch, live, surface, zones, cus, flags, out, 10);
+}
+static int plan_launch_impl(sosrt_t* h, int batch, int live, int surface, int zones, int cus, int flags, int* out, int nout) {
     if (!h || !out) return fail(SOSRT_E_INVALID, "null argument");
     if (!h->have_grid) return fail(SOSRT_E_STATE, "sosrt_set_grid has not been called");
     if (batch < 1 || live < 0 || live > batch) return fail(SOSRT_E_INVALID, "need 0 <= live <= batch, batch >= 1");
@@ -868,6 +885,8 @@
     oi.nb = nb; oi.known = live < nb ? live : nb; oi.surface = surface;
     oi.simple_zones = zones == 3 || zones == 1;
     oi.cu_share = h->cu_count / ng;
+    oi.need_small = (flags & SOSRT_PLAN_NEED_SMALL) && h->g.nsmall > 0;
+    oi.saving = (flags & SOSRT_PLAN_SAVING) != 0;
     const bool saved_sym = h->sym_ok;
     if (!h->have_phase) h->sym_ok = true;
     const LaunchPlan pl = plan_order(h, sh, oi);
@@ -875,6 +894,7 @@
     h->cu_count = saved_cus;
     out[0] = ng; out[1] = pl.gemm; out[2] = pl.tail_cols; out[3] = pl.transport; out[4] = pl.parts; out[5] = pl.repair;
     out[6] = pl.order_loop; out[7] = pl.ol_parts; out[8] = pl.ol_grid;
+    if (nout > 9) out[9] = pl.jn_moments;
     return 0;
 }
 
@@ -1753,7 +1773,7 @@
             n_max = n > n_max ? n : n_max;
             const int tail_cols = pl.tail_cols;
             run_source(h, q.In_1, h->d_Jn, h->d_active, tail_cols, tagbase + n - 1, k, q.known == q.nb, pl.gemm == SOSRT_PLAN_GEMM_LIVE16_REGS,
-                       tail_cols > 0 ? 0 : pl.live_cap);
+                       tail_cols > 0 ? 0 : pl.live_cap, pl.jn_moments != 0);
             if (g.nsmall > 0 && h->need_small) {
                 prof_begin(h, SOSRT_K_SMALLMU, k);
                 launch_smallmu(sg, g, q.nb, tau_g, h->d_Jn + fo, q.In + fo, h->d_desc + q.b0, q.cv.active);
@@ -1767,7 +1787,8 @@
                 launch_transport(sg, gt, q.nb, tau_g, h->d_Jn + fo, q.In + fo, d_I_out + fo, sv_n, saved_stride, h->d_desc + q.b0, q.cv, n, 1,
                                  h->d_E, pl.transport, erep_g, pl.live_cap, h->d_livelist + q.b0, NG > 1 ? h->coresident_slots : 0,
                                  pl.parts > 1 ? 1 : 0, h->d_scan_scratch + (size_t)q.b0 * transport_scan_scratch_doubles(),
-                                 h->d_scan_sync + 2 * q.b0, nzcap);
+                                 h->d_scan_sync + 2 * q.b0, nzcap, pl.jn_moments ? h->d_mom + (size_t)q.b0 * h->L * kMomStride : nullptr,
+                                 h->d_lrV, h->lr_rank);
                 if (pl.repair)
                     launch_transport(sg, g, q.nb, tau_g, h->d_Jn + fo, q.In + fo, d_I_out + fo, sv_n, saved_stride, h->d_desc + q.b0, q.cv, n, 1,
                                      h->d_E, 2, erep_g);
diff --git a/sos-radiative-transfer_amd/csrc/jn_gemm_tile.hpp b/sos-radiative-transfer_amd/csrc/jn_gemm_tile.hpp
--- a/sos-radiative-transfer_amd/csrc/jn_gemm_tile.hpp
+++ b/sos-radiative-transfer_amd/csrc/jn_gemm_tile.hpp
@@ -366,7 +366,7 @@
 }
 
 constexpr int LR_ROWS = 4;
-template <bool COH>
+template <bool COH, bool MOM = false>
 __device__ __forceinline__ void lowrank_rows(const GemmArgs& g, const int (&rows)[LR_ROWS], int lane) {
     const int D = g.D, R = g.lr_rank;
     __amdgpu_buffer_rsrc_t rA[LR_ROWS], rC[LR_ROWS];
@@ -408,24 +408,30 @@
 #pragma unroll
                 for (int i = 0; i < LR_ROWS; ++i) m[i][q] += __shfl_xor(m[i][q], s);
             }
+    if constexpr (MOM) {
+#pragma unroll
+        for (int i = 0; i < LR_ROWS; ++i) {
+            double x = cf[i];
+#pragma unroll
+            for (int q = 0; q < kLowRankMax; ++q) x = lane == q ? m[i][q] : x;
+            if (rows[i] >= 0 && lane <= kMomCf) g.mom[(size_t)rows[i] * kMomStride + lane] = x;
+        }
+        return;
+    }
 #pragma unroll 2
     for (int k = 2 * lane; k < D; k += 128) {
-        double2 o[LR_ROWS];
-#pragma unroll
-        for (int i = 0; i < LR_ROWS; ++i) o[i] = make_double2(0.0, 0.0);
+        double vx[kLowRankMax], vy[kLowRankMax];
 #pragma unroll
         for (int q = 0; q < kLowRankMax; ++q) {
+            vx[q] = 0.0; vy[q] = 0.0;
             if (q < R) {
                 const double2 v = *reinterpret_cast<const double2*>(V + (size_t)q * D + k);
-#pragma unroll
-                for (int i = 0; i < LR_ROWS; ++i) {
-                    o[i].x = __builtin_fma(m[i][q], v.x, o[i].x);
-                    o[i].y = __builtin_fma(m[i][q], v.y, o[i].y);
-                }
-            }
-        }
-#pragma unroll
-        for (int i = 0; i < LR_ROWS; ++i) bstore2_aux<COH ? 17 : 0>(rC[i], k * 8, 0, make_double2(cf[i] * o[i].x, cf[i] * o[i].y));
+                vx[q] = v.x; vy[q] = v.y;
+            }
+        }
+#pragma unroll
+        for (int i = 0; i < LR_ROWS; ++i)
+            bstore2_aux<COH ? 17 : 0>(rC[i], k * 8, 0, make_double2(lowrank_expand(m[i], cf[i], vx, R), lowrank_expand(m[i], cf[i], vy, R)));
     }
 }
 template <bool COH, class RowOf>
@@ -449,7 +455,8 @@
 #pragma unroll
             for (int i = 1; i < LR_ROWS; ++i)
                 if (rows[i] >= 0) { rows[0] = rows[i]; rows[i] = -1; break; }
-        lowrank_rows<COH>(g, rows, lane);
+        if (!COH && g.mom) lowrank_rows<COH, true>(g, rows, lane);
+        else lowrank_rows<COH>(g, rows, lane);
     }
 }
 
diff --git a/sos-radiative-transfer_amd/csrc/kernels.hip b/sos-radiative-transfer_amd/csrc/kernels.hip
--- a/sos-radiative-transfer_amd/csrc/kernels.hip
+++ b/sos-radiative-transfer_amd/csrc/kernels.hip
@@ -1033,12 +1033,14 @@
 void launch_transport(hipStream_t s, const Grid& g, int B, const double* tau, const double* Jn, double* In, double* I,
                       double* saved, size_t saved_col_stride, const ColDesc* desc, Conv cv, int order,
                       int accumulate, const double* Etab, int mode, const int* erep, int live, const int* live_list,
-                      int ring_slots, int scan_split, double* scan_scratch, int* scan_sync, int nzcap) {
+                      int ring_slots, int scan_split, double* scan_scratch, int* scan_sync, int nzcap, const double* mom,
+                      const double* lrV, int lr_rank) {
     const int nt = round64(g.N);
     const size_t shm = (size_t)(g.L + 2 * TC * (nt + 2) + 2 * nt + nt / 64 + 2) * sizeof(double);
     TransportArgs a{g, tau, Jn, In, I, accumulate ? saved : nullptr, saved_col_stride, desc, cv, order, accumulate, Etab, Etab ? erep : nullptr, g_transport_stamps};
     a.slots = ring_slots;
     a.nzcap = nzcap > kRingZones ? nzcap : kRingZones;
+    if ((mode == 3 || mode == 4) && accumulate && mom && lrV && lr_rank >= 1 && lr_rank <= kMomRankMax) { a.mom = mom; a.lrV = lrV; a.lr_rank = lr_rank; }
     if (mode == 4 && scan_split && scan_scratch && scan_sync) { a.scan_split = 1; a.scan_scratch = scan_scratch; a.scan_sync = scan_sync; }
     if ((mode == 3 || mode == 4) && accumulate && live > 0 && live < B && live_list) {
         a.live = live;
diff --git a/sos-radiative-transfer_amd/csrc/kernels.hpp b/sos-radiative-transfer_amd/csrc/kernels.hpp
--- a/sos-radiative-transfer_amd/csrc/kernels.hpp
+++ b/sos-radiative-transfer_amd/csrc/kernels.hpp
@@ -111,6 +111,9 @@
     int scan_split = 0;
     double* scan_scratch = nullptr;
     int* scan_sync = nullptr;
+    const double* mom = nullptr;
+    const double* lrV = nullptr;
+    int lr_rank = 0;
 };
 void launch_transport_fast(hipStream_t s, dim3 grid, dim3 block, const TransportArgs& a);
 bool transport_ring_ok(const Grid& g);
@@ -119,6 +122,7 @@
 bool transport_scan_ok(const Grid& g);
 bool transport_scan_split_ok(const Grid& g);
 bool transport_scan_fits(const Grid& g, int nzcap, bool split);
+bool transport_scan_moments_ok(const Grid& g, int nzcap, bool split);
 int transport_scan_parts(const Grid& g);
 size_t transport_scan_scratch_doubles();
 void launch_transport_scan(hipStream_t s, dim3 grid, const TransportArgs& a);
@@ -179,8 +183,12 @@
     int lr_rank = -1;
     const double* lrU = nullptr;
     const double* lrV = nullptr;
+    double* mom = nullptr;
 };
 constexpr int kLowRankMax = 4;
+constexpr int kMomStride = 8;
+constexpr int kMomCf = kLowRankMax;
+constexpr int kMomRankMax = 2;
 
 __device__ inline void publish_live_now(const GemmArgs& g) {
     const int live = __hip_atomic_load(g.nactive, __ATOMIC_RELAXED, __HIP_MEMORY_SCOPE_AGENT);
@@ -238,7 +246,7 @@
                       double* saved, size_t saved_col_stride, const ColDesc* desc, Conv cv, int order, int accumulate,
                       const double* Etab, int mode, const int* erep = nullptr, int live = 0, const int* live_list = nullptr,
                       int ring_slots = 0, int scan_split = 0, double* scan_scratch = nullptr, int* scan_sync = nullptr,
-                      int nzcap = kRingZones);
+                      int nzcap = kRingZones, const double* mom = nullptr, const double* lrV = nullptr, int lr_rank = 0);
 bool transport_fast_ok(const Plan& plan);
 void launch_attenuation(hipStream_t s, const Grid& g, int B, const double* tau, double* Etab, const int* erep);
 void launch_tau_groups(hipStream_t s, const Grid& g, int B, const double* tau, unsigned long long* hash, int* erep,
diff --git a/sos-radiative-transfer_amd/csrc/transport_ring.hip b/sos-radiative-transfer_amd/csrc/transport_ring.hip
--- a/sos-radiative-transfer_amd/csrc/transport_ring.hip
+++ b/sos-radiative-transfer_amd/csrc/transport_ring.hip
@@ -25,7 +25,7 @@
     asm volatile("s_waitcnt lgkmcnt(0)\n\ts_barrier" ::: "memory");
 }
 
-template <bool ACC, bool SAVED, int PIECES, bool MZ>
+template <bool ACC, bool SAVED, int PIECES, bool MZ, int LR = 0>
 __global__ __launch_bounds__(512) void k_transport_ring(TransportArgs a, int NS, int dbg_arg, int fixcap) {
     constexpr int NWL = 2;
 #ifdef SOSRT_RING_DEBUG
@@ -73,12 +73,20 @@
     const ColDesc* __restrict__ dg = a.desc + b;
     const int nz = dg->nz;
     const ZoneRows<MZ> zr(dg);
+    int mixmask = 0;
+    if constexpr (LR > 0) {
+#pragma unroll
+        for (int z = 0; z < (MZ ? kMaxZones : kRingZones); ++z) mixmask |= (z < nz && dg->mix[z]) ? 1 << z : 0;
+    }
+    auto plain_row = [&](int t) { return LR > 0 && !((mixmask >> zr.of(t)) & 1); };
     const int nfix0 = dg->nfix[0], nfix1 = dg->nfix[1], nfix2 = dg->nfix[2];
     const int surface = dg->surface;
     const double rho = dg->rho;
     const int fbytes = L * D * 8, RB = D * 8;
     const int lbytes = (dbg & 1) ? 0 : fbytes, sbytes = (dbg & 2) ? 0 : fbytes;
     const __amdgpu_buffer_rsrc_t rJ = make_rsrc(a.Jn + (size_t)b * L * D, lbytes);
+    const __amdgpu_buffer_rsrc_t rM = make_rsrc(LR > 0 ? a.mom + (size_t)b * L * kMomStride : a.Jn, (LR > 0 && !(dbg & 1)) ? L * kMomStride * 8 : 0);
+    const __amdgpu_buffer_rsrc_t rZ = make_rsrc(a.Jn, 0);
     const __amdgpu_buffer_rsrc_t rE = make_rsrc(a.Etab + (size_t)(a.erep ? a.erep[b] : b) * L * D, lbytes);
     const __amdgpu_buffer_rsrc_t rIn = make_rsrc(a.In + (size_t)b * L * D, sbytes);
     const __amdgpu_buffer_rsrc_t rIl = make_rsrc(ACC ? a.I + (size_t)b * L * D : a.In, ACC ? lbytes : 0);
@@ -108,6 +116,7 @@
         slot_ld = slot_ld + 1 == NS ? 0 : slot_ld + 1;
         const int half = up ? N * 8 : 0;
         const int vo = lane * 16;
+        const int voM = lane * 16 < kMomStride * 8 ? lane * 16 : 1 << 30;
 #pragma unroll
         for (int i = 0; i < TC / NWL; ++i) {
             const int u = i * NWL + lid;
@@ -115,6 +124,11 @@
 #pragma unroll
             for (int p = 0; p < PIECES; ++p) {
                 const int so = row * RB + half + p * 1024;
+                if constexpr (LR > 0) {
+                    const bool pl = plain_row(row);
+                    const __amdgpu_buffer_rsrc_t rj = pl ? (p == 0 ? rM : rZ) : rJ;
+                    __builtin_amdgcn_raw_ptr_buffer_load_lds(rj, (lds_ptr_t)(dst + (0 * TC + u) * RS + p * 128), 16, pl ? voM : vo, pl ? row * (kMomStride * 8) : so, 0, 0);
+                } else
                 __builtin_amdgcn_raw_ptr_buffer_load_lds(rJ, (lds_ptr_t)(dst + (0 * TC + u) * RS + p * 128), 16, vo, so, 0, 0);
                 __builtin_amdgcn_raw_ptr_buffer_load_lds(rE, (lds_ptr_t)(dst + (1 * TC + u) * RS + p * 128), 16, vo, so, 0, 0);
                 if (ACC) __builtin_amdgcn_raw_ptr_buffer_load_lds(rIl, (lds_ptr_t)(dst + (2 * TC + u) * RS + p * 128), 16, vo, so, 0, 0);
@@ -171,6 +185,14 @@
     } else {
     stamp(1);
     const double mu_up = (valid && tid > 0) ? g.mu[N + tidc] : 1.0;
+    double Vd[kLowRankMax] = {0, 0, 0, 0}, Vu[kLowRankMax] = {0, 0, 0, 0};
+    if constexpr (LR > 0) {
+#pragma unroll
+        for (int q = 0; q < LR; ++q) { Vd[q] = a.lrV[(size_t)q * D + tidc]; Vu[q] = a.lrV[(size_t)q * D + N + tidc]; }
+    }
+    using JS0 = std::integral_constant<int, 0>;
+    using JS1 = std::integral_constant<int, (LR > 0 ? 1 : 0)>;
+    using JS2 = std::integral_constant<int, (LR > 0 ? 2 : 0)>;
     const int uT = lane >> 3, pT = lane & 7;
     const double muT = (pT + 1 < N) ? g.mu[N + pT + 1] : 1.0;
     const double* xrow = s_x + uT * 16;
@@ -309,13 +331,20 @@
             Jprev = Jc[TC - 1];
             t0 += TC;
         };
-        auto chunk = [&](auto special_t, auto mode_t) __attribute__((always_inline)) {
+        auto chunk = [&](auto special_t, auto mode_t, auto jsrc_t) __attribute__((always_inline)) {
+            constexpr int JS = decltype(jsrc_t)::value;
             const double* sp = ring + (size_t)slot_rd * SLOT + tid;
             slot_rd = slot_rd + 1 == NS ? 0 : slot_rd + 1;
             double Jc[TC], Ic[TC], Ec[TC];
 #pragma unroll
             for (int u = 0; u < TC; ++u) {
-                Jc[u] = sp[(0 * TC + u) * RS];
+                if constexpr (JS == 0) {
+                    Jc[u] = sp[(0 * TC + u) * RS];
+                } else {
+                    const double* rec = sp - tid + (0 * TC + u) * RS;
+                    const double e = lowrank_expand<LR>(rec, rec[kMomCf], Vd);
+                    Jc[u] = (JS == 1 || plain_row(min(t0 + u, L - 1))) ? e : sp[(0 * TC + u) * RS];
+                }
                 Ec[u] = sp[(1 * TC + u) * RS];
                 Ic[u] = ACC ? sp[(2 * TC + u) * RS] : 0.0;
             }
@@ -325,13 +354,17 @@
         using M0 = std::integral_constant<int, 0>;
         using M1 = std::integral_constant<int, 1>;
         using M2 = std::integral_constant<int, 2>;
+        auto plain_chunks = [&](auto mode_t, int qe) __attribute__((always_inline)) {
+            if (LR > 0 && q < qe && plain_row(t0)) for (; q < qe; ++q) chunk(std::false_type{}, mode_t, JS1{});
+            else for (; q < qe; ++q) chunk(std::false_type{}, mode_t, JS0{});
+        };
         while (q < NCH) {
             const int qe = q + plain_run(sp_dn, q);
             const int mode = (!wl || (nfx == 0 && !has_small)) ? 0 : ((!has_small && nfx <= 8 && sl[0] >= xb_dn) ? 1 : 2);
-            if (mode == 0) for (; q < qe; ++q) chunk(std::false_type{}, M0{});
-            else if (mode == 1) for (; q < qe; ++q) chunk(std::false_type{}, M1{});
-            else for (; q < qe; ++q) chunk(std::false_type{}, M2{});
-            if (q < NCH) { chunk(std::true_type{}, M2{}); ++q; }
+            if (mode == 0) plain_chunks(M0{}, qe);
+            else if (mode == 1) plain_chunks(M1{}, qe);
+            else plain_chunks(M2{}, qe);
+            if (q < NCH) { chunk(std::true_type{}, M2{}, JS2{}); ++q; }
         }
     }
 
@@ -485,13 +518,20 @@
             Jnext = Jc[TC - 1];
             t0 -= TC;
         };
-        auto chunk = [&](auto special_t, auto mode_t) __attribute__((always_inline)) {
+        auto chunk = [&](auto special_t, auto mode_t, auto jsrc_t) __attribute__((always_inline)) {
+            constexpr int JS = decltype(jsrc_t)::value;
             const double* sp = ring + (size_t)slot_rd * SLOT + tid;
             slot_rd = slot_rd + 1 == NS ? 0 : slot_rd + 1;
             double Jc[TC], Ic[TC], Ec[TC];
 #pragma unroll
             for (int u = 0; u < TC; ++u) {
-                Jc[u] = sp[(0 * TC + u) * RS];
+                if constexpr (JS == 0) {
+                    Jc[u] = sp[(0 * TC + u) * RS];
+                } else {
+                    const double* rec = sp - tid + (0 * TC + u) * RS;
+                    const double e = lowrank_expand<LR>(rec, rec[kMomCf], Vu);
+                    Jc[u] = (JS == 1 || plain_row(max(t0 - u, 0))) ? e : sp[(0 * TC + u) * RS];
+                }
                 Ec[u] = sp[(1 * TC + u) * RS];
                 Ic[u] = ACC ? sp[(2 * TC + u) * RS] : 0.0;
             }
@@ -500,11 +540,15 @@
         };
         using M0 = std::integral_constant<int, 0>;
         using M1 = std::integral_constant<int, 1>;
+        auto plain_chunks = [&](auto mode_t, int qe) __attribute__((always_inline)) {
+            if (LR > 0 && q < qe && plain_row(t0)) for (; q < qe; ++q) chunk(std::false_type{}, mode_t, JS1{});
+            else for (; q < qe; ++q) chunk(std::false_type{}, mode_t, JS0{});
+        };
         while (q < NQ) {
             const int qe = q + plain_run(sp_up, q - NCH);
-            if (!w0) for (; q < qe; ++q) chunk(std::false_type{}, M0{});
-            else for (; q < qe; ++q) chunk(std::false_type{}, M1{});
-            if (q < NQ) { chunk(std::true_type{}, M1{}); ++q; }
+            if (!w0) plain_chunks(M0{}, qe);
+            else plain_chunks(M1{}, qe);
+            if (q < NQ) { chunk(std::true_type{}, M1{}, JS2{}); ++q; }
         }
         if (w0 && notfound && lane == 0 && N - 3 <= 61) s_flag[1] = 1;
     }
@@ -529,8 +573,13 @@
         }
     }
     if (s_flag[0]) {
-        const bool missing = redo_upward_sweep<ACC, SAVED, MZ>(L, N, RB, zr, s_hd, g.mu, rJ, rE, rIn, rI, rS, Bv, ring,
-                                                            rup_v, rup_i);
+        double Vr[kLowRankMax] = {0, 0, 0, 0};
+        if constexpr (LR > 0) {
+#pragma unroll
+            for (int q = 0; q < LR; ++q) Vr[q] = a.lrV[(size_t)q * D + N + tidc];
+        }
+        const bool missing = redo_upward_sweep<ACC, SAVED, MZ, 0, 0, LR>(L, N, RB, zr, s_hd, g.mu, rJ, rE, rIn, rI, rS, Bv, ring,
+                                                            rup_v, rup_i, LR > 0 ? a.mom + (size_t)b * L * kMomStride : nullptr, Vr, mixmask);
         if (missing) {
             if (tid == 0) {
                 a.cv.status[b] = SOSRT_COL_INDEXERROR;
@@ -567,9 +616,10 @@
     const int nt = (int)block.x;
     const int narr = a.accumulate ? 3 : 2;
     const size_t shm = ((size_t)NS * narr * TC * 128 * PIECES + ring_extra_doubles(a.g, nt, a.nzcap)) * sizeof(double);
-#define SOSRT_RING_LAUNCH_Z(ACC_, SAVED_, MZ_)                                                                 \
+#define SOSRT_RING_LAUNCH_Z(ACC_, SAVED_, MZ_) SOSRT_RING_LAUNCH_L(ACC_, SAVED_, MZ_, 0)
+#define SOSRT_RING_LAUNCH_L(ACC_, SAVED_, MZ_, LR_)                                                            \
     do {                                                                                                       \
-        auto kern = k_transport_ring<ACC_, SAVED_, PIECES, MZ_>;                                               \
+        auto kern = k_transport_ring<ACC_, SAVED_, PIECES, MZ_, LR_>;                                          \
         static PerDeviceOnce big_lds;                                                                                 \
         if (big_lds.first()) {                                                                                        \
             hipFuncSetAttribute(reinterpret_cast<const void*>(kern), hipFuncAttributeMaxDynamicSharedMemorySize, \
@@ -582,7 +632,21 @@
         if (a.nzcap > kRingZones) SOSRT_RING_LAUNCH_Z(ACC_, SAVED_, true);                                     \
         else SOSRT_RING_LAUNCH_Z(ACC_, SAVED_, false);                                                         \
     } while (0)
-    if (a.accumulate) {
+#define SOSRT_RING_LAUNCH_MOM(SAVED_)                                                                          \
+    do {                                                                                                       \
+        if (a.nzcap > kRingZones) {                                                                            \
+            if (a.lr_rank == 1) SOSRT_RING_LAUNCH_L(true, SAVED_, true, 1);                                    \
+            else SOSRT_RING_LAUNCH_L(true, SAVED_, true, 2);                                                   \
+        } else {                                                                                               \
+            if (a.lr_rank == 1) SOSRT_RING_LAUNCH_L(true, SAVED_, false, 1);                                   \
+            else SOSRT_RING_LAUNCH_L(true, SAVED_, false, 2);                                                  \
+        }                                                                                                      \
+    } while (0)
+    static_assert(kMomRankMax == 2, "an instantiation per rank");
+    if (a.accumulate && a.mom) {
+        if (a.saved) SOSRT_RING_LAUNCH_MOM(true);
+        else SOSRT_RING_LAUNCH_MOM(false);
+    } else if (a.accumulate) {
         if (a.saved) SOSRT_RING_LAUNCH(true, true);
         else SOSRT_RING_LAUNCH(true, false);
     } else {
@@ -590,6 +654,8 @@
     }
 #undef SOSRT_RING_LAUNCH
 #undef SOSRT_RING_LAUNCH_Z
+#undef SOSRT_RING_LAUNCH_L
+#undef SOSRT_RING_LAUNCH_MOM
 }
 
 }
diff --git a/sos-radiative-transfer_amd/csrc/transport_scan.hip b/sos-radiative-transfer_amd/csrc/transport_scan.hip
--- a/sos-radiative-transfer_amd/csrc/transport_scan.hip
+++ b/sos-radiative-transfer_amd/csrc/transport_scan.hip
@@ -4,7 +4,7 @@
 
 namespace {
 
-template <bool ACC, bool SAVED, bool SPLIT, int NC = 0, bool MZ = false, bool WIDE = false>
+template <bool ACC, bool SAVED, bool SPLIT, int NC = 0, bool MZ = false, bool WIDE = false, bool MOM = false>
 __global__ __launch_bounds__(768) void k_transport_scan(TransportArgs a, int fixcap) {
     const int nparts = SPLIT ? ((NC ? NC : a.g.N) + 63) >> 6 : 1;
     const int part = SPLIT ? (int)(blockIdx.x % nparts) : 0;
@@ -15,7 +15,7 @@
     } else if (ACC && !a.cv.active[b]) {
         return;
     }
-    (void)transport_scan_order<ACC, SAVED, SPLIT, NC, MZ, false, WIDE>(a, fixcap, b, part, ScanFused());
+    (void)transport_scan_order<ACC, SAVED, SPLIT, NC, MZ, false, WIDE, MOM>(a, fixcap, b, part, ScanFused());
 }
 
 inline bool scan_wide(const Grid& g) { return (g.N & 1) || g.N > 256 || (g.L + TC - 1) / TC > 64; }
@@ -47,10 +47,15 @@
     using C = ScanCfg<SPLIT>;
     const int nwc = SPLIT ? 1 : (a.g.N + 63) / 64;
     const dim3 block((nwc * C::SW + NLOAD) * 64);
-    const size_t shm = scan_lds_bytes<SPLIT>(a.g, a.nzcap);
+    const size_t shm = scan_lds_bytes<SPLIT>(a.g, a.nzcap) + (a.mom ? scan_mom_bytes(a.g) : 0);
 #define SOSRT_SCAN_LAUNCH_Z(ACC_, SAVED_, NC_, MZ_)                                                            \
     do {                                                                                                       \
-        auto kern = k_transport_scan<ACC_, SAVED_, SPLIT, NC_, MZ_>;                                           \
+        if (ACC_ && a.mom) SOSRT_SCAN_LAUNCH_M(ACC_, SAVED_, NC_, MZ_, ACC_);                                  \
+        else SOSRT_SCAN_LAUNCH_M(ACC_, SAVED_, NC_, MZ_, false);                                               \
+    } while (0)
+#define SOSRT_SCAN_LAUNCH_M(ACC_, SAVED_, NC_, MZ_, MOM_)                                                      \
+    do {                                                                                                       \
+        auto kern = k_transport_scan<ACC_, SAVED_, SPLIT, NC_, MZ_, false, MOM_>;                              \
         static PerDeviceOnce big_lds;                                                                                 \
         if (big_lds.first()) {                                                                                        \
             hipFuncSetAttribute(reinterpret_cast<const void*>(kern), hipFuncAttributeMaxDynamicSharedMemorySize, \
@@ -76,6 +81,7 @@
 #undef SOSRT_SCAN_LAUNCH
 #undef SOSRT_SCAN_LAUNCH_N
 #undef SOSRT_SCAN_LAUNCH_Z
+#undef SOSRT_SCAN_LAUNCH_M
 }
 
 }
@@ -96,6 +102,10 @@
     return (split ? scan_lds_bytes<true>(g, nzcap) : scan_lds_bytes<false>(g, nzcap)) <= kScanLdsBytes;
 }
 size_t transport_scan_scratch_doubles() { return kScanScratch; }
+bool transport_scan_moments_ok(const Grid& g, int nzcap, bool split) {
+    if (split && scan_wide(g)) return false;
+    return (split ? scan_lds_bytes<true>(g, nzcap) : scan_lds_bytes<false>(g, nzcap)) + scan_mom_bytes(g) <= kScanLdsBytes;
+}
 
 void launch_transport_scan(hipStream_t s, dim3 grid, const TransportArgs& a) {
     if (a.scan_split && a.accumulate && scan_wide(a.g)) launch_scan_wide(s, dim3(transport_scan_parts(a.g) * grid.x), a);
diff --git a/sos-radiative-transfer_amd/csrc/transport_scan_body.hpp b/sos-radiative-transfer_amd/csrc/transport_scan_body.hpp
--- a/sos-radiative-transfer_amd/csrc/transport_scan_body.hpp
+++ b/sos-radiative-transfer_amd/csrc/transport_scan_body.hpp
@@ -25,6 +25,7 @@
 static_assert(kScanChunks * TC / 32 <= 32, "the flagged-row mask of the split form's exchange holds 32 ints: 128 chunks of TC rows");
 constexpr size_t kScanLdsBytes = 152 * 1024;
 typedef __attribute__((address_space(3))) void* lds_ptr_t;
+constexpr int kScanOut = 1 << 30;
 constexpr unsigned kSpinLimit = 1u << 20;
 constexpr unsigned kFusedSpinLimit = 1u << 21;
 struct ScanFused {
@@ -60,9 +61,12 @@
     }
 }
 
-template <bool ACC, bool SAVED, bool SPLIT, int NC = 0, bool MZ = false, bool FUSED = false, bool WIDE = false>
+constexpr int kScanMomStride = 4;
+static_assert(kMomRankMax + 1 <= kScanMomStride, "a row of the LDS table: the moments, the coefficient");
+template <bool ACC, bool SAVED, bool SPLIT, int NC = 0, bool MZ = false, bool FUSED = false, bool WIDE = false, bool MOM = false>
 __device__ __forceinline__ int transport_scan_order(const TransportArgs& a, int fixcap, const int b, const int part, const ScanFused& fu) {
     static_assert(!WIDE || (SPLIT && !FUSED && NC == 0), "WIDE is an instantiation of the plain split form");
+    static_assert(!MOM || (ACC && !WIDE && !FUSED), "the records: orders of a solve, two launches per order, the BASELINE shapes");
     using Cfg = ScanCfg<SPLIT, WIDE>;
     constexpr int SW = Cfg::SW, NST = Cfg::NST, SROW = Cfg::SROW, STAGE = Cfg::STAGE;
     const int nparts = SPLIT ? ((NC ? NC : a.g.N) + 63) >> 6 : 1;
@@ -138,6 +142,7 @@
     int* s_taken = s_landed + NST;
     int* s_nf = s_taken + NST * nwc;
     int* s_nfz = s_nf + (L + 31) / 32;
+    double* s_mom = sm + ((reinterpret_cast<const char*>(s_nfz + kMaxZones) - reinterpret_cast<const char*>(sm)) + 7) / 8;
     __shared__ int s_flag[4];
     double* s_x = s_xw + (size_t)(loader ? 0 : wid) * 2 * TC * 16;
     double* s_xI = s_x + TC * 16;
@@ -146,6 +151,13 @@
     const ColDesc* __restrict__ dg = a.desc + b;
     const int nz = dg->nz;
     const ZoneRows<MZ> zr(dg);
+    int mixmask = 0;
+    if constexpr (MOM) {
+#pragma unroll
+        for (int z = 0; z < (MZ ? kMaxZones : kRingZones); ++z) mixmask |= (z < nz && dg->mix[z]) ? 1 << z : 0;
+    }
+    auto plain_row = [&](int t) __attribute__((always_inline)) { return MOM && !((mixmask >> zr.of(t)) & 1); };
+    const int lr_rank = a.lr_rank;
     const int nfix0 = dg->nfix[0], nfix1 = dg->nfix[1], nfix2 = dg->nfix[2];
     const int surface = dg->surface;
     const double rho = dg->rho;
@@ -155,6 +167,16 @@
     const __amdgpu_buffer_rsrc_t rIn = make_rsrc(a.In + (size_t)b * L * D, fbytes);
     const __amdgpu_buffer_rsrc_t rI = make_rsrc(ACC ? a.I + (size_t)b * L * D : a.In, ACC ? fbytes : 0);
     (void)rJ; (void)rE;
+    double Vd[kLowRankMax] = {0, 0, 0, 0}, Vu[kLowRankMax] = {0, 0, 0, 0};
+    if constexpr (MOM) {
+        if (!loader) {
+#pragma unroll
+            for (int q = 0; q < kMomRankMax; ++q) {
+                Vd[q] = q < lr_rank ? a.lrV[(size_t)q * D + dirc_dn] : 0.0;
+                Vu[q] = q < lr_rank ? a.lrV[(size_t)q * D + N + dirc] : 0.0;
+            }
+        }
+    }
     const __amdgpu_buffer_rsrc_t rS = make_rsrc(SAVED ? a.saved + (size_t)b * a.saved_col_stride : a.In, SAVED ? fbytes : 0);
 
     unsigned long long sp_dn = 0, sp_up = 0, sp_dn1 = 0, sp_up1 = 0;
@@ -220,6 +242,23 @@
         Jx = st[(2 * TC) * SROW];
         asm volatile("" ::: "memory");
         if (lane == 0) l_taken[stg * nwc + lg] = gq + 1;
+        if constexpr (MOM) {
+            const bool up = gq >= NCH;
+            const int t0r = up ? L - 1 - (gq - NCH) * TC : gq * TC;
+            const double* V = up ? Vu : Vd;
+            auto expand = [&](int row, double full) __attribute__((always_inline)) {
+                const lds_double* mp = (const lds_double*)s_mom + row * kScanMomStride;
+                auto uni = [](double x) __attribute__((always_inline)) {
+                    return __hiloint2double(__builtin_amdgcn_readfirstlane(__double2hiint(x)), __builtin_amdgcn_readfirstlane(__double2loint(x)));
+                };
+                double Mq[kLowRankMax] = {uni(mp[0]), uni(mp[1]), 0.0, 0.0};
+                const double e = lowrank_expand<>(Mq, uni(mp[kMomRankMax]), V, lr_rank);
+                return plain_row(row) ? e : full;
+            };
+#pragma unroll
+            for (int u = 0; u < TC; ++u) J[u] = expand(up ? max(t0r - u, 0) : min(t0r + u, L - 1), J[u]);
+            Jx = expand(up ? min(t0r + 1, L - 1) : max(t0r - 1, 0), Jx);
+        }
 #pragma unroll
         for (int u = 0; u < TC; ++u) I[u] = ACC ? bload_aux<LDX>(rI, vo_, CLAMP ? min(max(so0 + u * dso, 0), (L - 1) * RB) : so0 + u * dso) : 0.0;
     };
@@ -251,22 +290,22 @@
                 const int uu = u + hl;
                 const int row = up ? max(t0 - uu, 0) : min(t0 + uu, L - 1);
                 const int vo = vl + row * RB;
-                __builtin_amdgcn_raw_ptr_buffer_load_lds(rJ, (lds_ptr_t)(dst + (0 * TC + u) * SROW), 16, vo, half, 0, LDX);
+                __builtin_amdgcn_raw_ptr_buffer_load_lds(rJ, (lds_ptr_t)(dst + (0 * TC + u) * SROW), 16, plain_row(row) ? kScanOut : vo, half, 0, LDX);
                 __builtin_amdgcn_raw_ptr_buffer_load_lds(rE, (lds_ptr_t)(dst + (1 * TC + u) * SROW), 16, vo, half, 0, 0);
             }
             const int rx = up ? min(t0 + 1, L - 1) : max(t0 - 1, 0);
-            if (lane < 32) __builtin_amdgcn_raw_ptr_buffer_load_lds(rJ, (lds_ptr_t)(dst + (2 * TC) * SROW), 16, vl, rx * RB + half, 0, LDX);
+            if (lane < 32 && !plain_row(rx)) __builtin_amdgcn_raw_ptr_buffer_load_lds(rJ, (lds_ptr_t)(dst + (2 * TC) * SROW), 16, vl, rx * RB + half, 0, LDX);
         } else {
             const int vo = lane * 16;
 #pragma unroll
             for (int u = 0; u < TC; ++u) {
                 const int row = up ? max(t0 - u, 0) : min(t0 + u, L - 1);
                 const int so = row * RB + half;
-                __builtin_amdgcn_raw_ptr_buffer_load_lds(rJ, (lds_ptr_t)(dst + (0 * TC + u) * SROW), 16, vo, so, 0, LDX);
+                if (!plain_row(row)) __builtin_amdgcn_raw_ptr_buffer_load_lds(rJ, (lds_ptr_t)(dst + (0 * TC + u) * SROW), 16, vo, so, 0, LDX);
                 __builtin_amdgcn_raw_ptr_buffer_load_lds(rE, (lds_ptr_t)(dst + (1 * TC + u) * SROW), 16, vo, so, 0, 0);
             }
             const int rx = up ? min(t0 + 1, L - 1) : max(t0 - 1, 0);
-            __builtin_amdgcn_raw_ptr_buffer_load_lds(rJ, (lds_ptr_t)(dst + (2 * TC) * SROW), 16, vo, rx * RB + half, 0, LDX);
+            if (!plain_row(rx)) __builtin_amdgcn_raw_ptr_buffer_load_lds(rJ, (lds_ptr_t)(dst + (2 * TC) * SROW), 16, vo, rx * RB + half, 0, LDX);
         }
     };
     auto load_chunks = [&](int g0, int g1, bool first_issued) __attribute__((always_inline)) {
@@ -299,6 +338,13 @@
             const double* __restrict__ tau = a.tau + (size_t)b * L;
             for (int t = tid; t <= L; t += nt) s_hd[t] = (t == 0 || t == L) ? 0.0 : (tau[t] - tau[t - 1]) * 0.5;
             if (tid < 16) s_prmu[tid] = (tid > 0 && tid < N) ? 1.0 / g.mu[N + tid] : 0.0;
+        }
+        if constexpr (MOM) {
+            const double* __restrict__ rec = a.mom + (size_t)b * L * kMomStride;
+            for (int i = tid; i < L * kScanMomStride; i += nt) {
+                const int t = i / kScanMomStride, k = i - t * kScanMomStride;
+                s_mom[i] = k < kMomRankMax ? rec[(size_t)t * kMomStride + k] : (k == kMomRankMax ? rec[(size_t)t * kMomStride + kMomCf] : 0.0);
+            }
         }
         if (tid < 4) s_flag[tid] = 0;
         for (int i = tid; i < nwc * CR + NST + NST * nwc + (L + 31) / 32; i += nt) s_flagq[i] = 0;
@@ -916,7 +962,16 @@
     if (s_flag[0]) {
         const double U0 = SPLIT ? ((act && surface == SOSRT_SURFACE_SPECULAR) ? rho * s_sfc[N - 1 - tid] : 0.0) : Bv;
         __syncthreads();
-        const bool missing = redo_upward_sweep<ACC, SAVED, MZ, LDX, STX>(L, N, RB, zr, s_hd, g.mu, rJ, rE, rIn, rI, rS, U0,
+        bool missing;
+        if constexpr (MOM) {
+            double Vr[kLowRankMax] = {0, 0, 0, 0};
+#pragma unroll
+            for (int q = 0; q < kMomRankMax; ++q) Vr[q] = q < lr_rank ? a.lrV[(size_t)q * D + N + min(tid, N - 1)] : 0.0;
+            const double* rec = a.mom + (size_t)b * L * kMomStride;
+            missing = lr_rank == 1 ? redo_upward_sweep<ACC, SAVED, MZ, LDX, STX, 1>(L, N, RB, zr, s_hd, g.mu, rJ, rE, rIn, rI, rS, U0, s_stage, rup_v, rup_i, rec, Vr, mixmask)
+                                   : redo_upward_sweep<ACC, SAVED, MZ, LDX, STX, 2>(L, N, RB, zr, s_hd, g.mu, rJ, rE, rIn, rI, rS, U0, s_stage, rup_v, rup_i, rec, Vr, mixmask);
+        } else
+        missing = redo_upward_sweep<ACC, SAVED, MZ, LDX, STX>(L, N, RB, zr, s_hd, g.mu, rJ, rE, rIn, rI, rS, U0,
                                                             s_stage, rup_v, rup_i);
         if (missing) {
             if (tid == 0) {
@@ -954,6 +1009,7 @@
                            g.L + 1 + (WIDE ? 0 : (size_t)g.nsmall * g.L) + 16 + 4 * ND + (size_t)ncw * 2 * TC * 16;
     return doubles * sizeof(double) + ((size_t)(nwc * CR + C::NST + C::NST * nwc + (g.L + 31) / 32 + kMaxZones) * sizeof(int) + 7) / 8 * 8;
 }
+inline size_t scan_mom_bytes(const Grid& g) { return (size_t)g.L * kScanMomStride * sizeof(double); }
 
 }
 }
diff --git a/sos-radiative-transfer_amd/csrc/transport_util.hpp b/sos-radiative-transfer_amd/csrc/transport_util.hpp
--- a/sos-radiative-transfer_amd/csrc/transport_util.hpp
+++ b/sos-radiative-transfer_amd/csrc/transport_util.hpp
@@ -110,6 +110,16 @@
     return __builtin_fma(w, rk, a);
 }
 __device__ __forceinline__ double fix_acc(double c, double x, double acc) { return __builtin_fma(c, x, acc); }
+
+template <int RC = -1>
+__device__ __forceinline__ double lowrank_expand(const double* M, double cf, const double* v, int R = RC) {
+#pragma clang fp contract(off)
+    double o = 0.0;
+#pragma unroll
+    for (int q = 0; q < kLowRankMax; ++q)
+        if (q < (RC >= 0 ? RC : R)) o = __builtin_fma(M[q], v[q], o);
+    return cf * o;
+}
 
 template <bool MZ> struct ZoneRows {
     const ColDesc* dg;
@@ -261,11 +271,12 @@
 }
 
 constexpr int kRedoRows = 8;
-template <bool ACC, bool SAVED, bool MZ, int LDX = 0, int STX = 0>
+template <bool ACC, bool SAVED, bool MZ, int LDX = 0, int STX = 0, int LR = 0>
 __device__ SOSRT_HELPER_INLINE bool redo_upward_sweep(int L, int N, int RB, const ZoneRows<MZ>& zr, const double* s_hd,
                                   const double* __restrict__ gmu, __amdgpu_buffer_rsrc_t rJ, __amdgpu_buffer_rsrc_t rE,
                                   __amdgpu_buffer_rsrc_t rIn, __amdgpu_buffer_rsrc_t rI, __amdgpu_buffer_rsrc_t rS, double U0,
-                                  double* s_work, double& rup_v, double& rup_i) {
+                                  double* s_work, double& rup_v, double& rup_i, const double* __restrict__ mom = nullptr,
+                                  const double* Vu = nullptr, int mixmask = 0) {
     const int tid = threadIdx.x;
     double* s_row = s_work;
     int* s_kf = reinterpret_cast<int*>(s_work + 2 * (N + 2));
@@ -284,6 +295,10 @@
 #pragma unroll
         for (int u = 0; u < kRedoRows; ++u) {
             const int t = max(t0 - u, 0);
+            if (LR > 0 && !((mixmask >> zr.of(t)) & 1)) {
+                const double* rec = mom + (size_t)t * kMomStride;
+                Jc[u] = lowrank_expand<LR>(rec, rec[kMomCf], Vu);
+            } else
             Jc[u] = bload_aux<LDX>(rJ, vo, t * RB);
             Ec[u] = bload(rE, vo, t * RB);
             xo[u] = bload_aux<LDX ? LDX : 1>(rIn, vo, t * RB);
diff --git a/sos-radiative-transfer_amd/sosrt/_lib.py b/sos-radiative-transfer_amd/sosrt/_lib.py
--- a/sos-radiative-transfer_amd/sosrt/_lib.py
+++ b/sos-radiative-transfer_amd/sosrt/_lib.py
@@ -21,6 +21,8 @@
 _dp = POINTER(c_double)
 _ip = POINTER(c_int)
 
+ADDED_SYMBOLS = {"sosrt_plan_launch2"}
+
 SIGNATURES = {
     "sosrt_last_error": (c_char_p, []),
     "sosrt_version": (c_int, []),
@@ -37,6 +39,7 @@
     "sosrt_set_order_loop": (c_int, [c_void_p, c_int]),
     "sosrt_order_loop_stats": (c_int, [c_void_p, _ip, _ip, POINTER(c_longlong)]),
     "sosrt_plan_launch": (c_int, [c_void_p, c_int, c_int, c_int, c_int, c_int, _ip]),
+    "sosrt_plan_launch2": (c_int, [c_void_p, c_int, c_int, c_int, c_int, c_int, c_int, _ip]),
     "sosrt_set_first_order": (c_int, [c_void_p, c_int]),
     "sosrt_set_grid": (c_int, [c_void_p, c_void_p]),
     "sosrt_set_phase": (c_int, [c_void_p, c_void_p, c_void_p]),
@@ -116,6 +119,8 @@
         _preload_hip_runtime()
         L = ctypes.CDLL(LIB_PATH)
         for name, (res, args) in SIGNATURES.items():
+            if name in ADDED_SYMBOLS and os.environ.get("SOSRT_LIB") and not hasattr(L, name):
+                continue
             fn = getattr(L, name)
             fn.restype = res
             fn.argtypes = args
diff --git a/sos-radiative-transfer_amd/sosrt/solver.py b/sos-radiative-transfer_amd/sosrt/solver.py
--- a/sos-radiative-transfer_amd/sosrt/solver.py
+++ b/sos-radiative-transfer_amd/sosrt/solver.py
@@ -457,6 +457,14 @@
         keys = ("groups", "gemm", "tail_cols", "transport", "parts", "repair", "order_loop", "ol_parts", "ol_grid")
         return dict(zip(keys, list(out)))
 
+    def plan_jn_moments(self, batch, live, surface="specular", zones=3, cus=0, need_small=False, saving=False):
+        sf = {"none": _lib.SURFACE_NONE, "specular": _lib.SURFACE_SPECULAR, "lambertian": _lib.SURFACE_LAMBERTIAN,
+              "lambertian_readme": _lib.SURFACE_LAMBERTIAN_README}[surface]
+        out = (ctypes.c_int * 10)()
+        check(lib().sosrt_plan_launch2(self._h, int(batch), int(live), sf, int(zones), int(cus),
+                                       (1 if need_small else 0) | (2 if saving else 0), out))
+        return int(out[9])
+
     def microbench(self, which):
         r = ctypes.c_double()
         check(lib().sosrt_microbench(self._h, int(which), ctypes.byref(r)))
```

After: 128,600 (median of 6 runs). 1.04x the previous value.
